# amathislab/BUCTD

Hardware: AMD Instinct MI355X
Metric: images/sec (train) BUCTD-CoAM-W48 384x288 (higher is better)
Workload: dtype f32 (3x3 convs: operands split exactly into 3 bf16 pieces, 6 bf16 MFMAs per product, fp32 accumulate - fp32-class); 1 GPU; BUCTD-CoAM-W48 (pose_hrnet_coam, ATT_MODULES [F,T,F,F], colored condition) 384x288 CrowdPose-14kpt full train step: fwd + JointsMSE + bwd + grad all-reduce + Adam + arg-max accuracy decode; global_batch=32, batch_per_gpu=32, input=N x 6 x 384 x 288 fp32, params=115581770, parallelism=dp1, hip_streams=4, conv_math=bf16x6, step_graph=False

## Files before the change

buctd_amd/_C.py:

```python
import ctypes as C
import os

import torch

_HERE = os.path.dirname(os.path.abspath(__file__))
LIB_PATH = os.path.join(_HERE, "lib", "libbuctd_hip.so")


class ConvDesc(C.Structure):
    _fields_ = [(n, C.c_int) for n in ("N", "H", "W", "Ci", "Co", "R", "S", "stride", "pad", "Ho", "Wo")]


class BasicBlockDesc(C.Structure):
    _fields_ = ([(n, C.c_int) for n in ("N", "H", "W", "C")] +
                [(n, C.c_void_p) for n in ("x", "w1_fwd", "w2_fwd", "w1_bwd", "w2_bwd", "gamma1", "beta1", "gamma2", "beta2",
                                           "running_mean1", "running_var1", "running_mean2", "running_var2")] +
                [(n, C.c_float) for n in ("eps1", "momentum1", "eps2", "momentum2")] +
                [(n, C.c_void_p) for n in ("z1", "z2", "y", "acc", "stat")])


class BasicBlockGrads(C.Structure):
    _fields_ = ([(n, C.c_void_p) for n in ("dy", "dz2", "dres", "dy1", "dz1", "dx", "dw1", "dw2", "dgamma1", "dbeta1",
                                           "dgamma2", "dbeta2")] +
                [(n, C.c_int) for n in ("acc_w1", "acc_w2", "acc_bn1", "acc_bn2")] +
                [("bn_acc", C.c_void_p), ("wg_ws", C.c_void_p), ("wg_ws_bytes", C.c_size_t)])


class BnAccIn(C.Structure):
    _fields_ = [("acc", C.c_void_p), ("rows", C.c_long), ("eps", C.c_float), ("momentum", C.c_float),
                ("mean_out", C.c_void_p), ("invstd_out", C.c_void_p), ("running_mean", C.c_void_p),
                ("running_var", C.c_void_p)]


class C3Conv(C.Structure):
    _fields_ = ([(n, C.c_int) for n in ("N", "H", "W", "Ci", "Co")] +
                [(n, C.c_void_p) for n in ("x", "wprep", "residual")] + [("relu", C.c_int)] +
                [(n, C.c_void_p) for n in ("y", "stats_acc")] + [("in_bn", C.POINTER(BnAccIn))] +
                [(n, C.c_void_p) for n in ("in_gamma", "in_beta")] + [("in_relu", C.c_int)] +
                [(n, C.c_void_p) for n in ("bn_z", "bn_y", "bn_mean", "bn_invstd", "bn_gamma", "bn_beta", "bn_acc")])


class C3ConvEval(C.Structure):
    _fields_ = ([(n, C.c_int) for n in ("N", "H", "W", "Ci", "Co")] +
                [(n, C.c_void_p) for n in ("x", "wprep", "scale", "shift", "residual")] + [("relu", C.c_int), ("y", C.c_void_p)])


class BnApplyItem(C.Structure):
    _fields_ = [("z", C.c_void_p), ("st", BnAccIn), ("gamma", C.c_void_p), ("beta", C.c_void_p), ("residual", C.c_void_p),
                ("relu", C.c_int), ("y", C.c_void_p), ("rows", C.c_long), ("C", C.c_int)]


class BnBwdItem(C.Structure):
    _fields_ = ([(n, C.c_void_p) for n in ("dy", "y", "z", "mean", "invstd", "gamma", "beta")] +
                [("relu", C.c_int), ("rows", C.c_long), ("C", C.c_int)] +
                [(n, C.c_void_p) for n in ("dz", "dres", "dgamma", "dbeta")] +
                [("accumulate", C.c_int), ("acc", C.c_void_p), ("acc_ready", C.c_int)])


class Wg3Conv(C.Structure):
    _fields_ = ([(n, C.c_int) for n in ("N", "H", "W", "Ci", "Co")] +
                [(n, C.c_void_p) for n in ("x", "dy", "dw")] + [("accumulate", C.c_int)] +
                [(n, C.c_void_p) for n in ("x_mean", "x_invstd", "x_gamma", "x_beta")] + [("x_relu", C.c_int)] +
                [("workspace", C.c_void_p), ("workspace_bytes", C.c_size_t)])


class MhaArgs(C.Structure):
    _fields_ = ([(n, C.c_int) for n in ("B", "T", "h", "dh")] +
                [(n, C.c_void_p) for n in ("q", "k", "v")] + [(n, C.c_int) for n in ("ldq", "ldk", "ldv")] +
                [("out", C.c_void_p), ("ldo", C.c_int), ("lse", C.c_void_p), ("scale", C.c_float), ("p_drop", C.c_float),
                 ("dout", C.c_void_p), ("lddo", C.c_int)] +
                [(n, C.c_void_p) for n in ("dq", "dk", "dv")] + [(n, C.c_int) for n in ("lddq", "lddk", "lddv")])


class RefineArgs(C.Structure):
    _fields_ = ([(n, C.c_void_p) for n in ("coords", "maxvals", "offset", "center", "scale", "box_score", "items",
                                           "cond_trunc", "cond_joints", "status", "hist_preds", "hist_score",
                                           "hist_box_score", "hist_keypoint_score", "hist_center", "hist_scale")] +
                [(n, C.c_int) for n in ("B", "K", "pass_", "passes", "heatmap_w", "heatmap_h", "crop_w", "crop_h")] +
                [(n, C.c_double) for n in ("margin", "aspect_ratio", "in_vis_thre", "scale_thre")])


class SampleGeomArgs(C.Structure):
    _fields_ = ([(n, C.c_void_p) for n in ("joints", "joints_vis", "cond", "cond_vis", "center", "scale", "bbox",
                                           "half_body", "draws", "bbox_draws", "flags", "pair", "items", "out_joints",
                                           "out_joints_vis", "out_cond", "out_cond_vis", "cond_trunc", "target_xy",
                                           "target_vis", "out_center", "out_scale", "out_rotation", "status")] +
                [(n, C.c_int) for n in ("B", "K", "crop_w", "crop_h", "keep_rect", "bbox_aug")] +
                [(n, C.c_double) for n in ("margin", "aspect_ratio", "scale_thre", "stride_x", "stride_y")])


class MatmulDesc(C.Structure):
    _fields_ = [
        ("batch", C.c_int), ("M", C.c_int), ("N", C.c_int), ("K", C.c_int),
        ("a_layout", C.c_int), ("b_layout", C.c_int),
        ("lda", C.c_int), ("ldb", C.c_int), ("ldc", C.c_int),
        ("stride_a", C.c_long), ("stride_b", C.c_long), ("stride_c", C.c_long),
        ("Kc", C.c_int), ("group_stride_a", C.c_long), ("group_stride_bk", C.c_long),
        ("Nc", C.c_int), ("group_stride_bn", C.c_long), ("group_stride_c", C.c_long),
        ("alpha", C.c_float), ("bias_axis", C.c_int),
    ]


_P = C.c_void_p
_I = C.c_int
_L = C.c_long
_F = C.c_float
_U64 = C.c_uint64
_SZ = C.c_size_t
_PD = C.POINTER(ConvDesc)
_PM = C.POINTER(MatmulDesc)
_PI = C.POINTER(C.c_int)

SIGNATURES = {
    "buctd_version": (_I, []),
    "buctd_last_error": (C.c_char_p, []),
    "buctd_conv2d_fwd": (_I, [_PD, _P, _P, _P, _P, _P, _P, _I, _P, _P, _P]),
    "buctd_conv2d_fwd_thin": (_I, [_PD]),
    "buctd_conv2d_dgrad": (_I, [_PD, _P, _P, _P, _P, _P, _P]),
    "buctd_conv2d_stats_groups": (_I, [_PD, _I, _PI, _PI]),
    "buctd_conv2d_wgrad_workspace": (_SZ, [_PD]),
    "buctd_conv2d_wgrad": (_I, [_PD, _P, _P, _P, _I, _P, _SZ, _P]),
    "buctd_conv2d_plan": (_I, [_PD, _I, _I, _PI]),
    "buctd_matmul_workspace": (_SZ, [_PM]),
    "buctd_matmul": (_I, [_PM, _P, _P, _P, _P, _P, _SZ, _P]),
    "buctd_matmul_plan": (_I, [_PM, _P, _P, _PI]),
    "buctd_bn_finalize": (_I, [_P, _P, _I, _I, _L, _I, _F, _F, _P, _P, _P, _P, _P]),
    "buctd_conv3x3_bf16x3_supported": (_I, [_I, _I, _I, _I, _I]),
    "buctd_conv3x3_bf16x3_stats_groups": (_I, [_I, _I, _I, _I, _I, _PI, _PI]),
    "buctd_conv3x3_bf16x3_prep_bytes": (_SZ, [_I, _I, _I]),
    "buctd_conv3x3_bf16x3_prep": (_I, [_I, _I, _P, _I, _P, _P]),
    "buctd_conv3x3_bf16x3_prep_batched": (_I, [_P, _I, _L, _P]),
    "buctd_conv3x3_bf16x3": (_I, [_I, _I, _I, _I, _I, _P, _P, _P, _P, _P, _P, _I, _P, _P, _P, _P]),
    "buctd_conv3x3_wgrad_bf16x3_supported": (_I, [_I, _I, _I, _I, _I]),
    "buctd_conv3x3_wgrad_bf16x3_workspace": (_SZ, [_I, _I, _I, _I, _I]),
    "buctd_conv3x3_wgrad_bf16x3": (_I, [_I, _I, _I, _I, _I, _P, _P, _P, _I, _P, _SZ, _P]),
    "buctd_conv3x3_bf16x6_supported": (_I, [_I, _I, _I, _I, _I]),
    "buctd_conv3x3_bf16x6_stats_groups": (_I, [_I, _I, _I, _I, _I, _PI, _PI]),
    "buctd_conv3x3_bf16x6_prep_bytes": (_SZ, [_I, _I, _I]),
    "buctd_conv3x3_bf16x6_prep": (_I, [_I, _I, _P, _I, _P, _P]),
    "buctd_conv3x3_bf16x6": (_I, [_I, _I, _I, _I, _I, _P, _P, _P, _P, _P, _P, _I, _P, _P, _P, _P]),
    "buctd_conv3x3_bf16x6_bnin": (_I, [_I, _I, _I, _I, _I, _P, _P, _P, _P, _P, _P, _I, _P, _P, _P, _P, _P, _P, _P, _I, _P]),
    "buctd_conv3x3_bf16x6_bnstat": (_I, [_I, _I, _I, _I, _I, _P, _P, _P, _P, _P, _P, _P, _P, _P, _P, _P, _P]),
    "buctd_bn_bwd_from_partials": (_I, [_P, _P, _P, _P, _P, _P, _P, _I, _L, _I, _P, _I, _P, _P, _P, _P, _I, _P, _SZ, _P]),
    "buctd_conv3x3_wgrad_bf16x6_bnin": (_I, [_I, _I, _I, _I, _I, _P, _P, _P, _I, _P, _P, _P, _P, _I, _P, _SZ, _P]),
    "buctd_conv3x3_wgrad_bf16x6_supported": (_I, [_I, _I, _I, _I, _I]),
    "buctd_conv3x3_wgrad_bf16x6_workspace": (_SZ, [_I, _I, _I, _I, _I]),
    "buctd_conv3x3_wgrad_bf16x6": (_I, [_I, _I, _I, _I, _I, _P, _P, _P, _I, _P, _SZ, _P]),
    "buctd_bn_stats": (_I, [_P, _L, _I, _P, _PI, _PI, _P]),
    "buctd_bn_stats_groups": (_I, [_L, _I, _PI, _PI]),
    "buctd_bn_apply": (_I, [_P, _P, _P, _P, _P, _P, _I, _P, _L, _I, _P]),
    "buctd_bn_bwd_workspace": (_SZ, [_L, _I]),
    "buctd_bn_bwd": (_I, [_P, _P, _P, _P, _P, _P, _P, _I, _L, _I, _P, _P, _P, _P, _I, _P, _SZ, _P]),
    "buctd_bn_fold": (_I, [_P, _P, _P, _P, _F, _I, _P, _P, _P]),
    "buctd_bn_acc_bytes": (_SZ, [_I]),
    "buctd_bn_apply_acc": (_I, [_P, C.POINTER(BnAccIn), _P, _P, _P, _I, _P, _L, _I, _P]),
    "buctd_bn_bwd_acc": (_I, [_P, _P, _P, _P, _P, _P, _P, _I, _L, _I, _P, _P, _P, _P, _I, _P, _I, _P]),
    "buctd_conv3x3_bf16x6_acc": (_I, [_I] * 5 + [_P, _P, _P, _I, _P, _P, C.POINTER(BnAccIn), _P, _P, _I, _P]),
    "buctd_conv3x3_bf16x6_bnstat_acc": (_I, [_I] * 5 + [_P] * 12),
    "buctd_gconv_x6_fwd_acc": (_I, [_I] * 6 + [_P] * 6),
    "buctd_conv3x3_bf16x6_group": (_I, [_I, C.POINTER(C3Conv), _P]),
    "buctd_conv3x3_bf16x6_group_eval": (_I, [_I, C.POINTER(C3ConvEval), _P]),
    "buctd_conv3x3_bf16x6_group_workgroups": (_I, [_I, C.POINTER(C3Conv)]),
    "buctd_conv3x3_bf16x6_plan": (_I, [_I, _I, _I, _I, _I, _I, C.POINTER(C.c_int)]),
    "buctd_conv3x3_wgrad_bf16x6_plan": (_I, [_I, _I, _I, _I, _I, C.POINTER(C.c_int)]),
    "buctd_gconv_wgrad_x6_supported": (_I, [_I] * 6),
    "buctd_gconv_wgrad_x6_workspace": (_SZ, [_I] * 6),
    "buctd_gconv_wgrad_x6": (_I, [_I] * 6 + [_P, _P, _P, _I, _P, _SZ, _P]),
    "buctd_bn_apply_acc_group": (_I, [_I, C.POINTER(BnApplyItem), _P]),
    "buctd_bn_bwd_acc_group": (_I, [_I, C.POINTER(BnBwdItem), _P]),
    "buctd_conv3x3_wgrad_bf16x6_group_workspace": (_SZ, [_I] * 6),
    "buctd_conv3x3_wgrad_bf16x6_group": (_I, [_I, C.POINTER(Wg3Conv), _P]),
    "buctd_conv3x3_wgrad_bf16x6_group_workgroups": (_I, [_I, C.POINTER(Wg3Conv)]),
    "buctd_stream_fork": (_I, [_P, _P]),
    "buctd_basic_branches_fwd_train": (_I, [_I, _I, C.POINTER(BasicBlockDesc), _P]),
    "buctd_basic_branches_bwd": (_I, [_I, _I, C.POINTER(BasicBlockDesc), C.POINTER(BasicBlockGrads), _P, _P]),
    "buctd_basic_chain_fwd_train": (_I, [_I, C.POINTER(BasicBlockDesc), _P]),
    "buctd_basic_chain_bwd": (_I, [_I, C.POINTER(BasicBlockDesc), C.POINTER(BasicBlockGrads), _P, _P]),
    "buctd_x6_image_dims": (_I, [_I, _I, _I, _P, _P]),
    "buctd_x6_image_bytes": (C.c_size_t, [_I, _I, _I]),
    "buctd_x6_image": (_I, [_P, _I, _I, _I, _L, _L, _I, _L, _L, _I, _P, _P]),
    "buctd_x6_gemm": (_I, [_I, _I, _I, _P, _P, _P, _I, _F, _P, _L, _I, _L, _P]),
    "buctd_add": (_I, [_P, _P, _P, _L, _I, _P]),
    "buctd_add_n": (_I, [C.POINTER(_P), _I, _P, _L, _P]),
    "buctd_mul": (_I, [_P, _P, _P, _L, _P]),
    "buctd_scale": (_I, [_P, _P, _F, _P, _L, _P]),
    "buctd_copy_channels": (_I, [_P, _L, _I, _I, _P, _I, _I, _I, _P]),
    "buctd_add_bcast": (_I, [_P, _P, _P, _L, _L, _P]),
    "buctd_relu_bwd": (_I, [_P, _P, _P, _L, _P]),
    "buctd_colsum_workspace": (_SZ, [_L, _I]),
    "buctd_colsum": (_I, [_P, _L, _I, _P, _I, _P, _SZ, _P]),
    "buctd_nchw_to_nhwc": (_I, [_P, _I, _I, _I, _I, _I, _I, _P, _P]),
    "buctd_nhwc_to_nchw": (_I, [_P, _I, _I, _I, _I, _P, _P]),
    "buctd_fuse_sum": (_I, [C.POINTER(_P), _PI, _I, _I, _I, _I, _I, _I, _P, _P]),
    "buctd_fuse_sum_bwd": (_I, [_P, _P, _I, _I, _I, _I, _I, _P, _P]),
    "buctd_resize_bilinear": (_I, [_P, _I, _I, _I, _I, _I, _I, _I, _I, _P, _P]),
    "buctd_maxpool3x3s2_fwd": (_I, [_P, _I, _I, _I, _I, _P, _P, _P]),
    "buctd_maxpool3x3s2_bwd": (_I, [_P, _P, _I, _I, _I, _I, _P, _P]),
    "buctd_softmax_dropout_fwd": (_I, [_P, _L, _I, _F, _F, _U64, _P, _P, _P]),
    "buctd_softmax_dropout_bwd": (_I, [_P, _P, _L, _I, _F, _F, _U64, _P, _P]),
    "buctd_softmax_dropout_fwd_dseed": (_I, [_P, _L, _I, _F, _F, _P, _P, _P, _P]),
    "buctd_softmax_dropout_bwd_dseed": (_I, [_P, _P, _L, _I, _F, _F, _P, _P, _P]),
    "buctd_dropout": (_I, [_P, _P, _L, _F, _U64, _P]),
    "buctd_dropout_dseed": (_I, [_P, _P, _L, _F, _P, _P]),
    "buctd_dropout_seed_fill": (_I, [_P, _I, _U64, _U64, _P]),
    "buctd_attn_smallqk_supported": (_I, [_I, _I, _I]),
    "buctd_attn_smallqk_fwd": (_I, [_I, _I, _I, _I, _P, _P, _P, _F, _F, _U64, _I, _P, _P, _P, _P]),
    "buctd_attn_smallqk_bwd": (_I, [_I, _I, _I, _I, _P, _P, _P, _P, _P, _P, _P, _F, _F, _U64, _I, _P, _P, _P, _P, _P]),
    "buctd_attn_smallqk_fwd_dseed": (_I, [_I, _I, _I, _I, _P, _P, _P, _F, _F, _P, _I, _P, _P, _P, _P]),
    "buctd_attn_smallqk_bwd_dseed": (_I, [_I, _I, _I, _I, _P, _P, _P, _P, _P, _P, _P, _F, _F, _P, _I, _P, _P, _P, _P, _P]),
    "buctd_layernorm_fwd": (_I, [_P, _P, _P, _L, _I, _F, _P, _P, _P, _P]),
    "buctd_add_layernorm_fwd": (_I, [_P, _P, _P, _P, _L, _I, _F, _P, _P, _P, _P, _P]),
    "buctd_layernorm_bwd_workspace": (_SZ, [_L, _I]),
    "buctd_layernorm_bwd": (_I, [_P, _P, _P, _P, _P, _L, _I, _P, _P, _P, _I, _P, _SZ, _P]),
    "buctd_joints_mse": (_I, [_P, _P, _P, _I, _I, _I, _P, _P, _F, _P, _SZ, _P]),
    "buctd_joints_ohkm_mse_workspace": (_SZ, [_I, _I]),
    "buctd_joints_ohkm_mse": (_I, [_P, _P, _P, _I, _I, _I, _I, _P, _P, _F, _P, _SZ, _P]),
    "buctd_argmax_decode": (_I, [_P, _I, _I, _I, _P, _P, _P, _P]),
    "buctd_warp_affine_norm": (_I, [_P, _I, _I, _I, _P, _P, _P, _L, _P, _P]),
    "buctd_cond_render_into": (_I, [_P, _I, _P, _I, _I, _I, _I, _I, _I, _P, _L, _P, _SZ, _P]),
    "buctd_cond_geometry": (_I, [_P, _P, _P, _P, _I, _I, _P, _P, _P, _P]),
    "buctd_cond_mirror": (_I, [_P, _I, _P, _P, _I, _I, _I, _P, _P]),
    "buctd_mirror_rows": (_I, [_P, _L, _P, _L, _P, _I, _I, _I, _I, _I, _P]),
    "buctd_refine_step": (_I, [C.POINTER(RefineArgs), _P]),
    "buctd_sample_geometry": (_I, [C.POINTER(SampleGeomArgs), _P]),
    "buctd_synthesize_pose": (_I, [_P, _P, _P, _P, _P, _P, _I, _I, _I, C.c_ulonglong, _P, _P]),
    "buctd_mha_fwd_supported": (_I, [_I, _I]),
    "buctd_mha_fwd": (_I, [_I, _I, _I, _P, _P, _P, _I, _I, _F, _P, _P, _P]),
    "buctd_mha_fwd_bf16x6": (_I, [_I, _I, _I, _P, _P, _P, _I, _I, _F, _P, _P, _P]),
    "buctd_gconv_x6_supported": (_I, [_I] * 7),
    "buctd_gconv_x6_prep_bytes": (_SZ, [_I, _I, _I, _I]),
    "buctd_gconv_x6_prep": (_I, [_I, _I, _I, _P, _I, _P, _P]),
    "buctd_gconv_x6_prep_item_bytes": (_SZ, []),
    "buctd_gconv_x6_prep_item": (_I, [_I, _I, _I, _P, _I, _P, _P]),
    "buctd_gconv_x6_prep_batched": (_I, [_P, _I, _P]),
    "buctd_gconv_x6_stats_groups": (_I, [_I] * 6 + [_PI, _PI]),
    "buctd_gconv_x6_fwd": (_I, [_I] * 6 + [_P] * 6 + [_I, _P, _P, _P, _P]),
    "buctd_gconv_x6_dgrad": (_I, [_I] * 6 + [_P] * 4 + [_P]),
    "buctd_mha_fwd_bf16x6_workspace": (_SZ, [_I, _I, _I]),
    "buctd_mha_fwd_bf16x6_ws": (_I, [_I, _I, _I, _P, _P, _P, _I, _I, _F, _P, _P, _P, _SZ, _P]),
    "buctd_mha_train_supported": (_I, [_I, _I]),
    "buctd_mha_fwd_train": (_I, [_I, _I, _I, _P, _P, _P, _I, _I, _F, _F, _U64, _P, _P, _P]),
    "buctd_mha_bwd_workspace": (_SZ, [_I, _I]),
    "buctd_mha_bwd": (_I, [_I, _I, _I, _P, _P, _P, _I, _I, _P, _P, _P, _F, _F, _U64, _P, _P, _I, _P, _I, _P, _SZ, _P]),
    "buctd_mha_fwd_train_dseed": (_I, [_I, _I, _I, _P, _P, _P, _I, _I, _F, _F, _P, _P, _P, _P]),
    "buctd_mha_bwd_dseed": (_I, [_I, _I, _I, _P, _P, _P, _I, _I, _P, _P, _P, _F, _F, _P, _P, _P, _I, _P, _I, _P, _SZ, _P]),
    "buctd_mha_heads_fwd_supported": (_I, [_I, _I, _I]),
    "buctd_mha_heads_fwd": (_I, [C.POINTER(MhaArgs), _P]),
    "buctd_mha_heads_fwd_bf16x6": (_I, [C.POINTER(MhaArgs), _P]),
    "buctd_mha_heads_train_supported": (_I, [_I, _I, _I]),
    "buctd_mha_heads_fwd_train": (_I, [C.POINTER(MhaArgs), _U64, _P]),
    "buctd_mha_heads_bwd_workspace": (_SZ, [_I, _I, _I]),
    "buctd_mha_heads_bwd": (_I, [C.POINTER(MhaArgs), _U64, _P, _SZ, _P]),
    "buctd_mha_heads_fwd_train_dseed": (_I, [C.POINTER(MhaArgs), _P, _P]),
    "buctd_mha_heads_bwd_dseed": (_I, [C.POINTER(MhaArgs), _P, _P, _SZ, _P]),
    "buctd_nms_workspace": (_SZ, [_I]),
    "buctd_nms": (_I, [_P, _P, _P, _I, _I, _F, _P, _SZ, _P]),
    "buctd_cpu_nms": (_I, [_P, _I, _P, _F, _P, _P]),
    "buctd_argmax_decode_refined": (_I, [_P, _I, _I, _I, _P, _P, _P, _P, _P]),
    "buctd_argmax_decode_dark": (_I, [_P, _I, _I, _I, _P, _P, _P, _P, _P]),
    "buctd_gaussian_target": (_I, [_P, _P, _I, _I, _I, _I, _F, _F, _F, _P, _P, _P]),
    "buctd_cond_render_workspace": (_SZ, [_I, _I, _I, _I]),
    "buctd_cond_render": (_I, [_P, _I, _P, _I, _I, _I, _I, _I, _I, _P, _P, _SZ, _P]),
    "buctd_flipback_avg": (_I, [_P, _P, _P, _I, _I, _I, _I, _I, _P, _P]),
    "buctd_sgd_step": (_I, [_P, _P, _P, _L, _F, _F, _F, _I, _I, _F, _P]),
    "buctd_adam_step": (_I, [_P, _P, _P, _P, _L, _F, _F, _F, _F, _I, _F, _P]),
    "buctd_bf16_pack_conv": (_I, [_P, _L, _L, _L, _L, _I, _I, _I, _P, _P, _P, _P, _P, _F, _P, _P, _P]),
    "buctd_bf16_conv": (_I, [_P, _I, _I, _I, _I, _P, _P, _I, _I, _I, _I, _P, _I, _I, _P, _P, _SZ, _P]),
    "buctd_bf16_fuse_sum": (_I, [C.POINTER(_P), _PI, _I, _I, _I, _I, _I, _I, _P, _P]),
    "buctd_bf16_from_f32": (_I, [_P, _L, _P, _P]),
}

_lib = None


class BuctdHipError(RuntimeError):
    pass


def lib():
    global _lib
    if _lib is None:
        if not os.path.isfile(LIB_PATH):
            raise BuctdHipError(
                f"{LIB_PATH} is missing - build it with `make` (or __graft_entry__.build()); "
                "buctd_amd has no CPU / eager fallback")
        handle = C.CDLL(LIB_PATH, mode=C.RTLD_GLOBAL)
        for name, (res, args) in SIGNATURES.items():
            fn = getattr(handle, name)
            fn.restype = res
            fn.argtypes = args
        _lib = handle
    return _lib


def check(rc, what=""):
    if rc != 0:
        msg = lib().buctd_last_error()
        raise BuctdHipError(f"{what} failed ({rc}): {msg.decode() if msg else ''}")


_raw_stream = getattr(torch._C, "_cuda_getCurrentRawStream", None)
_raw_device = getattr(torch._C, "_cuda_getDevice", None)


def current_stream_handle():
    if _raw_stream is not None and _raw_device is not None:
        return _raw_stream(_raw_device())
    return torch.cuda.current_stream().cuda_stream


def stream_ptr():
# ... 10 lines not shown
```

buctd_amd/csrc/block.hip:

```cpp
#include "common.h"
#include "../../include/buctd_hip.h"
#include <string.h>

#define BLK_TRY(call)      \
  do {                     \
    const int rc_ = (call); \
    if (rc_) return rc_;   \
  } while (0)

static bool fwd_ptrs_ok(const buctd_basic_block& b) {
  return b.x && b.w1_fwd && b.w2_fwd && b.z1 && b.z2 && b.y && b.acc && b.stat;
}

static bool bwd_ptrs_ok(const buctd_basic_block& b, const buctd_basic_block_grads& g) {
  return b.x && b.w1_bwd && b.w2_bwd && b.z1 && b.z2 && b.y && b.stat && g.dy && g.dres && g.dy1 && g.dw1 && g.dw2 && g.bn_acc &&
         g.wg_ws && g.dz2 && g.dz1;
}


static float* mean1_of(const buctd_basic_block& b) { return b.stat; }
static float* invstd1_of(const buctd_basic_block& b) { return b.stat + b.C; }
static float* mean2_of(const buctd_basic_block& b) { return b.stat + 2 * b.C; }
static float* invstd2_of(const buctd_basic_block& b) { return b.stat + 3 * b.C; }
static void* acc1_of(void* acc) { return acc; }
static void* acc2_of(void* acc, int C) { return (char*)acc + buctd_bn_acc_bytes(C); }

static void acc_in_of(const buctd_basic_block& b, int second, buctd_bn_acc_in* st) {
  st->acc = second ? acc2_of(b.acc, b.C) : acc1_of(b.acc);
  st->rows = (long)b.N * b.H * b.W;
  st->eps = second ? b.eps2 : b.eps1;
  st->momentum = second ? b.momentum2 : b.momentum1;
  st->mean_out = second ? mean2_of(b) : mean1_of(b);
  st->invstd_out = second ? invstd2_of(b) : invstd1_of(b);
  st->running_mean = second ? b.running_mean2 : b.running_mean1;
  st->running_var = second ? b.running_var2 : b.running_var1;
}

static buctd_c3_conv c3_of(const buctd_basic_block& b) {
  buctd_c3_conv c;
  memset(&c, 0, sizeof(c));
  c.N = b.N; c.H = b.H; c.W = b.W; c.Ci = c.Co = b.C;
  return c;
}

static int stream_fork(hipStream_t from, hipStream_t to, const char* who) {
  if (from == to) return BUCTD_OK;
  static thread_local hipEvent_t evs[16] = {nullptr};
  int devid = 0;
  if (hipGetDevice(&devid) != hipSuccess || devid < 0 || devid >= 16) {
    buctd_set_error("%s: cannot identify the current device", who);
    return BUCTD_ELAUNCH;
  }
  hipEvent_t& ev = evs[devid];
  if (!ev && hipEventCreateWithFlags(&ev, hipEventDisableTiming) != hipSuccess) {
    buctd_set_error("%s: hipEventCreate failed", who);
    return BUCTD_ELAUNCH;
  }
  if (hipEventRecord(ev, from) != hipSuccess || hipStreamWaitEvent(to, ev, 0) != hipSuccess) {
    buctd_set_error("%s: stream fork failed", who);
    return BUCTD_ELAUNCH;
  }
  return BUCTD_OK;
}

static int issue_conv_fwd(bool group, int n, const buctd_c3_conv* c, void* s) {
  if (group) return buctd_conv3x3_bf16x6_group(n, c, s);
  return buctd_conv3x3_bf16x6_acc(c->N, c->H, c->W, c->Ci, c->Co, c->x, c->wprep, c->residual, c->relu, c->y, c->stats_acc,
                                  c->in_bn, c->in_gamma, c->in_beta, c->in_relu, s);
}
static int issue_dgrad(bool group, int n, const buctd_c3_conv* c, void* s) {
  if (group) return buctd_conv3x3_bf16x6_group(n, c, s);
  if (c->bn_acc)
    return buctd_conv3x3_bf16x6_bnstat_acc(c->N, c->H, c->W, c->Ci, c->Co, c->x, c->wprep, c->residual, c->y, c->bn_z, c->bn_y,
                                           c->bn_mean, c->bn_invstd, c->bn_gamma, c->bn_beta, c->bn_acc, s);
  return buctd_conv3x3_bf16x6(c->N, c->H, c->W, c->Ci, c->Co, c->x, c->wprep, nullptr, nullptr, nullptr, c->residual, 0, c->y,
                              nullptr, nullptr, s);
}
static int issue_wgrad(bool group, int n, const buctd_wg3_conv* c, void* s) {
  if (group) return buctd_conv3x3_wgrad_bf16x6_group(n, c, s);
  if (c->x_mean)
    return buctd_conv3x3_wgrad_bf16x6_bnin(c->N, c->H, c->W, c->Ci, c->Co, c->x, c->dy, c->dw, c->accumulate, c->x_mean,
                                           c->x_invstd, c->x_gamma, c->x_beta, c->x_relu, c->workspace, c->workspace_bytes, s);
  return buctd_conv3x3_wgrad_bf16x6(c->N, c->H, c->W, c->Ci, c->Co, c->x, c->dy, c->dw, c->accumulate, c->workspace,
                                    c->workspace_bytes, s);
}
static int issue_bn_apply(bool group, int n, const buctd_bn_apply_item* a, void* s) {
  if (group) return buctd_bn_apply_acc_group(n, a, s);
  return buctd_bn_apply_acc(a->z, &a->st, a->gamma, a->beta, a->residual, a->relu, a->y, a->rows, a->C, s);
}
static int issue_bn_bwd(bool group, int n, const buctd_bn_bwd_item* i, void* s) {
  if (group) return buctd_bn_bwd_acc_group(n, i, s);
  return buctd_bn_bwd_acc(i->dy, i->y, i->z, i->mean, i->invstd, i->gamma, i->beta, i->relu, i->rows, i->C, i->dz, i->dres,
                          i->dgamma, i->dbeta, i->accumulate, i->acc, i->acc_ready, s);
}

#define BR_MAX 4

static int row_fwd_train(bool group, int nb, int n, const buctd_basic_block* blocks, void* stream) {
  for (int k = 0; k < n; ++k) {
    buctd_c3_conv cv[BR_MAX];
    buctd_bn_acc_in st1[BR_MAX];
    buctd_bn_apply_item ap[BR_MAX];
    for (int b = 0; b < nb; ++b) {
      const buctd_basic_block& B = blocks[b * n + k];
      buctd_c3_conv& c = cv[b] = c3_of(B);
      c.x = B.x; c.wprep = B.w1_fwd; c.y = B.z1; c.stats_acc = acc1_of(B.acc);
    }
    BLK_TRY(issue_conv_fwd(group, nb, cv, stream));
    for (int b = 0; b < nb; ++b) {
      const buctd_basic_block& B = blocks[b * n + k];
      buctd_c3_conv& c = cv[b];
      acc_in_of(B, 0, &st1[b]);
      c.x = B.z1; c.wprep = B.w2_fwd; c.y = B.z2; c.stats_acc = acc2_of(B.acc, B.C);
      c.in_bn = &st1[b]; c.in_gamma = B.gamma1; c.in_beta = B.beta1; c.in_relu = 1;
    }
    BLK_TRY(issue_conv_fwd(group, nb, cv, stream));
    for (int b = 0; b < nb; ++b) {
      const buctd_basic_block& B = blocks[b * n + k];
      buctd_bn_apply_item& a = ap[b];
      a.z = B.z2;
      acc_in_of(B, 1, &a.st);
      a.gamma = B.gamma2; a.beta = B.beta2; a.residual = B.x; a.relu = 1; a.y = B.y;
      a.rows = a.st.rows; a.C = B.C;
    }
    BLK_TRY(issue_bn_apply(group, nb, ap, stream));
  }
  return BUCTD_OK;
}

static bool bn2_sums_chain(const buctd_basic_block* b, const buctd_basic_block_grads* g) {
  return g->dx && g->dx == g[-1].dy && g[-1].bn_acc && b[-1].y == b->x && b[-1].N == b->N && b[-1].H == b->H && b[-1].W == b->W &&
         b[-1].C == b->C;
}

static int row_bwd(bool group, const char* who, int nb, int n, const buctd_basic_block* blocks,
                   const buctd_basic_block_grads* grads, void* stream, void* side_stream) {
  hipStream_t main_s = (hipStream_t)stream, side_s = side_stream ? (hipStream_t)side_stream : main_s;
  bool ready[BR_MAX] = {false, false, false, false};
  for (int k = n - 1; k >= 0; --k) {
    buctd_bn_bwd_item bi[BR_MAX];
    buctd_wg3_conv wg[BR_MAX];
    buctd_c3_conv cv[BR_MAX];
    bool chain[BR_MAX];
    for (int b = 0; b < nb; ++b) {
      const buctd_basic_block& B = blocks[b * n + k];
      const buctd_basic_block_grads& G = grads[b * n + k];
      chain[b] = k > 0 && bn2_sums_chain(&B, &G);
      bi[b] = buctd_bn_bwd_item{G.dy, B.y, B.z2, mean2_of(B), invstd2_of(B), B.gamma2, nullptr, 1, (long)B.N * B.H * B.W, B.C,
                                G.dz2, G.dres, G.dgamma2, G.dbeta2, G.acc_bn2, acc2_of(G.bn_acc, B.C), ready[b] ? 1 : 0};
    }
    BLK_TRY(issue_bn_bwd(group, nb, bi, stream));
    BLK_TRY(stream_fork(main_s, side_s, who));
    for (int b = 0; b < nb; ++b) {
      const buctd_basic_block& B = blocks[b * n + k];
      const buctd_basic_block_grads& G = grads[b * n + k];
      wg[b] = buctd_wg3_conv{B.N, B.H, B.W, B.C, B.C, B.z1, G.dz2, G.dw2, G.acc_w2, mean1_of(B), invstd1_of(B), B.gamma1, B.beta1,
                             1, G.wg_ws, G.wg_ws_bytes};
    }
    BLK_TRY(issue_wgrad(group, nb, wg, side_s));
    for (int b = 0; b < nb; ++b) {
      const buctd_basic_block& B = blocks[b * n + k];
      const buctd_basic_block_grads& G = grads[b * n + k];
      buctd_c3_conv& c = cv[b] = c3_of(B);
      c.x = G.dz2; c.wprep = B.w2_bwd; c.y = G.dy1;
      c.bn_z = B.z1; c.bn_mean = mean1_of(B); c.bn_invstd = invstd1_of(B); c.bn_gamma = B.gamma1; c.bn_beta = B.beta1;
      c.bn_acc = acc1_of(G.bn_acc);
    }
    BLK_TRY(issue_dgrad(group, nb, cv, stream));
    for (int b = 0; b < nb; ++b) {
      const buctd_basic_block& B = blocks[b * n + k];
      const buctd_basic_block_grads& G = grads[b * n + k];
      bi[b] = buctd_bn_bwd_item{G.dy1, nullptr, B.z1, mean1_of(B), invstd1_of(B), B.gamma1, B.beta1, 1, (long)B.N * B.H * B.W, B.C,
                                G.dz1, nullptr, G.dgamma1, G.dbeta1, G.acc_bn1, acc1_of(G.bn_acc), 1};
    }
    BLK_TRY(issue_bn_bwd(group, nb, bi, stream));
    BLK_TRY(stream_fork(main_s, side_s, who));
    for (int b = 0; b < nb; ++b) {
      const buctd_basic_block& B = blocks[b * n + k];
      const buctd_basic_block_grads& G = grads[b * n + k];
      wg[b] = buctd_wg3_conv{B.N, B.H, B.W, B.C, B.C, B.x, G.dz1, G.dw1, G.acc_w1, nullptr, nullptr, nullptr, nullptr, 0,
                             G.wg_ws, G.wg_ws_bytes};
    }
    BLK_TRY(issue_wgrad(group, nb, wg, side_s));
    int m = 0;
    for (int b = 0; b < nb; ++b) {
      const buctd_basic_block& B = blocks[b * n + k];
      const buctd_basic_block_grads& G = grads[b * n + k];
      ready[b] = chain[b];
      if (!G.dx) continue;
      buctd_c3_conv& c = cv[m++] = c3_of(B);
      c.x = G.dz1; c.wprep = B.w1_bwd; c.residual = G.dres; c.y = G.dx;
      if (chain[b]) {
        const buctd_basic_block& Bp = blocks[b * n + k - 1];
        c.bn_z = Bp.z2; c.bn_y = Bp.y; c.bn_mean = mean2_of(Bp); c.bn_invstd = invstd2_of(Bp); c.bn_gamma = Bp.gamma2;
        c.bn_acc = acc2_of(grads[b * n + k - 1].bn_acc, B.C);
      }
    }
    if (m) BLK_TRY(issue_dgrad(group, m, cv, stream));
  }
  return BUCTD_OK;
}

extern "C" int buctd_basic_chain_fwd_train(int n, const buctd_basic_block* blocks, void* stream) {
  BUCTD_CHECK_ARG(n > 0 && blocks, "buctd_basic_chain_fwd_train: bad argument");
  for (int k = 0; k < n; ++k) BUCTD_CHECK_ARG(fwd_ptrs_ok(blocks[k]), "buctd_basic_chain_fwd_train: null pointer in block %d", k);
  return row_fwd_train(false, 1, n, blocks, stream);
}
extern "C" int buctd_basic_chain_bwd(int n, const buctd_basic_block* blocks, const buctd_basic_block_grads* grads, void* stream,
                                     void* side_stream) {
  BUCTD_CHECK_ARG(n > 0 && blocks && grads, "buctd_basic_chain_bwd: bad argument");
  for (int k = 0; k < n; ++k)
    BUCTD_CHECK_ARG(bwd_ptrs_ok(blocks[k], grads[k]), "buctd_basic_chain_bwd: null pointer in block %d", k);
  return row_bwd(false, "buctd_basic_chain_bwd", 1, n, blocks, grads, stream, side_stream);
}

extern "C" int buctd_basic_branches_fwd_train(int nb, int n, const buctd_basic_block* blocks, void* stream) {
  BUCTD_CHECK_ARG(nb > 0 && nb <= BR_MAX && n > 0 && blocks, "buctd_basic_branches_fwd_train: 1..%d branches", BR_MAX);
  for (int i = 0; i < nb * n; ++i)
    BUCTD_CHECK_ARG(fwd_ptrs_ok(blocks[i]), "buctd_basic_branches_fwd_train: null pointer in block %d", i);
  return row_fwd_train(true, nb, n, blocks, stream);
}
extern "C" int buctd_basic_branches_bwd(int nb, int n, const buctd_basic_block* blocks, const buctd_basic_block_grads* grads,
                                        void* stream, void* side_stream) {
  BUCTD_CHECK_ARG(nb > 0 && nb <= BR_MAX && n > 0 && blocks && grads, "buctd_basic_branches_bwd: 1..%d branches", BR_MAX);
  for (int i = 0; i < nb * n; ++i)
    BUCTD_CHECK_ARG(bwd_ptrs_ok(blocks[i], grads[i]), "buctd_basic_branches_bwd: null pointer in block %d", i);
  return row_bwd(true, "buctd_basic_branches_bwd", nb, n, blocks, grads, stream, side_stream);
}

extern "C" int buctd_stream_fork(void* from, void* to) {
  return stream_fork((hipStream_t)from, (hipStream_t)to, "buctd_stream_fork");
}
```

buctd_amd/csrc/c3_common.h:

```cpp
#pragma once
#include "common.h"
#include <stdlib.h>
#include "../../include/buctd_hip.h"
#include "bn_acc.h"

typedef __bf16 bf16x8 __attribute__((ext_vector_type(8)));
typedef unsigned short u16x4 __attribute__((ext_vector_type(4)));

#define CK 32

template <int NP> struct Geo;
template <> struct Geo<2> {
  static constexpr int ROWB = 160;
  static constexpr int PST = 64;
  static constexpr int CPR = 8;
  static constexpr int BROW = 128;
  static constexpr int BLDS = 160;
};
template <> struct Geo<3> {
  static constexpr int ROWB = 96;
  static constexpr int PST = 32;
  static constexpr int CPR = 4;
  static constexpr int BROW = 192;
  static constexpr int BLDS = 224;
};

struct C3Args {
  const float* x;
  const unsigned char* wp;
  float* out;
  const float* bias;
  const float* scale;
  const float* shift;
  const float* res;
  float* stats;
  int* counts;
  int N, H, W, Ci, Co;
  int SW, IB, P;
  int relu, na;
  const float* in_mean;
  const float* in_invstd;
  const float* in_gamma;
  const float* in_beta;
  int in_relu;
  int col_major;
  unsigned ib_mul, ib_sh, sw_mul, sw_sh;
  int omap, oH, oW, ost, oy0, ox0;
  const float* bs_z;
  const float* bs_y;
  const float* bs_mean;
  const float* bs_invstd;
  const float* bs_gamma;
  const float* bs_beta;
  float* bs_part;
  long long* stats_acc;
  long long* bs_acc;
  BnAccFwd in_acc;
};

#define C3G_MAX 4
struct C3Group {
  C3Args conv[C3G_MAX];
  int nconv;
  int tiles[C3G_MAX];
  int gx[C3G_MAX];
  int gy[C3G_MAX];
  int variant[C3G_MAX];
};

#define C3_EPI_EXCH_OFF 24576
#define C3_EPI_LDS (C3_EPI_EXCH_OFF + 256 * 16)

__device__ __forceinline__ int fast_div(int n, unsigned mul, unsigned sh) {
  return (int)(__umulhi((unsigned)n, mul) >> sh);
}

typedef float c3_f32x2 __attribute__((ext_vector_type(2)));
typedef __bf16 c3_bf16x2 __attribute__((ext_vector_type(2)));
typedef unsigned c3_u32x2 __attribute__((ext_vector_type(2)));
template <int NP, int PST>
__device__ __forceinline__ void split_store_pk(unsigned char* row, int c, f32x4 v) {
  c3_f32x2 lo = {v.x, v.y}, hi = {v.z, v.w};
#pragma unroll
  for (int q = 0; q < NP; ++q) {
    const unsigned a = __builtin_bit_cast(unsigned, __builtin_convertvector(lo, c3_bf16x2));
    const unsigned b = __builtin_bit_cast(unsigned, __builtin_convertvector(hi, c3_bf16x2));
    *reinterpret_cast<c3_u32x2*>(row + q * PST + 2 * c) = (c3_u32x2){a, b};
    if (q + 1 < NP) {
      lo -= (c3_f32x2){__uint_as_float(a << 16), __uint_as_float(a & 0xffff0000u)};
      hi -= (c3_f32x2){__uint_as_float(b << 16), __uint_as_float(b & 0xffff0000u)};
    }
  }
}

template <int NP, int PST>
__device__ __forceinline__ void split_store(unsigned char* row, int c, f32x4 v) {
#pragma unroll
  for (int q = 0; q < NP; ++q) {
    u16x4 pc;
#pragma unroll
    for (int j = 0; j < 4; ++j) {
      const __bf16 h = (__bf16)v[j];
      pc[j] = __builtin_bit_cast(unsigned short, h);
      v[j] -= (float)h;
    }
    *reinterpret_cast<u16x4*>(row + q * PST + 2 * c) = pc;
  }
}

#define MAX_SW 75

static inline int c3_row_width(int W) { return W + 1; }

template <int V>
struct IC { static constexpr int value = V; };

template <int MF, int NF, int WM, int WN>
__device__ __forceinline__ void c3_epilogue(const C3Args& p, f32x4 (&acc)[MF][NF], unsigned char* smem, int bx, int by,
                                            int p0, int n0) {
  const int t = threadIdx.x, lane = t & 63, wave = t >> 6;
  const int i16 = lane & 15, g = lane >> 4;
  const int wave_m = wave % WM, wave_n = wave / WM;
  constexpr int MR = MF * 16;
  constexpr int RH = (MR + 63) / 64;
  constexpr int LD = NF * 16 + 4;
  constexpr int EP = 1;
  static_assert(MR <= 128, "c3_epilogue: at most 128 rows per wave");
  float* stg = reinterpret_cast<float*>(smem) + wave * (EP * 16 * LD);
  int* rowoff = reinterpret_cast<int*>(smem) + 4 * EP * 16 * LD + wave * 128;
  unsigned long long vmask[RH];
  int cnt = 0;
#pragma unroll
  for (int h = 0; h < RH; ++h) {
    int myoff = -1;
    const int r = lane + 64 * h;
    if (r < MR) {
      const int pp = p0 + wave_m * MR + r;
      if (pp < p.P) {
        const int n = fast_div(pp, p.ib_mul, p.ib_sh);
        const int rem = pp - n * p.IB;
        const int yy = fast_div(rem, p.sw_mul, p.sw_sh), xx = rem - yy * p.SW;
        if (n < p.N && yy >= 1 && xx >= 1 && xx <= p.W)
          myoff = p.omap ? ((n * p.oH + (yy - 1) * p.ost + p.oy0) * p.oW + (xx - 1) * p.ost + p.ox0) * p.Co
                         : ((n * p.H + yy - 1) * p.W + xx - 1) * p.Co;
      }
    }
    vmask[h] = __ballot(myoff >= 0);
    cnt += __popcll(vmask[h]);
    rowoff[r] = myoff;
  }
  auto valid = [&](int row) -> bool { return (vmask[row >> 6] >> (row & 63)) & 1ull; };
  const int grp = bx * WM + wave_m;
  if (p.stats && p.counts && by == 0 && wave_n == 0 && lane == 0) p.counts[grp] = cnt;
  const int ncol0 = n0 + wave_n * NF * 16;
  float bv[NF];
#pragma unroll
  for (int nf = 0; nf < NF; ++nf) bv[nf] = p.bias ? p.bias[ncol0 + nf * 16 + i16] : 0.f;
  double2* exch = reinterpret_cast<double2*>(smem + C3_EPI_EXCH_OFF);
  if (p.stats || p.stats_acc) {
    const float inv_cnt = cnt > 0 ? 1.f / (float)cnt : 0.f;
#pragma unroll
    for (int nf = 0; nf < NF; ++nf) {
      float s1 = 0.f;
#pragma unroll
      for (int mf = 0; mf < MF; ++mf)
#pragma unroll
        for (int rg = 0; rg < 4; ++rg) s1 += valid(mf * 16 + g * 4 + rg) ? acc[mf][nf][rg] + bv[nf] : 0.f;
      s1 += __shfl_xor(s1, 16, 64);
      s1 += __shfl_xor(s1, 32, 64);
      const float mean = s1 * inv_cnt;
      float s2 = 0.f;
#pragma unroll
      for (int mf = 0; mf < MF; ++mf)
#pragma unroll
        for (int rg = 0; rg < 4; ++rg) {
          const float d = acc[mf][nf][rg] + bv[nf] - mean;
          s2 += valid(mf * 16 + g * 4 + rg) ? d * d : 0.f;
        }
      s2 += __shfl_xor(s2, 16, 64);
      s2 += __shfl_xor(s2, 32, 64);
      if (g == 0) {
        const int n = ncol0 + nf * 16 + i16;
        if (p.stats) *reinterpret_cast<float2*>(p.stats + ((long)grp * p.Co + n) * 2) = make_float2(mean, s2);
        if (p.stats_acc) {
          const double nn = (double)cnt, m = (double)mean;
          exch[wave_m * (WN * NF * 16) + wave_n * NF * 16 + nf * 16 + i16] = make_double2(nn * m, (double)s2 + nn * m * m);
        }
      }
    }
    if (p.stats_acc) {
      __syncthreads();
      if (t < WN * NF * 16) {
        double a1 = 0.0, a2 = 0.0;
#pragma unroll
        for (int w = 0; w < WM; ++w) {
          const double2 v = exch[w * (WN * NF * 16) + t];
          a1 += v.x;
          a2 += v.y;
        }
        bnacc_add(p.stats_acc, p.Co, bnacc_shard(), n0 + t, a1, a2);
      }
    }
  }
  constexpr int Q4 = NF * 4;
  constexpr int NACC = (64 % Q4 == 0) ? 1 : 3;
  static_assert(NF <= 4 && (64 % Q4 == 0 || Q4 == 12), "c3_epilogue: unexpected column count for the bs reduction");
  f32x4 bs1[NACC], bs2[NACC];
#pragma unroll
  for (int j = 0; j < NACC; ++j) bs1[j] = bs2[j] = (f32x4){0.f, 0.f, 0.f, 0.f};
  const bool bs_on = p.bs_part != nullptr || p.bs_acc != nullptr;
  const bool bs_rebuild = bs_on && p.bs_y == nullptr;
#define C3_EPI_SYNC() __builtin_amdgcn_wave_barrier()
  constexpr int NI = EP * NF;
  constexpr int NPASS = MF / EP;
  f32x4 pre_r[2][NI], pre_z[2][NI], pre_y[2][NI];
  const bool has_res = p.res != nullptr;
  const bool has_y = bs_on && !bs_rebuild;
  C3_EPI_SYNC();
  auto issue = [&](int ps, int buf) {
#pragma unroll
    for (int k = 0; k < NI; ++k) {
      const int item = lane + 64 * k;
      const int row = item / (NF * 4), c4 = item - row * (NF * 4);
      const int off = rowoff[ps * EP * 16 + row];
      const int o = off >= 0 ? off + ncol0 + c4 * 4 : 0;
      if (has_res) pre_r[buf][k] = *reinterpret_cast<const f32x4*>(p.res + o);
      if (bs_on) pre_z[buf][k] = *reinterpret_cast<const f32x4*>(p.bs_z + o);
      if (has_y) pre_y[buf][k] = *reinterpret_cast<const f32x4*>(p.bs_y + o);
    }
  };
  if (has_res || bs_on) issue(0, 0);
#pragma unroll
  for (int ps = 0; ps < NPASS; ++ps) {
    if (ps) C3_EPI_SYNC();
    if ((has_res || bs_on) && ps + 1 < NPASS) issue(ps + 1, (ps + 1) & 1);
#pragma unroll
    for (int e = 0; e < EP; ++e)
#pragma unroll
      for (int nf = 0; nf < NF; ++nf)
#pragma unroll
        for (int rg = 0; rg < 4; ++rg)
          stg[(e * 16 + g * 4 + rg) * LD + nf * 16 + i16] = acc[ps * EP + e][nf][rg] + bv[nf];
    C3_EPI_SYNC();
#pragma unroll
    for (int k = 0; k < NI; ++k) {
      const int item = lane + 64 * k;
      const int row = item / (NF * 4), c4 = item - row * (NF * 4);
      f32x4 v = *reinterpret_cast<const f32x4*>(stg + row * LD + c4 * 4);
      const int off = rowoff[ps * EP * 16 + row];
      const int n = ncol0 + c4 * 4;
      if (off >= 0) {
        if (p.scale) {
          const f32x4 sc = *reinterpret_cast<const f32x4*>(p.scale + n);
          const f32x4 sh = *reinterpret_cast<const f32x4*>(p.shift + n);
#pragma unroll
          for (int j = 0; j < 4; ++j) v[j] = v[j] * sc[j] + sh[j];
        }
        if (has_res) {
          const f32x4 r = pre_r[ps & 1][k];
#pragma unroll
          for (int j = 0; j < 4; ++j) v[j] += r[j];
        }
        if (p.relu) {
#pragma unroll
          for (int j = 0; j < 4; ++j) v[j] = fmaxf(v[j], 0.f);
        }
        *reinterpret_cast<f32x4*>(p.out + off + n) = v;
        if (bs_on) {
          const f32x4 zz = pre_z[ps & 1][k];
          const f32x4 mu = *reinterpret_cast<const f32x4*>(p.bs_mean + n);
          const f32x4 is = *reinterpret_cast<const f32x4*>(p.bs_invstd + n);
          f32x4 yy;
          if (bs_rebuild) {
            const f32x4 sc = is * *reinterpret_cast<const f32x4*>(p.bs_gamma + n);
            yy = (zz - mu) * sc + *reinterpret_cast<const f32x4*>(p.bs_beta + n);
          } else {
            yy = pre_y[ps & 1][k];
          }
          f32x4 gm = v;
#pragma unroll
          for (int j = 0; j < 4; ++j)
            if (!(yy[j] > 0.f)) gm[j] = 0.f;
          bs1[k % NACC] += gm;
          bs2[k % NACC] += gm * (zz - mu) * is;
        }
      }
    }
  }
  if (bs_on) {
    __syncthreads();
    f32x4* red = reinterpret_cast<f32x4*>(smem) + (size_t)wave * (NACC * 64 * 2);
#pragma unroll
    for (int j = 0; j < NACC; ++j) {
      red[(j * 64 + lane) * 2 + 0] = bs1[j];
      red[(j * 64 + lane) * 2 + 1] = bs2[j];
    }
    __syncthreads();
    if (lane < Q4) {
      f32x4 a1 = (f32x4){0.f, 0.f, 0.f, 0.f}, a2 = a1;
#pragma unroll
      for (int j = 0; j < NACC; ++j) {
        const int first = ((lane - (64 * j) % Q4) % Q4 + Q4) % Q4;
        for (int l = first; l < 64; l += Q4) {
          a1 += red[(j * 64 + l) * 2 + 0];
          a2 += red[(j * 64 + l) * 2 + 1];
        }
      }
      if (p.bs_part) {
        float* dst = p.bs_part + ((long)grp * 2) * p.Co + ncol0 + lane * 4;
        *reinterpret_cast<f32x4*>(dst) = a1;
        *reinterpret_cast<f32x4*>(dst + p.Co) = a2;
      }
      if (p.bs_acc) {
#pragma unroll
        for (int j = 0; j < 4; ++j)
          exch[wave_m * (WN * NF * 16) + wave_n * NF * 16 + lane * 4 + j] = make_double2((double)a1[j], (double)a2[j]);
      }
    }
    if (p.bs_acc) {
      __syncthreads();
      if (t < WN * NF * 16) {
        double a1 = 0.0, a2 = 0.0;
#pragma unroll
        for (int w = 0; w < WM; ++w) {
          const double2 v = exch[w * (WN * NF * 16) + t];
          a1 += v.x;
          a2 += v.y;
        }
        bnacc_add(p.bs_acc, p.Co, bnacc_shard(), n0 + t, a1, a2);
      }
    }
  }
}


static inline void magic_u32(unsigned d, unsigned* mul, unsigned* sh) {
  if (d == 1) { *mul = 0xFFFFFFFFu; *sh = 0; return; }
  unsigned l = 0;
  while ((1ull << l) < d) ++l;
  const unsigned long long m = ((1ull << (31 + l)) + d - 1) / d;
  *mul = (unsigned)m;
  *sh = l - 1;
}
```

buctd_amd/csrc/c3_lean.h:

```cpp
#pragma once
#include "c3_common.h"

enum { C3M_IN_BN = 1, C3M_STATS = 2, C3M_RES = 4, C3M_BS_REBUILD = 8, C3M_BS_Y = 16 };

#define C3_OOB 0x80000000u
__device__ __forceinline__ __amdgpu_buffer_rsrc_t c3_rsrc(const void* ptr, unsigned bytes) {
  return __builtin_amdgcn_make_buffer_rsrc(const_cast<void*>(ptr), 0, bytes, 0x00020000);
}
__device__ __forceinline__ f32x4 c3_bload(__amdgpu_buffer_rsrc_t r, unsigned off) {
  typedef unsigned u32x4_ __attribute__((ext_vector_type(4)));
  return __builtin_bit_cast(f32x4, __builtin_amdgcn_raw_buffer_load_b128(r, off, 0, 0));
}
__device__ __forceinline__ void c3_bstore(__amdgpu_buffer_rsrc_t r, unsigned off, f32x4 v) {
  typedef unsigned u32x4_ __attribute__((ext_vector_type(4)));
  __builtin_amdgcn_raw_buffer_store_b128(__builtin_bit_cast(u32x4_, v), r, off, 0, 0);
}

static inline size_t c3l_tab_bytes(int Ci, int BN) { return (size_t)3 * Ci * 4 + (size_t)4 * BN * 4; }

template <int MF, int NF, int WM, int WN, int MODE>
__device__ __forceinline__ void c3l_epilogue(const C3Args& p, f32x4 (&acc)[MF][NF], unsigned char* smem, float* tab, int p0,
                                             int n0) {
  constexpr bool STATS = (MODE & C3M_STATS) != 0, RES = (MODE & C3M_RES) != 0;
  constexpr bool BSR = (MODE & C3M_BS_REBUILD) != 0, BSY = (MODE & C3M_BS_Y) != 0, BS = BSR || BSY;
  static_assert(!(STATS && BS), "c3l_epilogue: forward statistics and backward sums never meet in one launch");
  const int t = threadIdx.x, lane = t & 63;
  const int wave = __builtin_amdgcn_readfirstlane(t >> 6);
  const int i16 = lane & 15, g = lane >> 4;
  const int wave_m = wave % WM, wave_n = wave / WM;
  constexpr int MR = MF * 16;
  constexpr int RH = (MR + 63) / 64;
  constexpr int LD = NF * 16 + 4;
  constexpr int BN = WN * NF * 16;
  constexpr int Q4 = NF * 4;
  constexpr int NACC = (64 % Q4 == 0) ? 1 : 3;
  constexpr int NI = NF;
  static_assert(MR <= 128 && NF <= 4 && (64 % Q4 == 0 || Q4 == 12), "c3l_epilogue: unexpected tile shape");
  float* stg = reinterpret_cast<float*>(smem) + wave * (16 * LD);
  int* rowoff = reinterpret_cast<int*>(smem) + 4 * 16 * LD + wave * 128;
  double2* exch = reinterpret_cast<double2*>(smem + C3_EPI_EXCH_OFF);

  const int oH = p.omap ? p.oH : p.H, oW = p.omap ? p.oW : p.W, ost = p.omap ? p.ost : 1;
  const int oy0 = p.omap ? p.oy0 : 0, ox0 = p.omap ? p.ox0 : 0;
  const unsigned obytes = (unsigned)p.N * oH * oW * p.Co * 4u;
  const __amdgpu_buffer_rsrc_t r_out = c3_rsrc(p.out, obytes);
  int cnt = 0;
  int r0 = -1;
#pragma unroll
  for (int h = 0; h < RH; ++h) {
    unsigned myoff = C3_OOB;
    const int r = lane + 64 * h;
    const int pp = p0 + wave_m * MR + r;
    const int n = fast_div(pp, p.ib_mul, p.ib_sh);
    const int rem = pp - n * p.IB;
    const int yy = fast_div(rem, p.sw_mul, p.sw_sh), xx = rem - yy * p.SW;
    if ((r < MR) & (pp < p.P) & (n < p.N) & (yy >= 1) & (xx >= 1) & (xx <= p.W))
      myoff = (unsigned)(((n * oH + (yy - 1) * ost + oy0) * oW + (xx - 1) * ost + ox0) * p.Co) * 4u;
    if (STATS) {
      const unsigned long long vm = __ballot(myoff != C3_OOB);
      cnt += __popcll(vm);
      if (r0 < 0 && vm) r0 = 64 * h + __builtin_ctzll(vm);
    }
    if (r < MR) reinterpret_cast<unsigned*>(rowoff)[r] = myoff;
  }
  const int ncol0 = n0 + wave_n * NF * 16;
  float* piv = tab + wave * (NF * 16);
  const float* btab = tab + wave_n * NF * 16;
  if constexpr (STATS) {
    r0 = r0 < 0 ? 0 : r0;
    const int mf0 = r0 >> 4, g0 = (r0 >> 2) & 3, rg0 = r0 & 3;
    float pv[NF];
#pragma unroll
    for (int nf = 0; nf < NF; ++nf) pv[nf] = 0.f;
#pragma unroll
    for (int mf = 0; mf < MF; ++mf)
      if (mf == mf0) {
#pragma unroll
        for (int nf = 0; nf < NF; ++nf)
          pv[nf] = rg0 == 0 ? acc[mf][nf][0] : rg0 == 1 ? acc[mf][nf][1] : rg0 == 2 ? acc[mf][nf][2] : acc[mf][nf][3];
      }
    if (g == g0) {
#pragma unroll
      for (int nf = 0; nf < NF; ++nf) piv[nf * 16 + i16] = pv[nf];
    }
  }
  __builtin_amdgcn_wave_barrier();

  const float* sp[NI];
  const unsigned* rp[NI];
  int c4_k[NI];
#pragma unroll
  for (int k = 0; k < NI; ++k) {
    const int item = lane + 64 * k;
    const int row = item / Q4;
    c4_k[k] = item - row * Q4;
    sp[k] = stg + row * LD + c4_k[k] * 4;
    rp[k] = reinterpret_cast<const unsigned*>(rowoff) + row;
  }
  const unsigned colb = (unsigned)ncol0 * 4u;
  f32x4 s1[NACC], s2[NACC], pq[NACC];
#pragma unroll
  for (int j = 0; j < NACC; ++j) {
    s1[j] = s2[j] = (f32x4){0.f, 0.f, 0.f, 0.f};
    if constexpr (STATS) pq[j] = *reinterpret_cast<const f32x4*>(piv + c4_k[j] * 4);
  }
  [[maybe_unused]] __amdgpu_buffer_rsrc_t r_res, r_z, r_y;
  if constexpr (RES) r_res = c3_rsrc(p.res, obytes);
  if constexpr (BS) r_z = c3_rsrc(p.bs_z, obytes);
  if constexpr (BSY) r_y = c3_rsrc(p.bs_y, obytes);
  f32x4 pre_r[2][RES ? NI : 1], pre_z[2][BS ? NI : 1], pre_y[2][BSY ? NI : 1];
  auto issue = [&](int ps, int buf) {
#pragma unroll
    for (int k = 0; k < NI; ++k) {
      const unsigned o = rp[k][ps * 16] + colb + c4_k[k] * 16;
      if constexpr (RES) pre_r[buf][k] = c3_bload(r_res, o);
      if constexpr (BS) pre_z[buf][k] = c3_bload(r_z, o);
      if constexpr (BSY) pre_y[buf][k] = c3_bload(r_y, o);
    }
  };
  if constexpr (RES || BS) issue(0, 0);
#pragma unroll
  for (int ps = 0; ps < MF; ++ps) {
    if (ps) __builtin_amdgcn_wave_barrier();
    if constexpr (RES || BS) {
      if (ps + 1 < MF) issue(ps + 1, (ps + 1) & 1);
    }
#pragma unroll
    for (int nf = 0; nf < NF; ++nf)
#pragma unroll
      for (int rg = 0; rg < 4; ++rg) stg[(g * 4 + rg) * LD + nf * 16 + i16] = acc[ps][nf][rg];
    __builtin_amdgcn_wave_barrier();
    f32x4 v[NI];
    unsigned off[NI];
#pragma unroll
    for (int k = 0; k < NI; ++k) {
      v[k] = *reinterpret_cast<const f32x4*>(sp[k]);
      off[k] = rp[k][ps * 16];
    }
#pragma unroll
    for (int k = 0; k < NI; ++k) {
      const bool ok = off[k] != C3_OOB;
      if constexpr (RES) v[k] += pre_r[ps & 1][k];
      c3_bstore(r_out, off[k] + colb + c4_k[k] * 16, v[k]);
      if constexpr (STATS) {
        f32x4 d = v[k] - pq[k % NACC];
#pragma unroll
        for (int j = 0; j < 4; ++j) d[j] = ok ? d[j] : 0.f;
        s1[k % NACC] += d;
        f32x4 q = s2[k % NACC];
#pragma unroll
        for (int j = 0; j < 4; ++j) q[j] = __builtin_fmaf(d[j], d[j], q[j]);
        s2[k % NACC] = q;
      }
      if constexpr (BS) {
        const f32x4 zz = pre_z[ps & 1][k];
        const f32x4 mu = *reinterpret_cast<const f32x4*>(btab + c4_k[k] * 4);
        const f32x4 is = *reinterpret_cast<const f32x4*>(btab + BN + c4_k[k] * 4);
        f32x4 yy;
        if constexpr (BSR) {
          const f32x4 sc = *reinterpret_cast<const f32x4*>(btab + 2 * BN + c4_k[k] * 4);
          yy = (zz - mu) * sc + *reinterpret_cast<const f32x4*>(btab + 3 * BN + c4_k[k] * 4);
        } else {
          yy = pre_y[ps & 1][k];
        }
        f32x4 gm;
#pragma unroll
        for (int j = 0; j < 4; ++j) gm[j] = (ok && yy[j] > 0.f) ? v[k][j] : 0.f;
        s1[k % NACC] += gm;
        f32x4 tm = gm * (zz - mu) * is;
        s2[k % NACC] += tm;
      }
    }
    if constexpr (STATS || BS) {
#pragma unroll
      for (int j = 0; j < NACC; ++j) asm volatile("" : "+v"(s1[j]), "+v"(s2[j]));
    }
  }
  if constexpr (STATS || BS) {
    __syncthreads();
    f32x4* red = reinterpret_cast<f32x4*>(smem) + (size_t)wave * (NACC * 64 * 2);
#pragma unroll
    for (int j = 0; j < NACC; ++j) {
      red[(j * 64 + lane) * 2 + 0] = s1[j];
      red[(j * 64 + lane) * 2 + 1] = s2[j];
    }
    __builtin_amdgcn_wave_barrier();
    if (lane < Q4) {
      if constexpr (BS) {
        f32x4 a1 = (f32x4){0.f, 0.f, 0.f, 0.f}, a2 = a1;
#pragma unroll
        for (int j = 0; j < NACC; ++j) {
          const int first = ((lane - (64 * j) % Q4) % Q4 + Q4) % Q4;
          for (int l = first; l < 64; l += Q4) {
            a1 += red[(j * 64 + l) * 2 + 0];
            a2 += red[(j * 64 + l) * 2 + 1];
          }
        }
#pragma unroll
        for (int j = 0; j < 4; ++j)
          exch[wave_m * BN + wave_n * NF * 16 + lane * 4 + j] = make_double2((double)a1[j], (double)a2[j]);
      } else {
        double a1[4] = {0.0, 0.0, 0.0, 0.0}, a2[4] = {0.0, 0.0, 0.0, 0.0};
#pragma unroll
        for (int j = 0; j < NACC; ++j) {
          const int first = ((lane - (64 * j) % Q4) % Q4 + Q4) % Q4;
          for (int l = first; l < 64; l += Q4) {
            const f32x4 u1 = red[(j * 64 + l) * 2 + 0], u2 = red[(j * 64 + l) * 2 + 1];
#pragma unroll
            for (int e = 0; e < 4; ++e) {
              a1[e] += (double)u1[e];
              a2[e] += (double)u2[e];
            }
          }
        }
        const double nn = (double)cnt;
#pragma unroll
        for (int e = 0; e < 4; ++e) {
          const double pi = (double)piv[lane * 4 + e];
          exch[wave_m * BN + wave_n * NF * 16 + lane * 4 + e] =
              make_double2(a1[e] + nn * pi, a2[e] + 2.0 * pi * a1[e] + nn * pi * pi);
        }
      }
    }
    __syncthreads();
    if (t < BN) {
      double a1 = 0.0, a2 = 0.0;
#pragma unroll
      for (int w = 0; w < WM; ++w) {
        const double2 v = exch[w * BN + t];
        a1 += v.x;
        a2 += v.y;
      }
      bnacc_add(STATS ? p.stats_acc : p.bs_acc, p.Co, bnacc_shard(), n0 + t, a1, a2);
    }
  }
}

template <int BM, bool IN_BN>
struct C3Stager {
  static constexpr int ROWB = Geo<3>::ROWB, PST = Geo<3>::PST, CPR = Geo<3>::CPR;
  static constexpr int RPP = 256 / CPR;
  static constexpr int PA = (BM + 2 * MAX_SW + 2 + RPP - 1) / RPP;
  static constexpr int P0 = (BM + 2 * 3 + 2) / RPP < PA ? (BM + 2 * 3 + 2) / RPP : PA;
  unsigned goff[PA], lrow[PA];
  f32x4 areg[PA];
  int arows, c4, prow;
  __amdgpu_buffer_rsrc_t r_x;

  __device__ __forceinline__ void init(const C3Args& p) {
    const int t = threadIdx.x;
    arows = p.na * 32;
    c4 = (t % CPR) * 4;
    prow = t / CPR;
    r_x = c3_rsrc(p.x, (unsigned)p.N * p.H * p.W * p.Ci * 4u);
#pragma unroll
    for (int q = 0; q < PA; ++q) {
      const int row = prow + RPP * q;
      lrow[q] = (unsigned)(row < arows ? row : arows - 1) * ROWB + 2 * c4;
    }
  }
  __device__ __forceinline__ void make(const C3Args& p, int p0) {
    const int halo = p.SW + 1;
#pragma unroll
    for (int q = 0; q < PA; ++q) {
      const int row = prow + RPP * q;
      const int pp = p0 - halo + row;
      const int n = fast_div(pp, p.ib_mul, p.ib_sh);
      const int rem = pp - n * p.IB;
      const int yy = fast_div(rem, p.sw_mul, p.sw_sh);
      const int xx = rem - yy * p.SW;
      const bool real = (row < arows) & (pp >= 0) & (pp < p.P) & (n < p.N) & (yy >= 1) & (xx >= 1) & (xx <= p.W);
      goff[q] = real ? (unsigned)(((n * p.H + yy - 1) * p.W + xx - 1) * p.Ci + c4) * 4u : C3_OOB;
    }
  }
  __device__ __forceinline__ void load(int c0) {
#pragma unroll
    for (int q = 0; q < P0; ++q) areg[q] = c3_bload(r_x, goff[q] + (unsigned)c0 * 4u);
#pragma unroll
    for (int q0 = P0; q0 < PA; q0 += 2)
      if (RPP * q0 < arows) {
        areg[q0] = c3_bload(r_x, goff[q0] + (unsigned)c0 * 4u);
        if (q0 + 1 < PA) areg[q0 + 1] = c3_bload(r_x, goff[q0 + 1] + (unsigned)c0 * 4u);
      }
  }
  __device__ __forceinline__ void store_pass(const C3Args& p, unsigned char* At, int q, const f32x4& mu, const f32x4& sc,
                                             const f32x4& be) {
    f32x4 v = areg[q];
    if constexpr (IN_BN) {
      const bool real = goff[q] != C3_OOB;
#pragma unroll
      for (int j = 0; j < 4; ++j) {
        const float u = (v[j] - mu[j]) * sc[j] + be[j];
        const float w = p.in_relu ? fmaxf(u, 0.f) : u;
        v[j] = real ? w : 0.f;
      }
    }
    split_store_pk<3, PST>(At + lrow[q], 0, v);
  }
  __device__ __forceinline__ void store(const C3Args& p, unsigned char* At, int c0, const float* bntab) {
    f32x4 mu = (f32x4){0.f, 0.f, 0.f, 0.f}, sc = mu, be = mu;
    if constexpr (IN_BN) {
      mu = *reinterpret_cast<const f32x4*>(bntab + c0 + c4);
      sc = *reinterpret_cast<const f32x4*>(bntab + p.Ci + c0 + c4);
      be = *reinterpret_cast<const f32x4*>(bntab + 2 * p.Ci + c0 + c4);
    }
#pragma unroll
    for (int q = 0; q < P0; ++q) store_pass(p, At, q, mu, sc, be);
#pragma unroll
    for (int q0 = P0; q0 < PA; q0 += 2)
      if (RPP * q0 < arows) {
        store_pass(p, At, q0, mu, sc, be);
        if (q0 + 1 < PA) store_pass(p, At, q0 + 1, mu, sc, be);
      }
  }
};

template <int MF, int NF, int WM, int WN, bool DBUF, bool BPF_, int MODE>
__device__ __forceinline__ void c3l_tile(const C3Args& p, unsigned char* smem, int bx, int by) {
  static_assert(DBUF || !BPF_, "c3l_tile: the single-buffer form fetches its B fragments in place (the next chunk's rows ride behind them)");
  constexpr bool IN_BN = (MODE & C3M_IN_BN) != 0;
// ... 158 lines not shown
```

buctd_amd/csrc/conv3x3.hip:

```cpp
#include "c3_common.h"
#include <string.h>

enum { C3M_IN_BN = 1, C3M_STATS = 2, C3M_RES = 4, C3M_BS_REBUILD = 8, C3M_BS_Y = 16 };
int c3_lean_launch(const C3Group& h, int fam, int mode, unsigned grid, size_t lds, hipStream_t st);

template <int NP, int MF, int NF, int WM, int WN>
__global__ __launch_bounds__(256, 2) void conv3x3_split_kernel(C3Args p) {
  using G = Geo<NP>;
  constexpr int ROWB = G::ROWB, PST = G::PST, CPR = G::CPR, BROW = G::BROW, BLDS = G::BLDS;
  constexpr int BM = WM * MF * 16, BN = WN * NF * 16;
  constexpr int RPP = 256 / CPR;
  constexpr int PA = (BM + 2 * MAX_SW + 2 + RPP - 1) / RPP;
  constexpr int BPR = BROW / 16;
  constexpr int PB = (BN * BPR + 255) / 256;
  extern __shared__ __attribute__((aligned(16))) unsigned char smem[];
  const int na = p.na;
  const int arows = na * 32;
  unsigned char* At = smem;
  unsigned char* Bt = smem + (size_t)arows * ROWB;

  const int t = threadIdx.x, lane = t & 63, wave = t >> 6;
  const int i16 = lane & 15, g = lane >> 4;
  const int wave_m = wave % WM, wave_n = wave / WM;

  int bx, by;
  {
    const unsigned gx = gridDim.x, gy = gridDim.y, total = gx * gy;
    const unsigned lin = blockIdx.y * gx + blockIdx.x;
    const unsigned xcd = lin & 7, idx = lin >> 3, per = total >> 3, rem = total & 7;
    const unsigned L = xcd < rem ? xcd * (per + 1) + idx : rem * (per + 1) + (xcd - rem) * per + idx;
    bx = (int)(L / gy);
    by = (int)(L - (unsigned)bx * gy);
  }
  const int p0 = bx * BM, n0 = by * BN;
  const int halo = p.SW + 1;
  const int c4 = (t % CPR) * 4;
  const int prow = t / CPR;

  int goff[PA];
#pragma unroll
  for (int q = 0; q < PA; ++q) {
    const int row = prow + RPP * q;
    const int pp = p0 - halo + row;
    int o = row < arows ? -1 : -2;
    if (row < arows && pp >= 0 && pp < p.P) {
      const int n = fast_div(pp, p.ib_mul, p.ib_sh);
      const int rem = pp - n * p.IB;
      const int yy = fast_div(rem, p.sw_mul, p.sw_sh);
      const int xx = rem - yy * p.SW;
      if (n < p.N && yy >= 1 && xx >= 1 && xx <= p.W) o = ((n * p.H + yy - 1) * p.W + xx - 1) * p.Ci;
    }
    goff[q] = o;
  }

  f32x4 areg[PA], breg[PB];
  auto load_a = [&](int c0, int cw) {
#pragma unroll
    for (int q = 0; q < PA; ++q)
      if (RPP * q < arows) {
        const bool ok = goff[q] >= 0 && c4 < cw * 16;
        areg[q] = *reinterpret_cast<const f32x4*>(p.x + (ok ? goff[q] + c0 + c4 : 0));
      }
  };
  auto store_a = [&](int cw) {
#pragma unroll
    for (int q = 0; q < PA; ++q)
      if (RPP * q < arows && goff[q] != -2) {
        const int row = prow + RPP * q;
        const bool ok = goff[q] >= 0 && c4 < cw * 16;
        split_store<NP, PST>(At + (size_t)row * ROWB, c4, ok ? areg[q] : (f32x4){0.f, 0.f, 0.f, 0.f});
      }
  };
  int bsrc[PB], bdst[PB];
#pragma unroll
  for (int q = 0; q < PB; ++q) {
    const int id = t + 256 * q;
    const int nl = id / BPR, pc = id - nl * BPR;
    const bool ok = nl < BN;
    bsrc[q] = ok ? (n0 + nl) * BROW + pc * 16 : 0;
    bdst[q] = ok ? nl * BLDS + pc * 16 : (nl & 15) * BLDS + BROW + (t & 1) * 16;
  }
  const long step_bytes = (long)p.Co * BROW;
  auto load_b = [&](int gs) {
    const unsigned char* src = p.wp + gs * step_bytes;
#pragma unroll
    for (int q = 0; q < PB; ++q) breg[q] = *reinterpret_cast<const f32x4*>(src + bsrc[q]);
  };
  auto store_b = [&](int buf) {
    unsigned char* dst = Bt + (size_t)buf * BN * BLDS;
#pragma unroll
    for (int q = 0; q < PB; ++q) *reinterpret_cast<f32x4*>(dst + bdst[q]) = breg[q];
  };

  f32x4 acc[MF][NF];
#pragma unroll
  for (int mf = 0; mf < MF; ++mf)
#pragma unroll
    for (int nf = 0; nf < NF; ++nf) acc[mf][nf] = (f32x4){0.f, 0.f, 0.f, 0.f};

  const int nfull = NP == 2 ? p.Ci / CK : 0;
  const int ntail = NP == 2 ? ((p.Ci % CK) ? 1 : 0) : p.Ci / 16;
  const int nchunks = nfull + ntail, last_step = nfull * 9 + ntail * 5 - 1;
  const unsigned char* abase = At + (size_t)(wave_m * MF * 16 + i16) * ROWB + (g & 1) * 16;
  const unsigned char* bbase = Bt + (size_t)(wave_n * NF * 16 + i16) * BLDS + g * 16;
  const bool lowk = g < 2;
  int gs = 0, buf = 0;

  auto run_chunk = [&](auto cw_tag) {
    constexpr int CW = decltype(cw_tag)::value;
    constexpr int NS = CW == 2 ? 9 : 5;
#pragma unroll
    for (int s = 0; s < NS; ++s) {
      load_b(gs < last_step ? gs + 1 : last_step);
      const int tap0 = CW == 2 ? s : 2 * s;
      const int tap1 = CW == 2 ? s : (2 * s + 1 < 9 ? 2 * s + 1 : 2 * s);
      const int o0 = ((tap0 / 3) * p.SW + tap0 % 3) * ROWB;
      const int o1 = ((tap1 / 3) * p.SW + tap1 % 3) * ROWB + (CW == 2 ? 32 : 0);
      const unsigned char* ap = abase + (lowk ? o0 : o1);
      const unsigned char* bp = bbase + (size_t)buf * BN * BLDS;
      bf16x8 a[NP][MF], b[NP][NF];
#pragma unroll
      for (int nf = 0; nf < NF; ++nf)
#pragma unroll
        for (int q = 0; q < NP; ++q) b[q][nf] = *reinterpret_cast<const bf16x8*>(bp + nf * 16 * BLDS + q * 64);
#pragma unroll
      for (int mf = 0; mf < MF; ++mf)
#pragma unroll
        for (int q = 0; q < NP; ++q) a[q][mf] = *reinterpret_cast<const bf16x8*>(ap + mf * 16 * ROWB + q * PST);
#pragma unroll
      for (int mf = 0; mf < MF; ++mf) {
#define C3_MMA(qa, qb)                                                                                          \
  _Pragma("unroll") for (int nf = 0; nf < NF; ++nf) acc[mf][nf] =                                                \
      __builtin_amdgcn_mfma_f32_16x16x32_bf16(a[qa][mf], b[qb][nf], acc[mf][nf], 0, 0, 0);
        if constexpr (NP == 3) {
          C3_MMA(2, 0) C3_MMA(0, 2) C3_MMA(1, 1) C3_MMA(1, 0) C3_MMA(0, 1) C3_MMA(0, 0)
        } else {
          C3_MMA(1, 0) C3_MMA(0, 1) C3_MMA(0, 0)
        }
#undef C3_MMA
      }
      store_b(buf ^ 1);
      __syncthreads();
      buf ^= 1;
      ++gs;
    }
  };

  const int cw0 = nfull > 0 ? 2 : 1;
  load_a(0, cw0);
  load_b(0);
  store_a(cw0);
  store_b(0);
  if (nchunks > 1) load_a(cw0 * 16, nfull > 1 ? 2 : 1);
  __syncthreads();
  int c_next = cw0 * 16;
  for (int ch = 0; ch < nchunks; ++ch) {
// ... 330 lines not shown
  }
  split_store<2, 64>(reinterpret_cast<unsigned char*>(it.wprep) + rown * 128, c4, v);
}

__device__ __forceinline__ void prep3_piece(const float* __restrict__ w, unsigned char* __restrict__ out, int Kc, int Nc,
                                            int flip, long idx) {
  const int k4 = (int)(idx & 7);
  const long rown = idx >> 3;
  const int n = (int)(rown % Nc), step = (int)(rown / Nc);
  const int chunk = step / 5, s = step - chunk * 5;
  const int tap = 2 * s + (k4 >> 2);
  const int cc = chunk * 16 + (k4 & 3) * 4;
  f32x4 v = (f32x4){0.f, 0.f, 0.f, 0.f};
  if (tap < 9) {
    if (!flip) v = *reinterpret_cast<const f32x4*>(w + ((long)n * 9 + tap) * Kc + cc);
    else {
#pragma unroll
      for (int j = 0; j < 4; ++j) v[j] = w[((long)(cc + j) * 9 + (8 - tap)) * Nc + n];
    }
  }
  const int lane = (k4 >> 1) * 16 + (n & 15);
  unsigned char* dst = out + (((size_t)step * (Nc / 16) + (n >> 4)) * 3) * 1024 + lane * 16;
  split_store<3, 1024>(dst, (k4 & 1) * 4, v);
}
__global__ __launch_bounds__(256) void conv3x3_prep3_kernel(const float* __restrict__ w, unsigned char* __restrict__ out,
                                                            int Kc, int Nc, int flip, long items) {
  const long idx = (long)blockIdx.x * 256 + threadIdx.x;
  if (idx >= items) return;
  prep3_piece(w, out, Kc, Nc, flip, idx);
}

struct C3Plan { int MF, NF, WM, WN, BM, BN, na; size_t lds; bool single; };


static int c3_steps(int Kc, int np) { return np == 3 ? (Kc / 16) * 5 : (Kc / CK) * 9 + ((Kc % CK) ? 5 : 0); }

static bool c3_plan(int np, int N, int H, int W, int Ci, int Co, C3Plan* pl) {
  if (N <= 0 || H <= 0 || W <= 0 || Ci <= 0 || Co <= 0 || Ci % 16 != 0 || Co % 16 != 0 || c3_row_width(W) > MAX_SW) return false;
  const int rowb = np == 3 ? Geo<3>::ROWB : Geo<2>::ROWB, blds = np == 3 ? Geo<3>::BLDS : Geo<2>::BLDS;
  const long P = (long)N * (H + 1) * c3_row_width(W) + c3_row_width(W);
  int nf, wn;
  if (Co % 96 == 0) { nf = 3; wn = 2; }
  else if (Co % 48 == 0) { nf = 3; wn = 1; }
  else if (Co % 128 == 0) { nf = 4; wn = 2; }
  else if (Co % 64 == 0) { nf = 4; wn = 1; }
  else if (Co % 32 == 0) { nf = 2; wn = 1; }
  else { nf = 1; wn = 1; }
  if (np == 2 && Co % 96 == 0 && ((P + 127) / 128) * (Co / 96) < 320) { nf = 3; wn = 1; }
  bool small = false;
  if (np == 3 && Co % 32 == 0 && ((P + 127) / 128) * ((Co + 95) / 96) < 200) { nf = 2; wn = 1; small = true; }
  int wm = 4 / wn, bn = wn * nf * 16;
  int mf = 1;
  const int cand[2] = {4, 2};
  for (int i = (nf == 4 ? 1 : 0); i < 2; ++i) {
    const long blocks = ((P + wm * cand[i] * 16 - 1) / (wm * cand[i] * 16)) * (Co / bn);
    const long need = np == 3 ? (small ? 160 : 224) : 320;
    if (blocks >= need) { mf = cand[i]; break; }
  }
  bool single = false;
  if (np == 3 && nf == 3 && wn == 1 && Co == bn) {
    const long b8 = (P + 511) / 512;
    if (b8 > 256 && b8 <= 512) {
      mf = 8; single = true;
      if ((P + 447) / 448 <= 512) mf = 7;
    }
  }
  pl->MF = mf; pl->NF = nf; pl->WM = wm; pl->WN = wn; pl->BM = wm * mf * 16; pl->BN = bn; pl->single = single;
  pl->na = (pl->BM + 2 * c3_row_width(W) + 3 + 31) / 32;
  size_t stage = (size_t)4 * (mf >= 2 ? 2 : 1) * 16 * (nf * 16 + 4) * 4 + 4 * 128 * 4;
  if (np == 3 && stage < (size_t)C3_EPI_LDS) stage = C3_EPI_LDS;
  if (np == 3) {
    const int nb = single ? 1 : 2;
    while ((size_t)nb * pl->na * 32 * rowb < stage) ++pl->na;
    pl->lds = (size_t)nb * pl->na * 32 * rowb + (size_t)3 * Ci * sizeof(float);
  } else {
    while ((size_t)pl->na * 32 * rowb < stage) ++pl->na;
    pl->lds = (size_t)pl->na * 32 * rowb + (size_t)2 * pl->BN * blds;
  }
  return pl->lds <= 160 * 1024;
}

static bool c3_np_ok(int np) { return np == 2 || np == 3; }

template <int NP, int MF, int NF, int WM, int WN>
static int c3_launch(const C3Args& a, const C3Plan& pl, hipStream_t st) {
  static unsigned char attr_done[3][BUCTD_MAX_DEVICES] = {{0}};
  void (*fn)(C3Args);
  int variant = 0;
  if constexpr (NP == 3) {
    if (MF >= 7) fn = conv3x3_x6_kernel<MF, NF, WM, WN, false, false, 2>;
    else { fn = conv3x3_x6_kernel<MF, NF, WM, WN, true, true, 2>; variant = 2; }
  }
  else fn = conv3x3_split_kernel<NP, (MF > 4 ? 4 : MF), NF, WM, WN>;
  if (const int rc = buctd_raise_lds_limit(reinterpret_cast<const void*>(fn), 160 * 1024, attr_done[variant], "conv3x3 (split bf16)"))
    return rc;
  dim3 grid(ceil_div(a.P, pl.BM), a.Co / pl.BN);
  hipLaunchKernelGGL(fn, grid, dim3(256), pl.lds, st, a);
  BUCTD_CHECK_LAUNCH("buctd_conv3x3 (split bf16)");
  return BUCTD_OK;
}

template <int NP>
static int c3_dispatch(const C3Args& a, const C3Plan& pl, hipStream_t st, bool dry = false) {
#define C3_CASE(mf, nf, wm, wn) \
  if (pl.MF == mf && pl.NF == nf && pl.WN == wn) return dry ? BUCTD_OK : c3_launch<NP, mf, nf, wm, wn>(a, pl, st);
#define C3_MF(nf, wm, wn) C3_CASE(4, nf, wm, wn) C3_CASE(2, nf, wm, wn) C3_CASE(1, nf, wm, wn)
  if constexpr (NP == 3) { C3_CASE(8, 3, 4, 1) C3_CASE(7, 3, 4, 1) C3_CASE(8, 3, 2, 2) }
  C3_MF(1, 4, 1) C3_MF(2, 4, 1) C3_MF(3, 4, 1) C3_MF(3, 2, 2)
  C3_CASE(2, 4, 4, 1) C3_CASE(1, 4, 4, 1) C3_CASE(2, 4, 2, 2) C3_CASE(1, 4, 2, 2)
#undef C3_MF
#undef C3_CASE
  buctd_set_error("conv3x3 (split bf16): no kernel for MF=%d NF=%d WN=%d", pl.MF, pl.NF, pl.WN);
  return BUCTD_EINVAL;
}

static int c3_supported(int np, int N, int H, int W, int Ci, int Co) {
  C3Plan pl;
  return c3_np_ok(np) && c3_plan(np, N, H, W, Ci, Co, &pl) ? 1 : 0;
}

static int c3_stats_groups(int np, int N, int H, int W, int Ci, int Co, int* ngroups, int* rows_per_group) {
  C3Plan pl;
  BUCTD_CHECK_ARG(ngroups && rows_per_group && c3_np_ok(np) && c3_plan(np, N, H, W, Ci, Co, &pl),
                  "buctd_conv3x3_*_stats_groups: unsupported shape");
  const long P = (long)N * (H + 1) * c3_row_width(W) + c3_row_width(W);
  *ngroups = ceil_div(P, pl.BM) * pl.WM;
  *rows_per_group = pl.MF * 16;
  return BUCTD_OK;
}

static size_t c3_prep_bytes(int np, int Ci, int Co, int flip) {
  if (!c3_np_ok(np) || Ci <= 0 || Co <= 0 || Ci % 16 != 0 || Co % 16 != 0) return 0;
  const int Kc = flip ? Co : Ci, Nc = flip ? Ci : Co;
  return (size_t)c3_steps(Kc, np) * Nc * (np == 3 ? Geo<3>::BROW : Geo<2>::BROW);
}

static int c3_prep(int np, int Ci, int Co, const float* w, int flip, void* wprep, void* stream) {
  BUCTD_CHECK_ARG(w && wprep && c3_np_ok(np), "buctd_conv3x3_*_prep: null pointer");
  BUCTD_CHECK_ARG(Ci > 0 && Co > 0 && Ci % 16 == 0 && Co % 16 == 0, "buctd_conv3x3_*_prep: Ci=%d Co=%d must be multiples of 16",
                  Ci, Co);
  const int Kc = flip ? Co : Ci, Nc = flip ? Ci : Co;
  const long pieces = (long)c3_steps(Kc, np) * Nc * 8;
  if (np == 3)
    hipLaunchKernelGGL(conv3x3_prep3_kernel, dim3(ceil_div(pieces, 256)), dim3(256), 0, (hipStream_t)stream, w,
                       (unsigned char*)wprep, Kc, Nc, flip ? 1 : 0, pieces);
  else
    hipLaunchKernelGGL(conv3x3_prep_kernel, dim3(ceil_div(pieces, 256)), dim3(256), 0, (hipStream_t)stream, w,
                       (unsigned char*)wprep, Kc, Nc, flip ? 1 : 0, pieces);
  BUCTD_CHECK_LAUNCH("buctd_conv3x3_*_prep");
  return BUCTD_OK;
}

struct C3InBn { const float* mean; const float* invstd; const float* gamma; const float* beta; int relu; };
struct C3BwdStat { const float* z; const float* y; const float* mean; const float* invstd; const float* gamma; const float* beta; float* part; long long* acc; };
struct C3Acc { long long* stats_acc; const buctd_bn_acc_in* in; };

static int c3_fill_shape(int np, int N, int H, int W, int Ci, int Co, C3Args& a, C3Plan& pl) {
  BUCTD_CHECK_ARG(c3_np_ok(np) && c3_plan(np, N, H, W, Ci, Co, &pl),
                  "buctd_conv3x3 (split bf16): unsupported shape N%d H%d W%d Ci%d Co%d", N, H, W, Ci, Co);
  a.N = N; a.H = H; a.W = W; a.Ci = Ci; a.Co = Co;
  a.SW = c3_row_width(W); a.IB = (H + 1) * a.SW;
  const long P = (long)N * a.IB + a.SW;
  BUCTD_CHECK_ARG(P < 2147483647L && (long)N * H * W * (Ci > Co ? Ci : Co) < 2147483647L,
                  "buctd_conv3x3 (split bf16): tensor too large");
  a.P = (int)P;
  a.na = pl.na;
  a.omap = 0; a.oH = H; a.oW = W; a.ost = 1; a.oy0 = a.ox0 = 0;
  a.col_major = (np == 3 && Co / pl.BN >= 2 && (size_t)c3_steps(Ci, 3) * Co * Geo<3>::BROW > ((size_t)3 << 20)) ? 1 : 0;
  magic_u32((unsigned)a.IB, &a.ib_mul, &a.ib_sh);
  magic_u32((unsigned)a.SW, &a.sw_mul, &a.sw_sh);
  return BUCTD_OK;
}

static int c3_fill(int np, int N, int H, int W, int Ci, int Co, const float* x, const void* wprep, const float* bias,
                   const float* scale, const float* shift, const float* residual, int relu, float* y,
                   float* stats_partials, int* stats_counts, const C3InBn* in_bn, const C3BwdStat* bst, const C3Acc* accs,
                   C3Args& a, C3Plan& pl) {
  BUCTD_CHECK_ARG(x && wprep && y, "buctd_conv3x3 (split bf16): null tensor pointer");
  if (const int rc = c3_fill_shape(np, N, H, W, Ci, Co, a, pl)) return rc;
  BUCTD_CHECK_ARG((scale == nullptr) == (shift == nullptr), "buctd_conv3x3 (split bf16): scale and shift go together");
  BUCTD_CHECK_ARG((stats_partials == nullptr) == (stats_counts == nullptr),
                  "buctd_conv3x3 (split bf16): stats partials and counts go together");
  a.x = x; a.wp = (const unsigned char*)wprep; a.out = y; a.bias = bias; a.scale = scale; a.shift = shift;
  a.res = residual; a.stats = stats_partials; a.counts = stats_counts;
  a.relu = relu;
  a.in_mean = a.in_invstd = a.in_gamma = a.in_beta = nullptr;
  a.in_relu = 0;
  if (in_bn && in_bn->mean) {
    BUCTD_CHECK_ARG(np == 3 && in_bn->invstd && in_bn->gamma && in_bn->beta,
                    "buctd_conv3x3: fused input BatchNorm needs the bf16x6 kernel and all four statistics arrays");
    a.in_mean = in_bn->mean; a.in_invstd = in_bn->invstd; a.in_gamma = in_bn->gamma; a.in_beta = in_bn->beta;
    a.in_relu = in_bn->relu;
  }
  a.stats_acc = nullptr; a.bs_acc = nullptr;
  memset(&a.in_acc, 0, sizeof(a.in_acc));
  if (accs) {
    BUCTD_CHECK_ARG(np == 3, "buctd_conv3x3: statistics accumulators need the bf16x6 kernel");
    a.stats_acc = accs->stats_acc;
    if (accs->in && accs->in->acc) {
      const buctd_bn_acc_in& i = *accs->in;
      BUCTD_CHECK_ARG(in_bn && !in_bn->mean && in_bn->gamma && in_bn->beta && i.rows > 0 && i.mean_out && i.invstd_out &&
                          (i.running_mean == nullptr) == (i.running_var == nullptr),
                      "buctd_conv3x3: input BatchNorm from an accumulator needs gamma, beta, rows, mean_out and invstd_out");
      a.in_gamma = in_bn->gamma; a.in_beta = in_bn->beta; a.in_relu = in_bn->relu;
      a.in_acc.acc = (const long long*)i.acc; a.in_acc.rows = (double)i.rows; a.in_acc.eps = i.eps; a.in_acc.momentum = i.momentum;
      a.in_acc.mean_out = i.mean_out; a.in_acc.invstd_out = i.invstd_out; a.in_acc.rmean = i.running_mean; a.in_acc.rvar = i.running_var;
    }
  }
  a.bs_z = a.bs_y = a.bs_mean = a.bs_invstd = a.bs_gamma = a.bs_beta = nullptr;
  a.bs_part = nullptr;
  if (bst && (bst->part || bst->acc)) {
    BUCTD_CHECK_ARG(np == 3 && bst->z && bst->mean && bst->invstd && (bst->y || (bst->gamma && bst->beta)),
                    "buctd_conv3x3: the BatchNorm-backward by-product needs the bf16x6 kernel, z, mean, invstd and y or gamma + beta");
    a.bs_z = bst->z; a.bs_y = bst->y; a.bs_mean = bst->mean; a.bs_invstd = bst->invstd; a.bs_gamma = bst->gamma;
    a.bs_beta = bst->beta; a.bs_part = bst->part; a.bs_acc = bst->acc;
  }
  return BUCTD_OK;
}

static int c3_lean_mask(int m) {
  switch (m) {
    case C3M_STATS: case C3M_STATS | C3M_IN_BN: case C3M_BS_REBUILD: case C3M_RES | C3M_BS_Y: case C3M_RES: return m;
    default: return -1;
  }
}

static int c3_lean_mode(const C3Args& a) {
  if ((long)a.N * a.H * a.W * (a.Ci > a.Co ? a.Ci : a.Co) * 4 >= 2147483648L) return -1;
  if (a.bias || a.scale || a.shift || a.relu || a.stats || a.counts || a.bs_part || a.omap || a.in_mean || a.in_invstd) return -1;
  if (a.in_acc.acc && (!a.in_gamma || !a.in_beta)) return -1;
  int m = 0;
  if (a.in_acc.acc) m |= C3M_IN_BN;
  if (a.stats_acc) m |= C3M_STATS;
  if (a.res) m |= C3M_RES;
  if (a.bs_acc) m |= a.bs_y ? C3M_BS_Y : C3M_BS_REBUILD;
  return c3_lean_mask(m);
}

static int c3_group_variant(const C3Plan& pl, int* fam, bool general = false) {
  struct V { int mf, nf, wm, wn; };
  static const V f0[] = {{7, 3, 4, 1}, {4, 3, 2, 2}, {2, 2, 4, 1}, {4, 3, 4, 1}, {4, 2, 4, 1}};
  static const V f1[] = {{4, 2, 4, 1}, {1, 4, 4, 1}, {2, 2, 4, 1}, {1, 2, 4, 1}, {2, 4, 4, 1}, {2, 4, 2, 2}, {1, 3, 4, 1}, {2, 3, 4, 1}};
  for (int f = 0; f < 2; ++f) {
    if (*fam >= 0 && *fam != f) continue;
    const V* l = f ? f1 : f0;
    const int n = f ? (general ? 8 : 6) : 5;
    for (int i = 0; i < n; ++i)
      if (l[i].mf == pl.MF && l[i].nf == pl.NF && l[i].wm == pl.WM && l[i].wn == pl.WN) {
        *fam = f;
        return i;
      }
  }
  return -1;
}

struct C3Dry { int kernel, fam, variant, wgs; };

static int c3_group_launch(int n, const C3Args* a, const C3Plan* pl, hipStream_t stream, bool* done, C3Dry* dry = nullptr) {
  *done = false;
  int order[C3G_MAX];
  double cost[C3G_MAX];
  int lean = c3_lean_mode(a[0]);
  for (int k = 0; k < n; ++k) {
    cost[k] = (double)pl[k].BM * pl[k].BN * a[k].Ci;
    order[k] = k;
    if (c3_lean_mode(a[k]) != lean) lean = -1;
  }
  if (n == 1 && lean < 0) return BUCTD_OK;
  int fam = -1;
  bool ok = false;
  int var[C3G_MAX];
  for (int f = 0; f < 2 && !ok; ++f) {
    ok = true;
    for (int k = 0; k < n && ok; ++k) {
      fam = f;
      var[k] = c3_group_variant(pl[k], &fam, lean < 0);
      ok = var[k] >= 0;
    }
  }
  if (!ok) return BUCTD_OK;
  for (int i = 1; i < n; ++i)
    for (int j = i; j > 0 && cost[order[j]] > cost[order[j - 1]]; --j) { const int t = order[j]; order[j] = order[j - 1]; order[j - 1] = t; }
  C3Group h;
  h.nconv = n;
  size_t lds = 0;
  unsigned per_xcd = 0;
  for (int i = 0; i < n; ++i) {
    const int k = order[i];
    h.conv[i] = a[k];
    h.gx[i] = ceil_div(h.conv[i].P, pl[k].BM);
    h.gy[i] = h.conv[i].Co / pl[k].BN;
    h.tiles[i] = h.gx[i] * h.gy[i];
    h.variant[i] = var[k];
    const size_t l = pl[k].lds + (lean >= 0 ? (size_t)4 * pl[k].BN * sizeof(float) : 0);
    if (l > lds) lds = l;
    per_xcd += ((unsigned)h.tiles[i] + 7) >> 3;
  }
  for (int i = n; i < C3G_MAX; ++i) h.tiles[i] = h.gx[i] = h.gy[i] = h.variant[i] = 0;
  if (lds > 160 * 1024) return BUCTD_OK;
  *done = true;
  if (dry) { *dry = C3Dry{1, fam, h.variant[0], (int)(per_xcd * 8)}; return BUCTD_OK; }
  if (lean >= 0) return c3_lean_launch(h, fam, lean, per_xcd * 8, lds, stream);
  static unsigned char attr_done[2][BUCTD_MAX_DEVICES] = {{0}};
  void (*fn)(C3Group) = fam ? conv3x3_x6_group_kernel<1> : conv3x3_x6_group_kernel<0>;
  if (const int rc = buctd_raise_lds_limit(reinterpret_cast<const void*>(fn), 160 * 1024, attr_done[fam], "buctd_conv3x3_bf16x6_group"))
    return rc;
  hipLaunchKernelGGL(fn, dim3(per_xcd * 8), dim3(256), lds, stream, h);
  BUCTD_CHECK_LAUNCH("buctd_conv3x3_bf16x6_group");
  return BUCTD_OK;
}

static int c3_launch_one(const C3Args& a, const C3Plan& pl, hipStream_t stream, C3Dry* dry = nullptr) {
  bool done = false;
  const int rc = c3_group_launch(1, &a, &pl, stream, &done, dry);
  if (rc || done) return rc;
  if (dry) *dry = C3Dry{0, -1, -1, ceil_div(a.P, pl.BM) * (a.Co / pl.BN)};
  return c3_dispatch<3>(a, pl, stream, dry != nullptr);
}

static int c3_run(int np, int N, int H, int W, int Ci, int Co, const float* x, const void* wprep, const float* bias,
                  const float* scale, const float* shift, const float* residual, int relu, float* y,
                  float* stats_partials, int* stats_counts, void* stream, const C3InBn* in_bn = nullptr,
                  const C3BwdStat* bst = nullptr, const C3Acc* accs = nullptr) {
  C3Args a;
  C3Plan pl;
  const int rc = c3_fill(np, N, H, W, Ci, Co, x, wprep, bias, scale, shift, residual, relu, y, stats_partials, stats_counts,
                         in_bn, bst, accs, a, pl);
  if (rc) return rc;
  return np == 3 ? c3_launch_one(a, pl, (hipStream_t)stream) : c3_dispatch<2>(a, pl, (hipStream_t)stream);
}

extern "C" int buctd_conv3x3_bf16x3_supported(int N, int H, int W, int Ci, int Co) { return c3_supported(2, N, H, W, Ci, Co); }
extern "C" int buctd_conv3x3_bf16x3_stats_groups(int N, int H, int W, int Ci, int Co, int* ngroups, int* rows_per_group) {
  return c3_stats_groups(2, N, H, W, Ci, Co, ngroups, rows_per_group);
}
extern "C" size_t buctd_conv3x3_bf16x3_prep_bytes(int Ci, int Co, int flip) { return c3_prep_bytes(2, Ci, Co, flip); }
extern "C" int buctd_conv3x3_bf16x3_prep(int Ci, int Co, const float* w, int flip, void* wprep, void* stream) {
  return c3_prep(2, Ci, Co, w, flip, wprep, stream);
}
extern "C" int buctd_conv3x3_bf16x3_prep_batched(const buctd_c3_prep_item* items_device, int n, long total_pieces,
                                                 void* stream) {
  BUCTD_CHECK_ARG(items_device && n > 0 && total_pieces > 0, "buctd_conv3x3_bf16x3_prep_batched: bad argument");
  hipLaunchKernelGGL(conv3x3_prep_batched_kernel, dim3(ceil_div(total_pieces, 256)), dim3(256), 0, (hipStream_t)stream,
                     items_device, n, total_pieces);
  BUCTD_CHECK_LAUNCH("buctd_conv3x3_bf16x3_prep_batched");
  return BUCTD_OK;
}
extern "C" int buctd_conv3x3_bf16x3(int N, int H, int W, int Ci, int Co, const float* x, const void* wprep,
                                    const float* bias, const float* scale, const float* shift, const float* residual,
                                    int relu, float* y, float* stats_partials, int* stats_counts, void* stream) {
  return c3_run(2, N, H, W, Ci, Co, x, wprep, bias, scale, shift, residual, relu, y, stats_partials, stats_counts, stream);
}

extern "C" int buctd_conv3x3_bf16x6_supported(int N, int H, int W, int Ci, int Co) { return c3_supported(3, N, H, W, Ci, Co); }
extern "C" int buctd_conv3x3_bf16x6_stats_groups(int N, int H, int W, int Ci, int Co, int* ngroups, int* rows_per_group) {
  return c3_stats_groups(3, N, H, W, Ci, Co, ngroups, rows_per_group);
}
extern "C" size_t buctd_conv3x3_bf16x6_prep_bytes(int Ci, int Co, int flip) { return c3_prep_bytes(3, Ci, Co, flip); }
extern "C" int buctd_conv3x3_bf16x6_prep(int Ci, int Co, const float* w, int flip, void* wprep, void* stream) {
  return c3_prep(3, Ci, Co, w, flip, wprep, stream);
}
extern "C" int buctd_conv3x3_bf16x6(int N, int H, int W, int Ci, int Co, const float* x, const void* wprep,
                                    const float* bias, const float* scale, const float* shift, const float* residual,
                                    int relu, float* y, float* stats_partials, int* stats_counts, void* stream) {
  return c3_run(3, N, H, W, Ci, Co, x, wprep, bias, scale, shift, residual, relu, y, stats_partials, stats_counts, stream);
}
extern "C" int buctd_conv3x3_bf16x6_bnin(int N, int H, int W, int Ci, int Co, const float* x, const void* wprep,
                                         const float* bias, const float* scale, const float* shift,
                                         const float* residual, int relu, float* y, float* stats_partials,
                                         int* stats_counts, const float* in_mean, const float* in_invstd,
                                         const float* in_gamma, const float* in_beta, int in_relu, void* stream) {
  C3InBn b{in_mean, in_invstd, in_gamma, in_beta, in_relu};
  return c3_run(3, N, H, W, Ci, Co, x, wprep, bias, scale, shift, residual, relu, y, stats_partials, stats_counts, stream, &b);
}

extern "C" int buctd_conv3x3_bf16x6_bnstat(int N, int H, int W, int Ci, int Co, const float* x, const void* wprep,
                                           const float* residual, float* y, const float* bn_z, const float* bn_y,
                                           const float* bn_mean, const float* bn_invstd, const float* bn_gamma,
                                           const float* bn_beta, float* bn_part, void* stream) {
  C3BwdStat b{bn_z, bn_y, bn_mean, bn_invstd, bn_gamma, bn_beta, bn_part, nullptr};
  BUCTD_CHECK_ARG(bn_part, "buctd_conv3x3_bf16x6_bnstat: null partials pointer");
  return c3_run(3, N, H, W, Ci, Co, x, wprep, nullptr, nullptr, nullptr, residual, 0, y, nullptr, nullptr, stream, nullptr,
                &b);
}

extern "C" int buctd_conv3x3_bf16x6_acc(int N, int H, int W, int Ci, int Co, const float* x, const void* wprep,
                                        const float* residual, int relu, float* y, void* stats_acc,
                                        const buctd_bn_acc_in* in_bn, const float* in_gamma, const float* in_beta, int in_relu,
                                        void* stream) {
  C3InBn b{nullptr, nullptr, in_gamma, in_beta, in_relu};
  C3Acc a{(long long*)stats_acc, in_bn};
  BUCTD_CHECK_ARG(!in_bn || in_bn->acc, "buctd_conv3x3_bf16x6_acc: in_bn without an accumulator");
  return c3_run(3, N, H, W, Ci, Co, x, wprep, nullptr, nullptr, nullptr, residual, relu, y, nullptr, nullptr, stream,
                in_bn ? &b : nullptr, nullptr, &a);
}
extern "C" int buctd_conv3x3_bf16x6_bnstat_acc(int N, int H, int W, int Ci, int Co, const float* x, const void* wprep,
                                               const float* residual, float* y, const float* bn_z, const float* bn_y,
                                               const float* bn_mean, const float* bn_invstd, const float* bn_gamma,
                                               const float* bn_beta, void* bn_acc, void* stream) {
  C3BwdStat b{bn_z, bn_y, bn_mean, bn_invstd, bn_gamma, bn_beta, nullptr, (long long*)bn_acc};
  BUCTD_CHECK_ARG(bn_acc, "buctd_conv3x3_bf16x6_bnstat_acc: null accumulator");
  return c3_run(3, N, H, W, Ci, Co, x, wprep, nullptr, nullptr, nullptr, residual, 0, y, nullptr, nullptr, stream, nullptr,
                &b);
}

static int c3_group_fill(int n, const buctd_c3_conv* convs, C3Args* a, C3Plan* pl) {
  for (int k = 0; k < n; ++k) {
    const buctd_c3_conv& c = convs[k];
    C3InBn ib{nullptr, nullptr, c.in_gamma, c.in_beta, c.in_relu};
    C3BwdStat bs{c.bn_z, c.bn_y, c.bn_mean, c.bn_invstd, c.bn_gamma, c.bn_beta, nullptr, (long long*)c.bn_acc};
    C3Acc ac{(long long*)c.stats_acc, c.in_bn};
    BUCTD_CHECK_ARG(!c.in_bn || c.in_bn->acc, "buctd_conv3x3_bf16x6_group: in_bn without an accumulator");
    const int rc = c3_fill(3, c.N, c.H, c.W, c.Ci, c.Co, c.x, c.wprep, nullptr, nullptr, nullptr, c.residual, c.relu, c.y,
                           nullptr, nullptr, c.in_bn ? &ib : nullptr, c.bn_acc ? &bs : nullptr, &ac, a[k], pl[k]);
    if (rc) return rc;
  }
  return BUCTD_OK;
}

extern "C" int buctd_conv3x3_bf16x6_group(int n, const buctd_c3_conv* convs, void* stream) {
  BUCTD_CHECK_ARG(n > 0 && n <= C3G_MAX && convs, "buctd_conv3x3_bf16x6_group: 1..%d convolutions", C3G_MAX);
  C3Args a[C3G_MAX];
  C3Plan pl[C3G_MAX];
  if (const int rc0 = c3_group_fill(n, convs, a, pl)) return rc0;
  bool done = false;
  const int rc = c3_group_launch(n, a, pl, (hipStream_t)stream, &done);
  if (rc || done) return rc;
  for (int k = 0; k < n; ++k)
    if (const int rc1 = c3_launch_one(a[k], pl[k], (hipStream_t)stream)) return rc1;
  return BUCTD_OK;
}

extern "C" int buctd_conv3x3_bf16x6_group_eval(int n, const buctd_c3_conv_eval* convs, void* stream) {
  BUCTD_CHECK_ARG(n > 0 && n <= C3G_MAX && convs, "buctd_conv3x3_bf16x6_group_eval: 1..%d convolutions", C3G_MAX);
  C3Args a[C3G_MAX];
  C3Plan pl[C3G_MAX];
  for (int k = 0; k < n; ++k) {
    const buctd_c3_conv_eval& c = convs[k];
    const int rc = c3_fill(3, c.N, c.H, c.W, c.Ci, c.Co, c.x, c.wprep, nullptr, c.scale, c.shift, c.residual, c.relu, c.y,
                           nullptr, nullptr, nullptr, nullptr, nullptr, a[k], pl[k]);
    if (rc) return rc;
  }
  bool done = false;
  const int rc = n > 1 ? c3_group_launch(n, a, pl, (hipStream_t)stream, &done) : BUCTD_OK;
  if (rc || done) return rc;
  for (int k = 0; k < n; ++k)
    if (const int rc1 = c3_dispatch<3>(a[k], pl[k], (hipStream_t)stream)) return rc1;
  return BUCTD_OK;
}

extern "C" int buctd_conv3x3_bf16x6_group_workgroups(int n, const buctd_c3_conv* convs) {
  BUCTD_CHECK_ARG(n > 0 && n <= C3G_MAX && convs, "buctd_conv3x3_bf16x6_group_workgroups: 1..%d convolutions", C3G_MAX);
  C3Args a[C3G_MAX];
  C3Plan pl[C3G_MAX];
  if (const int rc0 = c3_group_fill(n, convs, a, pl)) return rc0;
  bool done = false;
  C3Dry dry{};
  const int rc = c3_group_launch(n, a, pl, nullptr, &done, &dry);
  if (rc) return rc;
  return done ? dry.wgs : 0;
}

extern "C" int buctd_conv3x3_bf16x6_plan(int N, int H, int W, int Ci, int Co, int option_set, int* out) {
  BUCTD_CHECK_ARG(out && (option_set == -1 || c3_lean_mask(option_set) >= 0),
                  "buctd_conv3x3_bf16x6_plan: option set %d is not one of the train-mode sets (or -1)", option_set);
  static const float some = 0.f;
  const float* on = &some;
  C3Args a{};
  C3Plan pl;
  if (const int rc = c3_fill_shape(3, N, H, W, Ci, Co, a, pl)) return rc;
  if (option_set >= 0) {
    if (option_set & C3M_IN_BN) { a.in_acc.acc = (const long long*)on; a.in_gamma = a.in_beta = on; }
    if (option_set & C3M_STATS) a.stats_acc = (long long*)on;
    if (option_set & C3M_RES) a.res = on;
    if (option_set & (C3M_BS_REBUILD | C3M_BS_Y)) a.bs_acc = (long long*)on;
    if (option_set & C3M_BS_Y) a.bs_y = on;
  }
  C3Dry dry{};
  if (const int rc = c3_launch_one(a, pl, nullptr, &dry)) return rc;
  const int v[11] = {pl.MF, pl.NF, pl.WM, pl.WN, pl.single ? 1 : 0, a.col_major, dry.kernel, dry.fam, dry.variant, pl.BM, pl.BN};
  for (int i = 0; i < 11; ++i) out[i] = v[i];
  return BUCTD_OK;
}
```

buctd_amd/csrc/conv3x3_lean.hip:

```cpp
#include "c3_lean.h"

template <int FAM, int MODE>
__global__ __launch_bounds__(256, 2) void conv3x3_x6_lean_kernel(C3Group g_) {
  extern __shared__ __attribute__((aligned(16))) unsigned char smem[];
  const C3Group& g = *(const C3Group*)__builtin_amdgcn_kernarg_segment_ptr();
  const unsigned lin = blockIdx.x, xcd = lin & 7;
  unsigned idx = lin >> 3;
  int c = -1;
  unsigned L = 0;
  for (int k = 0; k < g.nconv; ++k) {
    const unsigned total = (unsigned)g.tiles[k], per = total >> 3, rem = total & 7;
    const unsigned mine = per + (xcd < rem ? 1u : 0u);
    if (idx < mine) {
      L = xcd < rem ? xcd * (per + 1) + idx : rem * (per + 1) + (xcd - rem) * per + idx;
      c = k;
      break;
    }
    idx -= mine;
  }
  if (c < 0) return;
  const C3Args& p = g.conv[c];
  int bx, by;
  if (p.col_major) {
    by = (int)(L / (unsigned)g.gx[c]);
    bx = (int)(L - (unsigned)by * g.gx[c]);
  } else {
    bx = (int)(L / (unsigned)g.gy[c]);
    by = (int)(L - (unsigned)bx * g.gy[c]);
  }
  const int v = g.variant[c];
  if constexpr (FAM == 0) {
    switch (v) {
      case 0: c3l_tile<7, 3, 4, 1, false, false, MODE>(p, smem, bx, by); break;
      case 1: c3l_tile<4, 3, 2, 2, true, true, MODE>(p, smem, bx, by); break;
      case 2: c3l_tile<2, 2, 4, 1, true, true, MODE>(p, smem, bx, by); break;
      case 3: c3l_tile<4, 3, 4, 1, true, true, MODE>(p, smem, bx, by); break;
      default: c3l_tile<4, 2, 4, 1, true, true, MODE>(p, smem, bx, by); break;
    }
  } else {
    switch (v) {
      case 0: c3l_tile<4, 2, 4, 1, true, true, MODE>(p, smem, bx, by); break;
      case 1: c3l_tile<1, 4, 4, 1, true, true, MODE>(p, smem, bx, by); break;
      case 2: c3l_tile<2, 2, 4, 1, true, true, MODE>(p, smem, bx, by); break;
      case 3: c3l_tile<1, 2, 4, 1, true, true, MODE>(p, smem, bx, by); break;
      case 4: c3l_tile<2, 4, 4, 1, true, true, MODE>(p, smem, bx, by); break;
      default: c3l_tile<2, 4, 2, 2, true, true, MODE>(p, smem, bx, by); break;
    }
  }
}

int c3_lean_launch(const C3Group& h, int fam, int mode, unsigned grid, size_t lds, hipStream_t st) {
  static unsigned char attr_done[2][5][BUCTD_MAX_DEVICES] = {{{0}}};
  void (*fn)(C3Group) = nullptr;
  int mi = -1;
#define C3L_PICK(i, m)                                                                               \
  if (mode == (m)) {                                                                                 \
    mi = i;                                                                                          \
    fn = fam ? conv3x3_x6_lean_kernel<1, (m)> : conv3x3_x6_lean_kernel<0, (m)>;                      \
  }
  C3L_PICK(0, C3M_STATS)
  C3L_PICK(1, C3M_STATS | C3M_IN_BN)
  C3L_PICK(2, C3M_BS_REBUILD)
  C3L_PICK(3, C3M_RES | C3M_BS_Y)
  C3L_PICK(4, C3M_RES)
#undef C3L_PICK
  if (!fn) {
    buctd_set_error("conv3x3 (bf16x6, train mode): no kernel for option set %d", mode);
    return BUCTD_EINVAL;
  }
  if (const int rc = buctd_raise_lds_limit(reinterpret_cast<const void*>(fn), 160 * 1024, attr_done[fam ? 1 : 0][mi],
                                           "conv3x3 (bf16x6, train mode)"))
    return rc;
  hipLaunchKernelGGL(fn, dim3(grid), dim3(256), lds, st, h);
  BUCTD_CHECK_LAUNCH("conv3x3 (bf16x6, train mode)");
  return BUCTD_OK;
}
```

buctd_amd/csrc/conv_gather_x6.hip:

```cpp
#include "c3_lean.h"
#include <string.h>

#define GC_MAXT 9
#define GC_TAB_OFF (56 * 1024)

struct GcClass {
  int ntaps, nhs, nsteps;
  int oy0, ox0;
  long wp_off;
  unsigned pdy, pdx;
};

struct GcArgs {
  C3Args e;
  const float* src;
  const unsigned char* wp;
  int SH, SWd, SC, ss, cpt;
  int ncls;
  GcClass cls[4];
};

template <int MF, int NF, int WM, int WN, int MODE>
__global__ __launch_bounds__(256, 2) void gconv_x6_kernel(GcArgs p) {
  constexpr int BM = WM * MF * 16, BN = WN * NF * 16, ROWB = 96, PST = 32, BROW = 192;
// ... 383 lines not shown
  for (; blk < p.nblocks; blk += nwaves) {
    f32x4 acc[2][NFT];
#pragma unroll
    for (int mf = 0; mf < 2; ++mf)
#pragma unroll
      for (int nf = 0; nf < NFT; ++nf) acc[mf][nf] = (f32x4){0.f, 0.f, 0.f, 0.f};
    for (int sIdx = 0; sIdx < KS; ++sIdx) {
      bf16x8 a[3][2];
#pragma unroll
      for (int mf = 0; mf < 2; ++mf) {
        c3_f32x2 v[4] = {{an[mf][0].x, an[mf][0].y}, {an[mf][0].z, an[mf][0].w}, {an[mf][1].x, an[mf][1].y}, {an[mf][1].z, an[mf][1].w}};
#pragma unroll
        for (int q = 0; q < 3; ++q) {
          unsigned w[4];
#pragma unroll
          for (int j = 0; j < 4; ++j) {
            w[j] = __builtin_bit_cast(unsigned, __builtin_convertvector(v[j], c3_bf16x2));
            if (q < 2) v[j] -= (c3_f32x2){__uint_as_float(w[j] << 16), __uint_as_float(w[j] & 0xffff0000u)};
          }
          typedef unsigned r1_u32x4 __attribute__((ext_vector_type(4)));
          a[q][mf] = __builtin_bit_cast(bf16x8, (r1_u32x4){w[0], w[1], w[2], w[3]});
        }
      }
      if (sIdx + 1 < KS) load_a(blk, sIdx + 1);
      else if (blk + nwaves < p.nblocks) load_a(blk + nwaves, 0);
      const unsigned char* bs = bl + (size_t)sIdx * Co * R1_WROW;
#pragma unroll
      for (int nf = 0; nf < NFT; ++nf) {
        bf16x8 b[3];
#pragma unroll
        for (int q = 0; q < 3; ++q) b[q] = *reinterpret_cast<const bf16x8*>(bs + (size_t)nf * 16 * R1_WROW + q * 64);
#define R1_MMA(qa, qb)                                                                                      \
  _Pragma("unroll") for (int mf = 0; mf < 2; ++mf) acc[mf][nf] =                                            \
      __builtin_amdgcn_mfma_f32_16x16x32_bf16(a[qa][mf], b[qb], acc[mf][nf], 0, 0, 0);
        R1_MMA(2, 0) R1_MMA(0, 2) R1_MMA(1, 1) R1_MMA(1, 0) R1_MMA(0, 1) R1_MMA(0, 0)
#undef R1_MMA
      }
    }
    if (first && p.stats_acc) {
      first = false;
#pragma unroll
      for (int nf = 0; nf < NFT; ++nf) piv[nf] = __shfl(acc[0][nf][0] + (p.bias ? p.bias[nf * 16 + i16] : 0.f), i16, 64);
    }
#pragma unroll
    for (int mf = 0; mf < 2; ++mf)
#pragma unroll
      for (int rg = 0; rg < 4; ++rg) nrows += ((long)blk * 32 + mf * 16 + g * 4 + rg < p.rows) ? 1 : 0;
#pragma unroll
    for (int mf = 0; mf < 2; ++mf) {
#pragma unroll
      for (int cg = 0; cg < NFT / 4; ++cg) {
#pragma unroll
        for (int nl = 0; nl < 4; ++nl) {
          const int nf = cg * 4 + nl;
          const float bv = p.bias ? p.bias[nf * 16 + i16] : 0.f;
#pragma unroll
          for (int rg = 0; rg < 4; ++rg) {
            const float v = acc[mf][nf][rg] + bv;
            stg[(g * 4 + rg) * R1_LD + nl * 16 + i16] = v;
            if ((long)blk * 32 + mf * 16 + g * 4 + rg < p.rows) {
              const float d = v - piv[nf];
              s1[nf] += d;
              s2[nf] = __builtin_fmaf(d, d, s2[nf]);
            }
          }
        }
        __builtin_amdgcn_wave_barrier();
#pragma unroll
        for (int k = 0; k < 4; ++k) {
          const int item = lane + 64 * k, row = item >> 4, c4 = item & 15;
          const long grow = (long)blk * 32 + mf * 16 + row;
          f32x4 v = *reinterpret_cast<const f32x4*>(stg + row * R1_LD + c4 * 4);
          if (grow < p.rows) {
            const long o = grow * Co + cg * 64 + c4 * 4;
            if (p.res) v += *reinterpret_cast<const f32x4*>(p.res + o);
            *reinterpret_cast<f32x4*>(p.out + o) = v;
          }
        }
        __builtin_amdgcn_wave_barrier();
      }
    }
  }
  if (p.stats_acc) {
    __syncthreads();
    double2* exch = reinterpret_cast<double2*>(smem);
#pragma unroll
    for (int nf = 0; nf < NFT; ++nf) {
      const double pi = (double)piv[nf], nn = (double)nrows;
      double a1 = (double)s1[nf] + nn * pi, a2 = (double)s2[nf] + 2.0 * pi * (double)s1[nf] + nn * pi * pi;
      a1 += __shfl_xor(a1, 16, 64); a1 += __shfl_xor(a1, 32, 64);
      a2 += __shfl_xor(a2, 16, 64); a2 += __shfl_xor(a2, 32, 64);
      if (g == 0) exch[wave * Co + nf * 16 + i16] = make_double2(a1, a2);
    }
    __syncthreads();
    for (int c = t; c < Co; c += 512) {
      double a1 = 0.0, a2 = 0.0;
#pragma unroll
      for (int w = 0; w < 8; ++w) {
        const double2 v = exch[w * Co + c];
        a1 += v.x;
        a2 += v.y;
      }
      bnacc_add(p.stats_acc, Co, bnacc_shard(), c, a1, a2);
    }
  }
}

static bool r1_ok(int kind, long rows, int cin, int cout) {
  if (kind != 1 || cin % 32 || (cout != 64 && cout != 128 && cout != 256)) return false;
  const size_t lds = (size_t)(cin / 32) * cout * R1_WROW + (size_t)8 * R1_STG;
  return lds <= 150 * 1024 && (size_t)8 * cout * 16 <= (size_t)(cin / 32) * cout * R1_WROW && rows >= 65536;
}

static int r1_run(long rows, int cin, int cout, const float* x, const void* wprep, const float* bias, const float* residual, float* out,
                  long long* stats_acc, hipStream_t st, const char* who) {
  R1Args a;
  a.x = x; a.wp = (const unsigned char*)wprep; a.bias = bias; a.res = residual; a.out = out; a.stats_acc = stats_acc;
  a.rows = rows; a.Ci = cin; a.Co = cout; a.nblocks = (int)((rows + 31) / 32);
  const size_t lds = (size_t)(cin / 32) * cout * R1_WROW + (size_t)8 * R1_STG;
  static unsigned char done[3][BUCTD_MAX_DEVICES] = {{0}};
  void (*fn)(R1Args) = cout == 64 ? conv1x1_rows_x6_kernel<4> : cout == 128 ? conv1x1_rows_x6_kernel<8> : conv1x1_rows_x6_kernel<16>;
  if (const int rc = buctd_raise_lds_limit(reinterpret_cast<const void*>(fn), 160 * 1024, done[cout == 64 ? 0 : cout == 128 ? 1 : 2], who))
    return rc;
  int grid = 256;
  if (grid * 8 > a.nblocks) grid = (a.nblocks + 7) / 8;
  hipLaunchKernelGGL(fn, dim3(grid), dim3(512), lds, st, a);
  BUCTD_CHECK_LAUNCH(who);
  return BUCTD_OK;
}

static int gc_run(int kind, int dir, int N, int H, int W, int Ci, int Co, const float* src, const void* wprep, const float* bias,
                  const float* scale, const float* shift, const float* residual, int relu, float* out, float* stats_partials,
                  int* stats_counts, void* stream, const char* who, long long* stats_acc = nullptr) {
  int Hg, Wg, SH, SWd, SC, nout;
  BUCTD_CHECK_ARG(src && wprep && out, "%s: null tensor pointer", who);
  BUCTD_CHECK_ARG(gc_geo(kind, dir, N, H, W, Ci, Co, &Hg, &Wg, &SH, &SWd, &SC, &nout),
                  "%s: unsupported shape kind %d N%d H%d W%d Ci%d Co%d", who, kind, N, H, W, Ci, Co);
  BUCTD_CHECK_ARG((scale == nullptr) == (shift == nullptr), "%s: scale and shift go together", who);
  BUCTD_CHECK_ARG((stats_partials == nullptr) == (stats_counts == nullptr), "%s: stats partials and counts go together", who);
  BUCTD_CHECK_ARG(!(dir && stats_partials), "%s: no statistics on the data gradient", who);
  if (!scale && !relu && !stats_partials && r1_ok(kind, (long)N * H * W, SC, nout))
    return r1_run((long)N * H * W, SC, nout, src, wprep, bias, residual, out, stats_acc, (hipStream_t)stream, who);
  GcPlan pl;
  gc_plan(nout, (long)N * (Hg + 1) * (Wg + 2) + Wg + 2, &pl);
  GcArgs a;
  C3Args& e = a.e;
  e.x = nullptr; e.wp = nullptr; e.out = out; e.bias = bias; e.scale = scale; e.shift = shift; e.res = residual;
  e.stats = stats_partials; e.counts = stats_counts;
  e.N = N; e.H = Hg; e.W = Wg; e.Ci = SC; e.Co = nout;
  e.SW = Wg + 2; e.IB = (Hg + 1) * (Wg + 2);
  e.P = (int)((long)N * e.IB + e.SW);
  e.relu = relu; e.na = 0;
  e.in_mean = e.in_invstd = e.in_gamma = e.in_beta = nullptr; e.in_relu = 0; e.col_major = 0;
  e.bs_z = e.bs_y = e.bs_mean = e.bs_invstd = e.bs_gamma = e.bs_beta = nullptr; e.bs_part = nullptr;
  e.stats_acc = stats_acc; e.bs_acc = nullptr;
  memset(&e.in_acc, 0, sizeof(e.in_acc));
  BUCTD_CHECK_ARG(!(dir && stats_acc), "%s: no statistics on the data gradient", who);
  magic_u32((unsigned)e.IB, &e.ib_mul, &e.ib_sh);
  magic_u32((unsigned)e.SW, &e.sw_mul, &e.sw_sh);
  const bool par = kind == 2 && dir;
  e.omap = par ? 1 : 0; e.oH = H; e.oW = W; e.ost = par ? 2 : 1; e.oy0 = e.ox0 = 0;
  a.src = src; a.wp = (const unsigned char*)wprep;
  a.SH = SH; a.SWd = SWd; a.SC = SC; a.ss = (kind == 2 && !dir) ? 2 : 1; a.cpt = SC / 16;
  a.ncls = gc_ncls(kind, dir);
  long off = 0;
  int tr[GC_MAXT], ts[GC_MAXT];
  for (int c = 0; c < 4; ++c) {
    GcClass& k = a.cls[c];
    k.ntaps = k.nhs = k.nsteps = 0; k.oy0 = k.ox0 = 0; k.wp_off = 0; k.pdy = k.pdx = 0u;
    if (c >= a.ncls) continue;
    int tdy[GC_MAXT], tdx[GC_MAXT];
    k.ntaps = gc_taps(kind, dir, c, tr, ts, tdy, tdx);
    k.pdy = k.pdx = 0u;
    for (int t = 0; t < k.ntaps; ++t) {
      k.pdy |= (unsigned)(tdy[t] + 1) << (2 * t);
      k.pdx |= (unsigned)(tdx[t] + 1) << (2 * t);
    }
    k.nhs = k.ntaps * a.cpt;
    k.nsteps = (k.nhs + 1) / 2;
    k.oy0 = par ? (c >> 1) : 0; k.ox0 = par ? (c & 1) : 0;
    k.wp_off = off;
    off += (long)gc_class_bytes(k.ntaps, SC, nout);
  }
  const int tiles = (e.P + pl.BM - 1) / pl.BM, ncol = nout / pl.BN;
  hipStream_t st = (hipStream_t)stream;
  int mode = -1;
  if (!bias && !scale && !relu && !stats_partials && !(stats_acc && residual) &&
      (long)N * H * W * (Ci > Co ? Ci : Co) * 4 < 2147483648L)
    mode = stats_acc ? C3M_STATS : residual ? C3M_RES : 0;
  if (pl.NF == 3 && pl.WM == 2) gc_launch<4, 3, 2, 2>(a, tiles, ncol, st, mode);
  else if (pl.NF == 4 && pl.WM == 2) gc_launch<4, 4, 2, 2>(a, tiles, ncol, st, mode);
  else if (pl.NF == 4) gc_launch<2, 4, 4, 1>(a, tiles, ncol, st, mode);
  else gc_launch<2, 3, 4, 1>(a, tiles, ncol, st, mode);
  BUCTD_CHECK_LAUNCH(who);
  return BUCTD_OK;
}

extern "C" int buctd_gconv_x6_fwd(int kind, int N, int H, int W, int Ci, int Co, const float* x, const void* wprep,
                                  const float* bias, const float* scale, const float* shift, const float* residual, int relu,
                                  float* y, float* stats_partials, int* stats_counts, void* stream) {
  return gc_run(kind, 0, N, H, W, Ci, Co, x, wprep, bias, scale, shift, residual, relu, y, stats_partials, stats_counts, stream,
                "buctd_gconv_x6_fwd");
}

extern "C" int buctd_gconv_x6_fwd_acc(int kind, int N, int H, int W, int Ci, int Co, const float* x, const void* wprep,
                                      const float* bias, float* y, void* stats_acc, void* stream) {
  BUCTD_CHECK_ARG(stats_acc, "buctd_gconv_x6_fwd_acc: null accumulator");
  return gc_run(kind, 0, N, H, W, Ci, Co, x, wprep, bias, nullptr, nullptr, nullptr, 0, y, nullptr, nullptr, stream,
                "buctd_gconv_x6_fwd_acc", (long long*)stats_acc);
}

extern "C" int buctd_gconv_x6_dgrad(int kind, int N, int H, int W, int Ci, int Co, const float* dy, const void* wprep,
                                    const float* residual, float* dx, void* stream) {
  return gc_run(kind, 1, N, H, W, Ci, Co, dy, wprep, nullptr, nullptr, nullptr, residual, 0, dx, nullptr, nullptr, stream,
                "buctd_gconv_x6_dgrad");
}
```

buctd_amd/ops.py:

```python
import ctypes as C
import math

import torch

from . import _C
from ._C import ConvDesc, MatmulDesc, check, lib, ptr, stream_ptr

_capture = {"on": False, "events": set(), "allow_seeds": False, "seed_table": None, "seed_draws": 0}
_SEED_TABLE_SLOTS = 1024


def capturing():
    return _capture["on"]


def _new_event(stream=None):
    ev = torch.cuda.Event()
    ev.record(stream) if stream is not None else ev.record()
    if _capture["on"]:
        _capture["events"].add(id(ev))
        _capture.setdefault("keep", []).append(ev)
    return ev


# ... 1477 lines not shown
        return y

    @staticmethod
    def backward(ctx, dy):
        c1, c2, c3, cd = ctx.sub
        _unpack_subs(ctx, ctx.sub)
        r3 = ConvBnAct.backward(c3, dy)
        d_out2, dres = r3[0], r3[4]
        d_out1 = ConvBnAct.backward(c2, d_out2)[0]
        dx = None
        if ctx.needs_input_grad[0]:
            if cd is not None:
                dres = ConvBnAct.backward(cd, dres)[0]
            c1.dx_residual = dres
        elif cd is not None:
            ConvBnAct.backward(cd, dres)
        dx = ConvBnAct.backward(c1, d_out1)[0]
        for c in ctx.sub:
            if c is not None:
                c.saved_tensors = ()
        return dx, None, None


class ForkConvBnFn(torch.autograd.Function):

    @staticmethod
    def forward(ctx, x, w0, groups):
        need = ctx.needs_input_grad[0]
        subs, outs = [], []
        for conv, bn, relu in groups:
            c = _SubCtx(need)
            s, p = conv._geom()
            outs.append(ConvBnAct.forward(c, x, conv.weight, conv.bias, bn, None, relu, s, p, True, None))
            subs.append(c)
        ctx.sub = subs
        _pack_subs(ctx, subs)
        return tuple(outs)

    @staticmethod
    def backward(ctx, *dys):
        subs = ctx.sub
        _unpack_subs(ctx, subs)
        dx = None
        for c, dy in zip(subs, dys):
            if dy is None:
                continue
            c.dx_residual = dx
            r = ConvBnAct.backward(c, dy)[0]
            dx = r if r is not None else dx
        for c in subs:
            c.saved_tensors = ()
        return dx, None, None


class BasicBlockFn(torch.autograd.Function):

    @staticmethod
    def forward(ctx, x, w1, bn1, w2, bn2):
        fuse = bn_in_fusable(tuple(x.shape), w2)
        veto = native_block_veto["fn"]
        if (fuse and bn_in_fusable(tuple(x.shape), w1) and bn1.track_running_stats == bn2.track_running_stats
                and not (veto is not None and veto(tuple(x.shape)))):
            ctx.native = True
            return _chain_forward(ctx, x, [(w1, bn1, w2, bn2)])
        ctx.native = False
        z1, part, info = conv_fwd(x, w1, None, 1, 1, stats="acc")
        Cn = z1.shape[-1]
        rows = z1.numel() // Cn
        y1 = None
        if info[0] == "acc":
            bnin1 = BnAccInput(part, rows, bn1, True, relu=True)
            if fuse:
                z2, part2, info2 = conv_fwd(z1, w2, None, 1, 1, stats="acc", in_bn=bnin1)
            else:
                y1 = bn_apply_acc(z1, bnin1, None, True)
                z2, part2, info2 = conv_fwd(y1, w2, None, 1, 1, stats="acc")
            bnin2 = BnAccInput(part2, rows, bn2, True)
            y = bn_apply_acc(z2, bnin2, x, True)
            mean1, invstd1, mean2, invstd2 = bnin1.mean, bnin1.invstd, bnin2.mean, bnin2.invstd
        else:
            def fin(bn, part, info):
                track = bn.track_running_stats
                return bn_finalize(part, info, rows, Cn, bn.eps, 0.1 if bn.momentum is None else bn.momentum,
                                   bn.running_mean if track else None, bn.running_var if track else None)
            mean1, invstd1 = fin(bn1, part, info)
            if fuse:
                z2, part2, info2 = conv_fwd(z1, w2, None, 1, 1, stats=True, in_bn=(mean1, invstd1, bn1.weight, bn1.bias, True))
            else:
                y1 = bn_apply(z1, mean1, invstd1, bn1.weight, bn1.bias, None, True)
                z2, part2, info2 = conv_fwd(y1, w2, None, 1, 1, stats=True)
            mean2, invstd2 = fin(bn2, part2, info2)
            y = bn_apply(z2, mean2, invstd2, bn2.weight, bn2.bias, x, True)
        for bn in (bn1, bn2):
            if bn.track_running_stats:
                _count_batch(bn)
        ctx.meta = (w1, bn1, w2, bn2, fuse)
        ctx.save_for_backward(x, z1, mean1, invstd1, None if fuse else y1, z2, mean2, invstd2, y)
        return y

    @staticmethod
    def backward(ctx, dy):
        if ctx.native:
            return _chain_backward(ctx, dy, ctx.needs_input_grad[0]), None, None, None, None
        w1, bn1, w2, bn2, fuse = ctx.meta
        x, z1, mean1, invstd1, y1, z2, mean2, invstd2, y2 = ctx.saved_tensors
        dy = _contig(dy)
        dg, acc_g = grad_target(bn2.weight)
        db, acc_b = grad_target(bn2.bias)
        assert acc_g == acc_b
        dz2, dres = bn_bwd(dy, y2, z2, mean2, invstd2, bn2.weight, True, True, dg, db, acc_g)
        dy1 = conv_dgrad(dz2, w2, tuple(z1.shape), 1, 1)
        dw, acc_w = grad_target(w2)
        if fuse:
            conv_wgrad_async(z1, dz2, w2, 1, 1, dw, acc_w, x_bn=(mean1, invstd1, bn1.weight, bn1.bias, True))
        else:
            conv_wgrad_async(y1, dz2, w2, 1, 1, dw, acc_w)
        grad_done(bn2.weight, bn2.bias, w2)
        dg, acc_g = grad_target(bn1.weight)
        db, acc_b = grad_target(bn1.bias)
        assert acc_g == acc_b
        dz1, _ = bn_bwd(dy1, None, z1, mean1, invstd1, bn1.weight, True, False, dg, db, acc_g, beta=bn1.bias)
        dx = conv_dgrad(dz1, w1, tuple(x.shape), 1, 1, residual=dres) if ctx.needs_input_grad[0] else None
        dw, acc_w = grad_target(w1)
        conv_wgrad_async(x, dz1, w1, 1, 1, dw, acc_w)
        grad_done(bn1.weight, bn1.bias, w1)
        return dx, None, None, None, None


def _block_desc(d, shape, step, xin, params, act, stat, acc=None):
    w1, bn1, w2, bn2 = params
    d.N, d.H, d.W, d.C = shape
    d.x = xin
    d.gamma1, d.beta1 = bn1.weight.data_ptr(), bn1.bias.data_ptr()
    d.gamma2, d.beta2 = bn2.weight.data_ptr(), bn2.bias.data_ptr()
    d.z1, d.z2, d.y = act, act + step, act + 2 * step
    d.stat = stat
    if acc is None:
        d.w1_bwd = _conv3x3_prepared(w1, 1).data_ptr()
        d.w2_bwd = _conv3x3_prepared(w2, 1).data_ptr()
    else:
        d.w1_fwd = _conv3x3_prepared(w1, 0).data_ptr()
        d.w2_fwd = _conv3x3_prepared(w2, 0).data_ptr()
        if bn1.track_running_stats:
            d.running_mean1, d.running_var1 = bn1.running_mean.data_ptr(), bn1.running_var.data_ptr()
            d.running_mean2, d.running_var2 = bn2.running_mean.data_ptr(), bn2.running_var.data_ptr()
            _count_batch(bn1)
            _count_batch(bn2)
        d.eps1, d.momentum1 = bn1.eps, 0.1 if bn1.momentum is None else bn1.momentum
        d.eps2, d.momentum2 = bn2.eps, 0.1 if bn2.momentum is None else bn2.momentum
        d.acc = acc
    return act + 2 * step


def _block_grads(g, tmp, step, dy, want_dx, params, bn_acc, ws, ws_bytes):
    w1, bn1, w2, bn2 = params
    g.dy = dy
    g.dz2, g.dres, g.dy1, g.dz1 = tmp, tmp + step, tmp + 2 * step, tmp + 3 * step
    g.dx = tmp + 4 * step if want_dx else 0
    dg2, acc_g2 = grad_target(bn2.weight)
    db2, acc_b2 = grad_target(bn2.bias)
    dw2, acc_w2 = grad_target(w2)
    dg1, acc_g1 = grad_target(bn1.weight)
    db1, acc_b1 = grad_target(bn1.bias)
    dw1, acc_w1 = grad_target(w1)
    assert acc_g2 == acc_b2 and acc_g1 == acc_b1
    weight_rsc(dw1)
    weight_rsc(dw2)
    g.dw1, g.dw2 = dw1.data_ptr(), dw2.data_ptr()
    g.dgamma1, g.dbeta1, g.dgamma2, g.dbeta2 = dg1.data_ptr(), db1.data_ptr(), dg2.data_ptr(), db2.data_ptr()
    g.acc_w1, g.acc_w2, g.acc_bn1, g.acc_bn2 = int(acc_w1), int(acc_w2), int(acc_g1), int(acc_g2)
    g.bn_acc = bn_acc
    g.wg_ws, g.wg_ws_bytes = ws, ws_bytes


def _native_bwd_done(side, tensors, blocks):
    if side is not None:
        for t in tensors:
            t.record_stream(side)
        _queue_join()
    elif _branch["on"]:
        _queue_join()
    for (w1, bn1, w2, bn2) in blocks:
        grad_done(bn2.weight, bn2.bias, w2)
        grad_done(bn1.weight, bn1.bias, w1)


class _Chain:
    ACT = 3
    STAT = 4
    TMP, DX = 5, 4
    ACCS = 2

    def __init__(self, x, blocks, descs, at=0):
        self.x, self.blocks, self.n, self.descs, self.at, self.shape = x, blocks, len(blocks), descs, at, tuple(x.shape)
        self.step, self.accb = 4 * x.numel(), self.ACCS * acc_bytes(self.shape[3])

    def _fill(self, act, stat, pbase=None):
        shape, step, accb, descs, at = self.shape, self.step, self.accb, self.descs, self.at
        xin, abase, sbase, astep, sstep = self.x.data_ptr(), act.data_ptr(), stat.data_ptr(), self.ACT * step, self.STAT * shape[3] * 4
        for k, blk in enumerate(self.blocks):
            xin = _block_desc(descs[at + k], shape, step, xin, blk, abase + astep * k, sbase + sstep * k, pbase and pbase + k * accb)

    def forward(self):
        n, shape, dev = self.n, self.shape, self.x.device
        act = torch.empty((n, self.ACT) + shape, dtype=torch.float32, device=dev)
        stat = torch.empty((n, self.STAT, shape[3]), dtype=torch.float32, device=dev)
        self._fill(act, stat, AccRef(shape[3], dev, self.ACCS * n).ptr)
        return act, stat

    def grad_buffers(self, slabs=TMP):
        self.tmp = torch.empty((self.n, slabs) + self.shape, dtype=torch.float32, device=self.x.device)
        self.bn_acc = AccRef(self.shape[3], self.x.device, self.ACCS * self.n).ptr
        return self.tmp

    def backward(self, grads, act, stat, dy, want_dx, ws, ws_bytes):
        n, step, tb, at, bn_acc, accb = self.n, self.step, self.tmp.data_ptr(), self.at, self.bn_acc, self.accb
        tstep = self.TMP * step
        self._fill(act, stat)
        for k, blk in enumerate(self.blocks):
            up = dy.data_ptr() if k == n - 1 else tb + tstep * (k + 1) + self.DX * step
            _block_grads(grads[at + k], tb + tstep * k, step, up, k > 0 or want_dx, blk, bn_acc + k * accb, ws, ws_bytes)


def _chain_forward(ctx, x, blocks):
    n = len(blocks)
    descs = (_C.BasicBlockDesc * n)()
    act, stat = _Chain(x, blocks, descs).forward()
    check(lib().buctd_basic_chain_fwd_train(n, descs, stream_ptr()), "basic_chain_fwd_train")
    ctx.blocks = blocks
    ctx.save_for_backward(x, act, stat)
    return act[n - 1, 2]


def _chain_backward(ctx, dy, want_dx):
    blocks = ctx.blocks
    n = len(blocks)
    x, act, stat = ctx.saved_tensors
    dy = _contig(dy)
    descs = (_C.BasicBlockDesc * n)()
    grads = (_C.BasicBlockGrads * n)()
    ch = _Chain(x, blocks, descs)
    tmp = ch.grad_buffers(_Chain.TMP if (n > 1 or want_dx) else _Chain.TMP - 1)
    main = torch.cuda.current_stream(x.device)
    use_side = _side["on"]
    side = _side_stream(x.device) if use_side else main
    wg_ws = workspace_on(side, _wgrad3x3_workspace("bf16x6", *ch.shape, ch.shape[3]), x.device)
    ch.backward(grads, act, stat, dy, want_dx, wg_ws.data_ptr(), wg_ws.numel())
    check(lib().buctd_basic_chain_bwd(n, descs, grads, main.cuda_stream, side.cuda_stream if use_side else None),
          "basic_chain_bwd")
    _native_bwd_done(side if use_side else None, (x, act, stat, tmp, dy), reversed(blocks))
    return tmp[0, _Chain.DX] if want_dx else None


class BasicChainFn(torch.autograd.Function):

    @staticmethod
    def forward(ctx, x, w_first, blocks):
        return _chain_forward(ctx, x, blocks)

    @staticmethod
    def backward(ctx, dy):
        return _chain_backward(ctx, dy, ctx.needs_input_grad[0]), None, None


_GROUP_BRANCHES = {"on": True}


def set_group_branches(on):
    old = _GROUP_BRANCHES["on"]
    _GROUP_BRANCHES["on"] = bool(on)
    return old


_GROUP_PARTS = {"n": 2}


def set_group_parts(n):
    old = _GROUP_PARTS["n"]
    _GROUP_PARTS["n"] = int(n)
    return old


def group_branch_partition(nb):
    if _GROUP_PARTS["n"] <= 1 or nb < 3:
        return [list(range(nb))]
    if nb == 3:
        return [[0], [1, 2]] if _GROUP_PARTS["n"] == 2 else [[0, 2], [1]]
    return [[0, 1], [2, 3]] if _GROUP_PARTS["n"] == 2 else [[0, 3], [1, 2]]


def group_branches_ok(xs, chains):
    if not (_GROUP_BRANCHES["on"] and 1 <= len(xs) <= 4 and len({len(c) for c in chains}) == 1):
        return False
    cfs = set()
    for x, chain in zip(xs, chains):
        if not (x.is_cuda and x.dim() == 4 and native_chain_ok(tuple(x.shape)) and bn_in_fusable(tuple(x.shape), chain[0][0])):
            return False
        Cn = x.shape[-1]
        cfs.add(3 if Cn % 48 == 0 else 2 if Cn % 32 == 0 else 0)
    return len(cfs) == 1 and 0 not in cfs


def eval_branches_ok(xs, chains):
    if not (_GROUP_BRANCHES["on"] and _conv_math["mode"] == "bf16x6" and 2 <= len(xs) <= 4 and len({len(c) for c in chains}) == 1):
        return False
    for x, chain in zip(xs, chains):
        if not (x.is_cuda and x.dim() == 4 and x.dtype == torch.float32 and x.is_contiguous()):
            return False
        for (w1, _, w2, _) in chain:
            if not (_bf16x3_ok(conv_desc(x.shape, _wshape(w1), 1, 1)) and _bf16x3_ok(conv_desc(x.shape, _wshape(w2), 1, 1))):
                return False
            if _wshape(w1)[0] != x.shape[-1] or _wshape(w2)[0] != x.shape[-1]:
                return False

    def one_kernel():
        items = (_C.C3Conv * len(xs))()
        for it, x in zip(items, xs):
            it.N, it.H, it.W, it.Ci, it.Co = x.shape[0], x.shape[1], x.shape[2], x.shape[3], x.shape[3]
            it.x = it.wprep = it.y = xs[0].data_ptr()
        return lib().buctd_conv3x3_bf16x6_group_workgroups(len(xs), items) > 0
    return _memo(("evalgrp",) + tuple(tuple(x.shape) for x in xs), one_kernel)


def basic_branches_eval(xs, chains):
    nb, n = len(xs), len(chains[0])
    cur = list(xs)
    for k in range(n):
        folded = [(bn_fold_cached(ch[k][1], ch[k][1].weight, ch[k][1].bias, ch[k][1].eps),
                   bn_fold_cached(ch[k][3], ch[k][3].weight, ch[k][3].bias, ch[k][3].eps)) for ch in chains]
        mids = [torch.empty_like(x) for x in cur]
        outs = [torch.empty_like(x) for x in cur]
        for half, dst in ((0, mids), (1, outs)):
            items = (_C.C3ConvEval * nb)()
            for b in range(nb):
                x = cur[b] if half == 0 else mids[b]
                w = chains[b][k][2 * half]
                weight_rsc(w)
                N, H, W, Cn = x.shape
                sc, sh = folded[b][half]
                it = items[b]
                it.N, it.H, it.W, it.Ci, it.Co = N, H, W, Cn, _wshape(w)[0]
                it.x, it.wprep = x.data_ptr(), _conv3x3_prepared(w, 0).data_ptr()
                it.scale, it.shift = sc.data_ptr(), sh.data_ptr()
                it.residual = cur[b].data_ptr() if half == 1 else None
                it.relu = 1
                it.y = dst[b].data_ptr()
            check(lib().buctd_conv3x3_bf16x6_group_eval(nb, items, stream_ptr()), "conv3x3_group_eval")
        cur = outs
    return cur


class BasicBranchesFn(torch.autograd.Function):

    @staticmethod
    def forward(ctx, w_first, chains, *xs):
        nb, n = len(xs), len(chains[0])
        descs = (_C.BasicBlockDesc * (nb * n))()
        acts, stats = zip(*(_Chain(x, chains[b], descs, b * n).forward() for b, x in enumerate(xs)))
        check(lib().buctd_basic_branches_fwd_train(nb, n, descs, stream_ptr()), "basic_branches_fwd_train")
        ctx.chains = chains
        ctx.save_for_backward(*xs, *acts, *stats)
        return tuple(act[n - 1, 2] for act in acts)

    @staticmethod
    def backward(ctx, *dys):
        chains = ctx.chains
        nb, n = len(chains), len(chains[0])
        saved = ctx.saved_tensors
        xs, acts, stats = saved[:nb], saved[nb:2 * nb], saved[2 * nb:]
        dev = xs[0].device
        descs = (_C.BasicBlockDesc * (nb * n))()
        grads = (_C.BasicBlockGrads * (nb * n))()
        main = torch.cuda.current_stream(dev)
        use_side = _side["on"]
        side = _side_stream(dev) if use_side else main
        needs = []
        for x in xs:
            N, H, W, Cn = x.shape
            needs.append(_memo(("wg3g", nb, N, H, W, Cn), lambda: (int(lib().buctd_conv3x3_wgrad_bf16x6_group_workspace(
                nb, N, H, W, Cn, Cn)) + 255) & ~255))
        wg_ws = workspace_on(side, sum(needs), dev)
        ws_ptr = wg_ws.data_ptr()
        tmps, keep = [], []
        for b, x in enumerate(xs):
            dy = torch.zeros_like(x) if dys[b] is None else _contig(dys[b])
            keep.append(dy)
            ch = _Chain(x, chains[b], descs, b * n)
            tmps.append(ch.grad_buffers())
            ch.backward(grads, acts[b], stats[b], dy, ctx.needs_input_grad[2 + b], ws_ptr, needs[b])
            ws_ptr += needs[b]
        check(lib().buctd_basic_branches_bwd(nb, n, descs, grads, main.cuda_stream, side.cuda_stream if use_side else None),
              "basic_branches_bwd")
        _native_bwd_done(side if use_side else None, list(xs) + list(acts) + list(stats) + tmps + keep,
                         (chains[b][k] for k in range(n - 1, -1, -1) for b in range(nb)))
        return (None, None) + tuple(tmps[b][0, _Chain.DX] if ctx.needs_input_grad[2 + b] else None for b in range(nb))


class Conv(torch.autograd.Function):

    @staticmethod
    def forward(ctx, x, w, b, stride, pad, relu):
        y = conv_fwd(x, w, b, stride, pad, relu=relu)
        ctx.meta = (w, b, stride, pad, relu, tuple(x.shape))
        ctx.save_for_backward(x, y if relu else None)
        return y

    @staticmethod
    def backward(ctx, dy):
        w, b, stride, pad, relu, x_shape = ctx.meta
        x, y = ctx.saved_tensors
        dy = _contig(dy)
        if relu:
            dy = relu_bwd(dy, y)
        dx = conv_dgrad(dy, w, x_shape, stride, pad) if ctx.needs_input_grad[0] else None
        if w.requires_grad:
            dw, acc = grad_target(w)
            conv_wgrad_async(x, dy, w, stride, pad, dw, acc)
        if b is not None and b.requires_grad:
            db, acc = grad_target(b)
            colsum(dy, dy.shape[-1], db, acc)
        grad_done(w, b)
        return dx, None, None, None, None, None


class FuseSum(torch.autograd.Function):

    @staticmethod
    def forward(ctx, shifts, relu, *terms):
        out = fuse_sum(list(terms), list(shifts), relu)
        ctx.shifts, ctx.relu = shifts, relu
        ctx.save_for_backward(out if relu else None)
        return out

    @staticmethod
    def backward(ctx, dy):
        (y,) = ctx.saved_tensors
        dy = _contig(dy)
        cache = {}
        grads = []
        for j, s in enumerate(ctx.shifts):
            if not ctx.needs_input_grad[2 + j]:
                grads.append(None)
                continue
            if s not in cache:
                cache[s] = fuse_sum_bwd(dy, y, s) if s > 0 or ctx.relu else dy
            grads.append(cache[s])
        return (None, None, *grads)


class AddN(torch.autograd.Function):

    @staticmethod
    def forward(ctx, a, b, c):
        out = add(a, b)
        if c is not None:
            out = add(out, c, out=out)
        ctx.n = 3 if c is not None else 2
        return out

    @staticmethod
    def backward(ctx, dy):
        return dy, dy, (dy if ctx.n == 3 else None)


def add_n(terms):
    acc = terms[0]
    k = 1
    while k < len(terms):
        group = [acc] + list(terms[k:k + 3])
        k += 3
        out = torch.empty_like(acc)
        arr = (C.c_void_p * len(group))(*[t.data_ptr() for t in group])
        check(lib().buctd_add_n(arr, len(group), ptr(out), acc.numel(), stream_ptr()), "add_n")
        acc = out
    return acc


class FanOut(torch.autograd.Function):

    @staticmethod
    def forward(ctx, x, n):
        return tuple(x.view_as(x) for _ in range(n))

    @staticmethod
    def backward(ctx, *grads):
        gs = [_contig(g) for g in grads if g is not None]
        if not gs:
            return None, None
        return (gs[0] if len(gs) == 1 else add_n(gs)), None


class ToNCHW(torch.autograd.Function):
    @staticmethod
    def forward(ctx, x):
        return nhwc_to_nchw(x)

    @staticmethod
    def backward(ctx, dy):
        return nchw_to_nhwc(_contig(dy))


class PositionAttention(torch.autograd.Function):

    @staticmethod
    def forward(ctx, q, k, v, h, p_drop, training):
        packed = k is None
        B, Tq = q.shape[0], q.shape[1]
        ldq = q.shape[2]
        hdk = ldq // 2 if packed else ldq
        kt, k_off, ldk = (q, hdk, ldq) if packed else (k, 0, k.shape[2])
        Tk = kt.shape[1]
        dk, dv = hdk // h, v.shape[2] // h
        scale = 1.0 / math.sqrt(dk)
        p_eff = p_drop if training else 0.0
        seed = next_seed()
        S = torch.empty((B, h, Tq, Tk), dtype=torch.float32, device=q.device)
        for i in range(h):
            matmul(q, kt, S, batch=B, M=Tq, N=Tk, K=dk, a_layout=0, b_layout=0, lda=ldq, ldb=ldk, ldc=Tk,
                   stride_a=Tq * ldq, stride_b=Tk * ldk, stride_c=h * Tq * Tk, a_off=i * dk, b_off=k_off + i * dk,
                   c_off=i * Tq * Tk)
        P, Pd = softmax_dropout_fwd(S, Tk, scale, p_eff, seed)
        O = torch.empty((B, Tq, h * dv), dtype=torch.float32, device=q.device)
        for i in range(h):
            matmul(Pd, v, O, batch=B, M=Tq, N=dv, K=Tk, a_layout=0, b_layout=1, lda=Tk, ldb=h * dv, ldc=h * dv,
                   stride_a=h * Tq * Tk, stride_b=Tk * h * dv, stride_c=Tq * h * dv, a_off=i * Tq * Tk,
                   b_off=i * dv, c_off=i * dv)
        ctx.meta = (h, dk, dv, scale, p_eff, seed, packed)
        ctx.save_for_backward(q, k, v, P, Pd if p_eff > 0 else None)
        return O

    @staticmethod
    def backward(ctx, dO):
        h, dk, dv, scale, p_eff, seed, packed = ctx.meta
        q, k, v, P, Pd = ctx.saved_tensors
        if Pd is None:
            Pd = P
        dO = _contig(dO)
        B, Tq, ldq = q.shape
        hdk = h * dk
        kt, k_off, ldk = (q, hdk, ldq) if packed else (k, 0, k.shape[2])
        Tk = kt.shape[1]
        hdv = h * dv
        dq = torch.empty_like(q)
        dkk = dq if packed else torch.empty_like(k)
        dvv = torch.empty_like(v)
        dP = torch.empty_like(P)
        for i in range(h):
            matmul(Pd, dO, dvv, batch=B, M=Tk, N=dv, K=Tq, a_layout=1, b_layout=1, lda=Tk, ldb=hdv, ldc=hdv,
# ... 327 lines not shown
```

include/buctd_hip.h:

```cpp
#ifndef BUCTD_HIP_H
#define BUCTD_HIP_H
#include <stddef.h>
#include <stdint.h>

#ifdef __cplusplus
extern "C" {
#endif

int buctd_version(void);
const char* buctd_last_error(void);

typedef struct {
  int N, H, W, Ci;
  int Co, R, S;
  int stride, pad;
  int Ho, Wo;
} buctd_conv_desc;

int buctd_conv2d_fwd_thin(const buctd_conv_desc* d);
int buctd_conv2d_fwd(const buctd_conv_desc* d, const float* x, const float* w, const float* bias,
                     const float* scale, const float* shift, const float* residual, int relu, float* y,
                     float* stats_partials, void* stream);
int buctd_conv2d_dgrad(const buctd_conv_desc* d, const float* dy, const float* w, const float* bias, float* dx,
                       float* stats_partials, void* stream);
int buctd_conv2d_stats_groups(const buctd_conv_desc* d, int transposed, int* ngroups, int* rows_per_group);
size_t buctd_conv2d_wgrad_workspace(const buctd_conv_desc* d);
int buctd_conv2d_wgrad(const buctd_conv_desc* d, const float* x, const float* dy, float* dw, int accumulate,
                       void* workspace, size_t workspace_bytes, void* stream);
#define BUCTD_CONV_BIAS 1
#define BUCTD_CONV_SCALE 2
#define BUCTD_CONV_RESIDUAL 4
#define BUCTD_CONV_RELU 8
#define BUCTD_CONV_STATS 16
#define BUCTD_CONV_PLAN_INTS 11
int buctd_conv2d_plan(const buctd_conv_desc* d, int direction, int flags, int* out);

int buctd_conv3x3_bf16x6_supported(int N, int H, int W, int Ci, int Co);
int buctd_conv3x3_bf16x6_stats_groups(int N, int H, int W, int Ci, int Co, int* ngroups, int* rows_per_group);
size_t buctd_conv3x3_bf16x6_prep_bytes(int Ci, int Co, int flip);
int buctd_conv3x3_bf16x6_prep(int Ci, int Co, const float* w, int flip, void* wprep, void* stream);
int buctd_conv3x3_bf16x6(int N, int H, int W, int Ci, int Co, const float* x, const void* wprep, const float* bias,
                         const float* scale, const float* shift, const float* residual, int relu, float* y,
                         float* stats_partials, int* stats_counts, void* stream);
int buctd_conv3x3_bf16x6_bnin(int N, int H, int W, int Ci, int Co, const float* x, const void* wprep, const float* bias,
                              const float* scale, const float* shift, const float* residual, int relu, float* y,
                              float* stats_partials, int* stats_counts, const float* in_mean, const float* in_invstd,
                              const float* in_gamma, const float* in_beta, int in_relu, void* stream);
int buctd_conv3x3_bf16x6_bnstat(int N, int H, int W, int Ci, int Co, const float* x, const void* wprep, const float* residual,
                                float* y, const float* bn_z, const float* bn_y, const float* bn_mean, const float* bn_invstd,
                                const float* bn_gamma, const float* bn_beta, float* bn_part, void* stream);
struct buctd_bn_acc_in_;
int buctd_conv3x3_bf16x6_acc(int N, int H, int W, int Ci, int Co, const float* x, const void* wprep, const float* residual,
                             int relu, float* y, void* stats_acc, const struct buctd_bn_acc_in_* in_bn, const float* in_gamma,
                             const float* in_beta, int in_relu, void* stream);
int buctd_conv3x3_bf16x6_bnstat_acc(int N, int H, int W, int Ci, int Co, const float* x, const void* wprep,
                                    const float* residual, float* y, const float* bn_z, const float* bn_y,
                                    const float* bn_mean, const float* bn_invstd, const float* bn_gamma, const float* bn_beta,
                                    void* bn_acc, void* stream);
typedef struct {
  int N, H, W, Ci, Co;
  const float* x;
  const void* wprep;
  const float* residual;
  int relu;
  float* y;
  void* stats_acc;
  const struct buctd_bn_acc_in_* in_bn;
  const float *in_gamma, *in_beta;
  int in_relu;
  const float *bn_z, *bn_y, *bn_mean, *bn_invstd, *bn_gamma, *bn_beta;
  void* bn_acc;
} buctd_c3_conv;
int buctd_conv3x3_bf16x6_group(int n, const buctd_c3_conv* convs, void* stream);
typedef struct {
  int N, H, W, Ci, Co;
  const float* x;
  const void* wprep;
  const float *scale, *shift;
  const float* residual;
  int relu;
  float* y;
} buctd_c3_conv_eval;
int buctd_conv3x3_bf16x6_group_eval(int n, const buctd_c3_conv_eval* convs, void* stream);
int buctd_conv3x3_bf16x6_group_workgroups(int n, const buctd_c3_conv* convs);
int buctd_conv3x3_bf16x6_plan(int N, int H, int W, int Ci, int Co, int option_set, int* out);
int buctd_conv3x3_bf16x3_supported(int N, int H, int W, int Ci, int Co);
int buctd_conv3x3_bf16x3_stats_groups(int N, int H, int W, int Ci, int Co, int* ngroups, int* rows_per_group);
size_t buctd_conv3x3_bf16x3_prep_bytes(int Ci, int Co, int flip);
int buctd_conv3x3_bf16x3_prep(int Ci, int Co, const float* w, int flip, void* wprep, void* stream);
typedef struct {
  const float* w;
  void* wprep;
  int Ci, Co, flip, reserved;
  long piece_begin;
} buctd_c3_prep_item;
int buctd_conv3x3_bf16x3_prep_batched(const buctd_c3_prep_item* items_device, int n, long total_pieces, void* stream);
int buctd_conv3x3_bf16x3(int N, int H, int W, int Ci, int Co, const float* x, const void* wprep, const float* bias,
                         const float* scale, const float* shift, const float* residual, int relu, float* y,
                         float* stats_partials, int* stats_counts, void* stream);

int buctd_conv3x3_wgrad_bf16x6_supported(int N, int H, int W, int Ci, int Co);
int buctd_conv3x3_wgrad_bf16x6_plan(int N, int H, int W, int Ci, int Co, int* out);
size_t buctd_conv3x3_wgrad_bf16x6_workspace(int N, int H, int W, int Ci, int Co);
int buctd_conv3x3_wgrad_bf16x6(int N, int H, int W, int Ci, int Co, const float* x, const float* dy, float* dw,
                               int accumulate, void* workspace, size_t workspace_bytes, void* stream);
int buctd_conv3x3_wgrad_bf16x6_bnin(int N, int H, int W, int Ci, int Co, const float* x, const float* dy, float* dw,
                                    int accumulate, const float* x_mean, const float* x_invstd, const float* x_gamma,
                                    const float* x_beta, int x_relu, void* workspace, size_t workspace_bytes,
                                    void* stream);
typedef struct {
  int N, H, W, Ci, Co;
  const float *x, *dy;
  float* dw;
  int accumulate;
  const float *x_mean, *x_invstd, *x_gamma, *x_beta;
  int x_relu;
  void* workspace;
  size_t workspace_bytes;
} buctd_wg3_conv;
size_t buctd_conv3x3_wgrad_bf16x6_group_workspace(int n, int N, int H, int W, int Ci, int Co);
int buctd_conv3x3_wgrad_bf16x6_group(int n, const buctd_wg3_conv* convs, void* stream);
int buctd_conv3x3_wgrad_bf16x6_group_workgroups(int n, const buctd_wg3_conv* convs);
int buctd_conv3x3_wgrad_bf16x3_supported(int N, int H, int W, int Ci, int Co);
size_t buctd_conv3x3_wgrad_bf16x3_workspace(int N, int H, int W, int Ci, int Co);
int buctd_conv3x3_wgrad_bf16x3(int N, int H, int W, int Ci, int Co, const float* x, const float* dy, float* dw,
                               int accumulate, void* workspace, size_t workspace_bytes, void* stream);

typedef struct {
  int batch, M, N, K;
  int a_layout;
  int b_layout;
  int lda, ldb, ldc;
  long stride_a, stride_b, stride_c;
  int Kc; long group_stride_a, group_stride_bk;
  int Nc; long group_stride_bn, group_stride_c;
  float alpha;
  int bias_axis;
} buctd_matmul_desc;
size_t buctd_matmul_workspace(const buctd_matmul_desc* d);
int buctd_matmul(const buctd_matmul_desc* d, const float* A, const float* B, const float* bias, float* C,
                 void* workspace, size_t workspace_bytes, void* stream);
#define BUCTD_MATMUL_PLAN_INTS 8
int buctd_matmul_plan(const buctd_matmul_desc* d, const void* A, const void* B, int* out);

int buctd_bn_finalize(const float* partials, const int* group_counts, int ngroups, int rows_per_group, long rows,
                      int C, float eps, float momentum, float* mean, float* invstd, float* running_mean,
                      float* running_var, void* stream);
int buctd_bn_stats(const float* z, long rows, int C, float* partials, int* ngroups, int* rows_per_group,
                   void* stream);
int buctd_bn_stats_groups(long rows, int C, int* ngroups, int* rows_per_group);
int buctd_bn_apply(const float* z, const float* mean, const float* invstd, const float* gamma, const float* beta,
                   const float* residual, int relu, float* y, long rows, int C, void* stream);
size_t buctd_bn_bwd_workspace(long rows, int C);
int buctd_bn_bwd(const float* dy, const float* y, const float* z, const float* mean, const float* invstd,
                 const float* gamma, const float* beta, int relu, long rows, int C, float* dz, float* dres,
                 float* dgamma, float* dbeta, int accumulate, void* workspace, size_t workspace_bytes, void* stream);
int buctd_bn_bwd_from_partials(const float* dy, const float* y, const float* z, const float* mean, const float* invstd,
                               const float* gamma, const float* beta, int relu, long rows, int C, const float* part,
                               int nparts, float* dz, float* dres, float* dgamma, float* dbeta, int accumulate,
                               void* workspace, size_t workspace_bytes, void* stream);
size_t buctd_bn_acc_bytes(int C);
typedef struct buctd_bn_acc_in_ {
  const void* acc;
  long rows;
  float eps, momentum;
  float *mean_out, *invstd_out;
  float *running_mean, *running_var;
} buctd_bn_acc_in;
int buctd_bn_apply_acc(const float* z, const buctd_bn_acc_in* st, const float* gamma, const float* beta,
                       const float* residual, int relu, float* y, long rows, int C, void* stream);
int buctd_bn_bwd_acc(const float* dy, const float* y, const float* z, const float* mean, const float* invstd,
                     const float* gamma, const float* beta, int relu, long rows, int C, float* dz, float* dres,
                     float* dgamma, float* dbeta, int accumulate, void* acc, int acc_ready, void* stream);
typedef struct {
  const float* z;
  buctd_bn_acc_in st;
  const float *gamma, *beta, *residual;
  int relu;
  float* y;
  long rows;
  int C;
} buctd_bn_apply_item;
int buctd_bn_apply_acc_group(int n, const buctd_bn_apply_item* items, void* stream);
typedef struct {
  const float *dy, *y, *z, *mean, *invstd, *gamma, *beta;
  int relu;
  long rows;
  int C;
  float *dz, *dres, *dgamma, *dbeta;
  int accumulate;
  void* acc;
  int acc_ready;
} buctd_bn_bwd_item;
int buctd_bn_bwd_acc_group(int n, const buctd_bn_bwd_item* items, void* stream);
int buctd_bn_fold(const float* gamma, const float* beta, const float* running_mean, const float* running_var,
                  float eps, int C, float* scale, float* shift, void* stream);

int buctd_add(const float* a, const float* b, float* out, long n, int relu, void* stream);
int buctd_add_n(const float* const* terms, int n, float* out, long count, void* stream);
int buctd_mul(const float* a, const float* b, float* out, long n, void* stream);
int buctd_scale(const float* x, const float* dev_scalar, float alpha, float* out, long n, void* stream);
int buctd_copy_channels(const float* src, long rows, int Cs, int cs0, float* dst, int Cd, int cd0, int Cc,
                        void* stream);
int buctd_add_bcast(const float* a, const float* v, float* out, long batch, long n, void* stream);
int buctd_relu_bwd(const float* dy, const float* y, float* dx, long n, void* stream);
size_t buctd_colsum_workspace(long rows, int C);
int buctd_colsum(const float* x, long rows, int C, float* out, int accumulate, void* workspace,
                 size_t workspace_bytes, void* stream);
int buctd_nchw_to_nhwc(const float* x, int N, int Ctot, int c0, int Cc, int H, int W, float* y, void* stream);
int buctd_nhwc_to_nchw(const float* x, int N, int C, int H, int W, float* y, void* stream);
int buctd_fuse_sum(const float* const* terms, const int* shifts, int nterms, int N, int H, int W, int C, int relu,
                   float* out, void* stream);
int buctd_fuse_sum_bwd(const float* dy, const float* y, int shift, int N, int H, int W, int C, float* g,
                       void* stream);
int buctd_resize_bilinear(const float* x, int N, int Ctot, int c0, int Cc, int H, int W, int Ho, int Wo, float* y,
                          void* stream);
int buctd_maxpool3x3s2_fwd(const float* x, int N, int H, int W, int C, float* y, int32_t* idx, void* stream);
int buctd_maxpool3x3s2_bwd(const float* dy, const int32_t* idx, int N, int H, int W, int C, float* dx,
                           void* stream);

int buctd_softmax_dropout_fwd(const float* s, long rows, int L, float scale, float p_drop, uint64_t seed, float* p,
                              float* pd, void* stream);
int buctd_softmax_dropout_bwd(const float* dpd, const float* p, long rows, int L, float scale, float p_drop,
                              uint64_t seed, float* ds, void* stream);
// ... 272 lines not shown
```

Before: 512.9 images/s.

## Store ReLU-masked gradient from dgrad epilogue, dropping separate dres buffer in chains

When the BN-backward sums of the next block are fused into the conv1 dgrad epilogue, the kernel now writes the ReLU-masked gradient instead of the raw dx. The following BN-backward then reads dy directly and skips its own ReLU mask and its residual-gradient write. The residual skip path uses that masked tensor. This removes one full-size activation write and read per inner block and one temp slab per block, at the cost of a new kernel variant and more intricate buffer indexing.

```diff
diff --git a/buctd_amd/_C.py b/buctd_amd/_C.py
--- a/buctd_amd/_C.py
+++ b/buctd_amd/_C.py
@@ -37,7 +37,8 @@
                 [(n, C.c_void_p) for n in ("x", "wprep", "residual")] + [("relu", C.c_int)] +
                 [(n, C.c_void_p) for n in ("y", "stats_acc")] + [("in_bn", C.POINTER(BnAccIn))] +
                 [(n, C.c_void_p) for n in ("in_gamma", "in_beta")] + [("in_relu", C.c_int)] +
-                [(n, C.c_void_p) for n in ("bn_z", "bn_y", "bn_mean", "bn_invstd", "bn_gamma", "bn_beta", "bn_acc")])
+                [(n, C.c_void_p) for n in ("bn_z", "bn_y", "bn_mean", "bn_invstd", "bn_gamma", "bn_beta", "bn_acc")] +
+                [("mask_out", C.c_int)])
 
 
 class C3ConvEval(C.Structure):
@@ -157,6 +158,7 @@
     "buctd_bn_bwd_acc": (_I, [_P, _P, _P, _P, _P, _P, _P, _I, _L, _I, _P, _P, _P, _P, _I, _P, _I, _P]),
     "buctd_conv3x3_bf16x6_acc": (_I, [_I] * 5 + [_P, _P, _P, _I, _P, _P, C.POINTER(BnAccIn), _P, _P, _I, _P]),
     "buctd_conv3x3_bf16x6_bnstat_acc": (_I, [_I] * 5 + [_P] * 12),
+    "buctd_conv3x3_bf16x6_bnstat_acc_mask": (_I, [_I] * 5 + [_P] * 11 + [_I, _P]),
     "buctd_gconv_x6_fwd_acc": (_I, [_I] * 6 + [_P] * 6),
     "buctd_conv3x3_bf16x6_group": (_I, [_I, C.POINTER(C3Conv), _P]),
     "buctd_conv3x3_bf16x6_group_eval": (_I, [_I, C.POINTER(C3ConvEval), _P]),
diff --git a/buctd_amd/csrc/block.hip b/buctd_amd/csrc/block.hip
--- a/buctd_amd/csrc/block.hip
+++ b/buctd_amd/csrc/block.hip
@@ -12,9 +12,9 @@
   return b.x && b.w1_fwd && b.w2_fwd && b.z1 && b.z2 && b.y && b.acc && b.stat;
 }
 
-static bool bwd_ptrs_ok(const buctd_basic_block& b, const buctd_basic_block_grads& g) {
-  return b.x && b.w1_bwd && b.w2_bwd && b.z1 && b.z2 && b.y && b.stat && g.dy && g.dres && g.dy1 && g.dw1 && g.dw2 && g.bn_acc &&
-         g.wg_ws && g.dz2 && g.dz1;
+static bool bwd_ptrs_ok(const buctd_basic_block& b, const buctd_basic_block_grads& g, bool masked) {
+  return b.x && b.w1_bwd && b.w2_bwd && b.z1 && b.z2 && b.y && b.stat && g.dy && (g.dres || masked) && g.dy1 && g.dw1 && g.dw2 &&
+         g.bn_acc && g.wg_ws && g.dz2 && g.dz1;
 }
 
 
@@ -71,8 +71,8 @@
 static int issue_dgrad(bool group, int n, const buctd_c3_conv* c, void* s) {
   if (group) return buctd_conv3x3_bf16x6_group(n, c, s);
   if (c->bn_acc)
-    return buctd_conv3x3_bf16x6_bnstat_acc(c->N, c->H, c->W, c->Ci, c->Co, c->x, c->wprep, c->residual, c->y, c->bn_z, c->bn_y,
-                                           c->bn_mean, c->bn_invstd, c->bn_gamma, c->bn_beta, c->bn_acc, s);
+    return buctd_conv3x3_bf16x6_bnstat_acc_mask(c->N, c->H, c->W, c->Ci, c->Co, c->x, c->wprep, c->residual, c->y, c->bn_z, c->bn_y,
+                                                c->bn_mean, c->bn_invstd, c->bn_gamma, c->bn_beta, c->bn_acc, c->mask_out, s);
   return buctd_conv3x3_bf16x6(c->N, c->H, c->W, c->Ci, c->Co, c->x, c->wprep, nullptr, nullptr, nullptr, c->residual, 0, c->y,
                               nullptr, nullptr, s);
 }
@@ -146,8 +146,12 @@
       const buctd_basic_block& B = blocks[b * n + k];
       const buctd_basic_block_grads& G = grads[b * n + k];
       chain[b] = k > 0 && bn2_sums_chain(&B, &G);
-      bi[b] = buctd_bn_bwd_item{G.dy, B.y, B.z2, mean2_of(B), invstd2_of(B), B.gamma2, nullptr, 1, (long)B.N * B.H * B.W, B.C,
-                                G.dz2, G.dres, G.dgamma2, G.dbeta2, G.acc_bn2, acc2_of(G.bn_acc, B.C), ready[b] ? 1 : 0};
+      if (ready[b])
+        bi[b] = buctd_bn_bwd_item{G.dy, nullptr, B.z2, mean2_of(B), invstd2_of(B), B.gamma2, nullptr, 0, (long)B.N * B.H * B.W, B.C,
+                                  G.dz2, nullptr, G.dgamma2, G.dbeta2, G.acc_bn2, acc2_of(G.bn_acc, B.C), 1};
+      else
+        bi[b] = buctd_bn_bwd_item{G.dy, B.y, B.z2, mean2_of(B), invstd2_of(B), B.gamma2, nullptr, 1, (long)B.N * B.H * B.W, B.C,
+                                  G.dz2, G.dres, G.dgamma2, G.dbeta2, G.acc_bn2, acc2_of(G.bn_acc, B.C), 0};
     }
     BLK_TRY(issue_bn_bwd(group, nb, bi, stream));
     BLK_TRY(stream_fork(main_s, side_s, who));
@@ -186,14 +190,16 @@
     for (int b = 0; b < nb; ++b) {
       const buctd_basic_block& B = blocks[b * n + k];
       const buctd_basic_block_grads& G = grads[b * n + k];
+      const float* skip = ready[b] ? G.dy : G.dres;
       ready[b] = chain[b];
       if (!G.dx) continue;
       buctd_c3_conv& c = cv[m++] = c3_of(B);
-      c.x = G.dz1; c.wprep = B.w1_bwd; c.residual = G.dres; c.y = G.dx;
+      c.x = G.dz1; c.wprep = B.w1_bwd; c.residual = skip; c.y = G.dx;
       if (chain[b]) {
         const buctd_basic_block& Bp = blocks[b * n + k - 1];
         c.bn_z = Bp.z2; c.bn_y = Bp.y; c.bn_mean = mean2_of(Bp); c.bn_invstd = invstd2_of(Bp); c.bn_gamma = Bp.gamma2;
         c.bn_acc = acc2_of(grads[b * n + k - 1].bn_acc, B.C);
+        c.mask_out = 1;
       }
     }
     if (m) BLK_TRY(issue_dgrad(group, m, cv, stream));
@@ -210,7 +216,8 @@
                                      void* side_stream) {
   BUCTD_CHECK_ARG(n > 0 && blocks && grads, "buctd_basic_chain_bwd: bad argument");
   for (int k = 0; k < n; ++k)
-    BUCTD_CHECK_ARG(bwd_ptrs_ok(blocks[k], grads[k]), "buctd_basic_chain_bwd: null pointer in block %d", k);
+    BUCTD_CHECK_ARG(bwd_ptrs_ok(blocks[k], grads[k], k + 1 < n && bn2_sums_chain(&blocks[k + 1], &grads[k + 1])),
+                    "buctd_basic_chain_bwd: null pointer in block %d", k);
   return row_bwd(false, "buctd_basic_chain_bwd", 1, n, blocks, grads, stream, side_stream);
 }
 
@@ -224,7 +231,8 @@
                                         void* stream, void* side_stream) {
   BUCTD_CHECK_ARG(nb > 0 && nb <= BR_MAX && n > 0 && blocks && grads, "buctd_basic_branches_bwd: 1..%d branches", BR_MAX);
   for (int i = 0; i < nb * n; ++i)
-    BUCTD_CHECK_ARG(bwd_ptrs_ok(blocks[i], grads[i]), "buctd_basic_branches_bwd: null pointer in block %d", i);
+    BUCTD_CHECK_ARG(bwd_ptrs_ok(blocks[i], grads[i], i % n + 1 < n && bn2_sums_chain(&blocks[i + 1], &grads[i + 1])),
+                    "buctd_basic_branches_bwd: null pointer in block %d", i);
   return row_bwd(true, "buctd_basic_branches_bwd", nb, n, blocks, grads, stream, side_stream);
 }
 
diff --git a/buctd_amd/csrc/c3_common.h b/buctd_amd/csrc/c3_common.h
--- a/buctd_amd/csrc/c3_common.h
+++ b/buctd_amd/csrc/c3_common.h
@@ -53,6 +53,7 @@
   const float* bs_gamma;
   const float* bs_beta;
   float* bs_part;
+  int mask_out;
   long long* stats_acc;
   long long* bs_acc;
   BnAccFwd in_acc;
@@ -265,7 +266,7 @@
 #pragma unroll
           for (int j = 0; j < 4; ++j) v[j] = fmaxf(v[j], 0.f);
         }
-        *reinterpret_cast<f32x4*>(p.out + off + n) = v;
+        if (!p.mask_out) *reinterpret_cast<f32x4*>(p.out + off + n) = v;
         if (bs_on) {
           const f32x4 zz = pre_z[ps & 1][k];
           const f32x4 mu = *reinterpret_cast<const f32x4*>(p.bs_mean + n);
@@ -281,6 +282,7 @@
 #pragma unroll
           for (int j = 0; j < 4; ++j)
             if (!(yy[j] > 0.f)) gm[j] = 0.f;
+          if (p.mask_out) *reinterpret_cast<f32x4*>(p.out + off + n) = gm;
           bs1[k % NACC] += gm;
           bs2[k % NACC] += gm * (zz - mu) * is;
         }
diff --git a/buctd_amd/csrc/c3_lean.h b/buctd_amd/csrc/c3_lean.h
--- a/buctd_amd/csrc/c3_lean.h
+++ b/buctd_amd/csrc/c3_lean.h
@@ -1,7 +1,7 @@
 #pragma once
 #include "c3_common.h"
 
-enum { C3M_IN_BN = 1, C3M_STATS = 2, C3M_RES = 4, C3M_BS_REBUILD = 8, C3M_BS_Y = 16 };
+enum { C3M_IN_BN = 1, C3M_STATS = 2, C3M_RES = 4, C3M_BS_REBUILD = 8, C3M_BS_Y = 16, C3M_MASK_OUT = 32 };
 
 #define C3_OOB 0x80000000u
 __device__ __forceinline__ __amdgpu_buffer_rsrc_t c3_rsrc(const void* ptr, unsigned bytes) {
@@ -23,7 +23,9 @@
                                              int n0) {
   constexpr bool STATS = (MODE & C3M_STATS) != 0, RES = (MODE & C3M_RES) != 0;
   constexpr bool BSR = (MODE & C3M_BS_REBUILD) != 0, BSY = (MODE & C3M_BS_Y) != 0, BS = BSR || BSY;
+  constexpr bool MASK = (MODE & C3M_MASK_OUT) != 0;
   static_assert(!(STATS && BS), "c3l_epilogue: forward statistics and backward sums never meet in one launch");
+  static_assert(!MASK || (BSY && RES), "c3l_epilogue: the masked store belongs to the RES | BS_Y option set");
   const int t = threadIdx.x, lane = t & 63;
   const int wave = __builtin_amdgcn_readfirstlane(t >> 6);
   const int i16 = lane & 15, g = lane >> 4;
@@ -141,7 +143,7 @@
     for (int k = 0; k < NI; ++k) {
       const bool ok = off[k] != C3_OOB;
       if constexpr (RES) v[k] += pre_r[ps & 1][k];
-      c3_bstore(r_out, off[k] + colb + c4_k[k] * 16, v[k]);
+      if constexpr (!MASK) c3_bstore(r_out, off[k] + colb + c4_k[k] * 16, v[k]);
       if constexpr (STATS) {
         f32x4 d = v[k] - pq[k % NACC];
 #pragma unroll
@@ -166,6 +168,7 @@
         f32x4 gm;
 #pragma unroll
         for (int j = 0; j < 4; ++j) gm[j] = (ok && yy[j] > 0.f) ? v[k][j] : 0.f;
+        if constexpr (MASK) c3_bstore(r_out, off[k] + colb + c4_k[k] * 16, gm);
         s1[k % NACC] += gm;
         f32x4 tm = gm * (zz - mu) * is;
         s2[k % NACC] += tm;
diff --git a/buctd_amd/csrc/conv3x3.hip b/buctd_amd/csrc/conv3x3.hip
--- a/buctd_amd/csrc/conv3x3.hip
+++ b/buctd_amd/csrc/conv3x3.hip
@@ -1,7 +1,7 @@
 #include "c3_common.h"
 #include <string.h>
 
-enum { C3M_IN_BN = 1, C3M_STATS = 2, C3M_RES = 4, C3M_BS_REBUILD = 8, C3M_BS_Y = 16 };
+enum { C3M_IN_BN = 1, C3M_STATS = 2, C3M_RES = 4, C3M_BS_REBUILD = 8, C3M_BS_Y = 16, C3M_MASK_OUT = 32 };
 int c3_lean_launch(const C3Group& h, int fam, int mode, unsigned grid, size_t lds, hipStream_t st);
 
 template <int NP, int MF, int NF, int WM, int WN>
@@ -638,7 +638,7 @@
 }
 
 struct C3InBn { const float* mean; const float* invstd; const float* gamma; const float* beta; int relu; };
-struct C3BwdStat { const float* z; const float* y; const float* mean; const float* invstd; const float* gamma; const float* beta; float* part; long long* acc; };
+struct C3BwdStat { const float* z; const float* y; const float* mean; const float* invstd; const float* gamma; const float* beta; float* part; long long* acc; int mask_out; };
 struct C3Acc { long long* stats_acc; const buctd_bn_acc_in* in; };
 
 static int c3_fill_shape(int np, int N, int H, int W, int Ci, int Co, C3Args& a, C3Plan& pl) {
@@ -695,18 +695,23 @@
   }
   a.bs_z = a.bs_y = a.bs_mean = a.bs_invstd = a.bs_gamma = a.bs_beta = nullptr;
   a.bs_part = nullptr;
+  a.mask_out = 0;
+  BUCTD_CHECK_ARG(!(bst && bst->mask_out) || (bst->acc && bst->y && residual),
+                  "buctd_conv3x3: the masked store needs the BatchNorm-backward accumulator, the forward output y and a residual");
   if (bst && (bst->part || bst->acc)) {
     BUCTD_CHECK_ARG(np == 3 && bst->z && bst->mean && bst->invstd && (bst->y || (bst->gamma && bst->beta)),
                     "buctd_conv3x3: the BatchNorm-backward by-product needs the bf16x6 kernel, z, mean, invstd and y or gamma + beta");
     a.bs_z = bst->z; a.bs_y = bst->y; a.bs_mean = bst->mean; a.bs_invstd = bst->invstd; a.bs_gamma = bst->gamma;
     a.bs_beta = bst->beta; a.bs_part = bst->part; a.bs_acc = bst->acc;
+    a.mask_out = bst->mask_out ? 1 : 0;
   }
   return BUCTD_OK;
 }
 
 static int c3_lean_mask(int m) {
   switch (m) {
-    case C3M_STATS: case C3M_STATS | C3M_IN_BN: case C3M_BS_REBUILD: case C3M_RES | C3M_BS_Y: case C3M_RES: return m;
+    case C3M_STATS: case C3M_STATS | C3M_IN_BN: case C3M_BS_REBUILD: case C3M_RES | C3M_BS_Y: case C3M_RES:
+    case C3M_RES | C3M_BS_Y | C3M_MASK_OUT: return m;
     default: return -1;
   }
 }
@@ -720,6 +725,7 @@
   if (a.stats_acc) m |= C3M_STATS;
   if (a.res) m |= C3M_RES;
   if (a.bs_acc) m |= a.bs_y ? C3M_BS_Y : C3M_BS_REBUILD;
+  if (a.mask_out) m |= C3M_MASK_OUT;
   return c3_lean_mask(m);
 }
 
@@ -864,7 +870,7 @@
                                            const float* residual, float* y, const float* bn_z, const float* bn_y,
                                            const float* bn_mean, const float* bn_invstd, const float* bn_gamma,
                                            const float* bn_beta, float* bn_part, void* stream) {
-  C3BwdStat b{bn_z, bn_y, bn_mean, bn_invstd, bn_gamma, bn_beta, bn_part, nullptr};
+  C3BwdStat b{bn_z, bn_y, bn_mean, bn_invstd, bn_gamma, bn_beta, bn_part, nullptr, 0};
   BUCTD_CHECK_ARG(bn_part, "buctd_conv3x3_bf16x6_bnstat: null partials pointer");
   return c3_run(3, N, H, W, Ci, Co, x, wprep, nullptr, nullptr, nullptr, residual, 0, y, nullptr, nullptr, stream, nullptr,
                 &b);
@@ -884,7 +890,14 @@
                                                const float* residual, float* y, const float* bn_z, const float* bn_y,
                                                const float* bn_mean, const float* bn_invstd, const float* bn_gamma,
                                                const float* bn_beta, void* bn_acc, void* stream) {
-  C3BwdStat b{bn_z, bn_y, bn_mean, bn_invstd, bn_gamma, bn_beta, nullptr, (long long*)bn_acc};
+  return buctd_conv3x3_bf16x6_bnstat_acc_mask(N, H, W, Ci, Co, x, wprep, residual, y, bn_z, bn_y, bn_mean, bn_invstd, bn_gamma,
+                                              bn_beta, bn_acc, 0, stream);
+}
+extern "C" int buctd_conv3x3_bf16x6_bnstat_acc_mask(int N, int H, int W, int Ci, int Co, const float* x, const void* wprep,
+                                                    const float* residual, float* y, const float* bn_z, const float* bn_y,
+                                                    const float* bn_mean, const float* bn_invstd, const float* bn_gamma,
+                                                    const float* bn_beta, void* bn_acc, int mask_out, void* stream) {
+  C3BwdStat b{bn_z, bn_y, bn_mean, bn_invstd, bn_gamma, bn_beta, nullptr, (long long*)bn_acc, mask_out};
   BUCTD_CHECK_ARG(bn_acc, "buctd_conv3x3_bf16x6_bnstat_acc: null accumulator");
   return c3_run(3, N, H, W, Ci, Co, x, wprep, nullptr, nullptr, nullptr, residual, 0, y, nullptr, nullptr, stream, nullptr,
                 &b);
@@ -894,7 +907,8 @@
   for (int k = 0; k < n; ++k) {
     const buctd_c3_conv& c = convs[k];
     C3InBn ib{nullptr, nullptr, c.in_gamma, c.in_beta, c.in_relu};
-    C3BwdStat bs{c.bn_z, c.bn_y, c.bn_mean, c.bn_invstd, c.bn_gamma, c.bn_beta, nullptr, (long long*)c.bn_acc};
+    C3BwdStat bs{c.bn_z, c.bn_y, c.bn_mean, c.bn_invstd, c.bn_gamma, c.bn_beta, nullptr, (long long*)c.bn_acc, c.mask_out};
+    BUCTD_CHECK_ARG(!c.mask_out || c.bn_acc, "buctd_conv3x3_bf16x6_group: mask_out without a BatchNorm-backward accumulator");
     C3Acc ac{(long long*)c.stats_acc, c.in_bn};
     BUCTD_CHECK_ARG(!c.in_bn || c.in_bn->acc, "buctd_conv3x3_bf16x6_group: in_bn without an accumulator");
     const int rc = c3_fill(3, c.N, c.H, c.W, c.Ci, c.Co, c.x, c.wprep, nullptr, nullptr, nullptr, c.residual, c.relu, c.y,
@@ -961,6 +975,7 @@
     if (option_set & C3M_RES) a.res = on;
     if (option_set & (C3M_BS_REBUILD | C3M_BS_Y)) a.bs_acc = (long long*)on;
     if (option_set & C3M_BS_Y) a.bs_y = on;
+    if (option_set & C3M_MASK_OUT) a.mask_out = 1;
   }
   C3Dry dry{};
   if (const int rc = c3_launch_one(a, pl, nullptr, &dry)) return rc;
diff --git a/buctd_amd/csrc/conv3x3_lean.hip b/buctd_amd/csrc/conv3x3_lean.hip
--- a/buctd_amd/csrc/conv3x3_lean.hip
+++ b/buctd_amd/csrc/conv3x3_lean.hip
@@ -50,7 +50,7 @@
 }
 
 int c3_lean_launch(const C3Group& h, int fam, int mode, unsigned grid, size_t lds, hipStream_t st) {
-  static unsigned char attr_done[2][5][BUCTD_MAX_DEVICES] = {{{0}}};
+  static unsigned char attr_done[2][6][BUCTD_MAX_DEVICES] = {{{0}}};
   void (*fn)(C3Group) = nullptr;
   int mi = -1;
 #define C3L_PICK(i, m)                                                                               \
@@ -63,6 +63,7 @@
   C3L_PICK(2, C3M_BS_REBUILD)
   C3L_PICK(3, C3M_RES | C3M_BS_Y)
   C3L_PICK(4, C3M_RES)
+  C3L_PICK(5, C3M_RES | C3M_BS_Y | C3M_MASK_OUT)
 #undef C3L_PICK
   if (!fn) {
     buctd_set_error("conv3x3 (bf16x6, train mode): no kernel for option set %d", mode);
diff --git a/buctd_amd/csrc/conv_gather_x6.hip b/buctd_amd/csrc/conv_gather_x6.hip
--- a/buctd_amd/csrc/conv_gather_x6.hip
+++ b/buctd_amd/csrc/conv_gather_x6.hip
@@ -559,7 +559,7 @@
   e.P = (int)((long)N * e.IB + e.SW);
   e.relu = relu; e.na = 0;
   e.in_mean = e.in_invstd = e.in_gamma = e.in_beta = nullptr; e.in_relu = 0; e.col_major = 0;
-  e.bs_z = e.bs_y = e.bs_mean = e.bs_invstd = e.bs_gamma = e.bs_beta = nullptr; e.bs_part = nullptr;
+  e.bs_z = e.bs_y = e.bs_mean = e.bs_invstd = e.bs_gamma = e.bs_beta = nullptr; e.bs_part = nullptr; e.mask_out = 0;
   e.stats_acc = stats_acc; e.bs_acc = nullptr;
   memset(&e.in_acc, 0, sizeof(e.in_acc));
   BUCTD_CHECK_ARG(!(dir && stats_acc), "%s: no statistics on the data gradient", who);
diff --git a/buctd_amd/ops.py b/buctd_amd/ops.py
--- a/buctd_amd/ops.py
+++ b/buctd_amd/ops.py
@@ -1653,11 +1653,14 @@
     return act + 2 * step
 
 
-def _block_grads(g, tmp, step, dy, want_dx, params, bn_acc, ws, ws_bytes):
+def _block_grads(g, tmp, step, dy, want_dx, params, bn_acc, ws, ws_bytes, inner=False):
     w1, bn1, w2, bn2 = params
     g.dy = dy
-    g.dz2, g.dres, g.dy1, g.dz1 = tmp, tmp + step, tmp + 2 * step, tmp + 3 * step
-    g.dx = tmp + 4 * step if want_dx else 0
+    if inner:
+        g.dz2, g.dres, g.dy1, g.dz1 = tmp, 0, tmp + step, tmp + 2 * step
+    else:
+        g.dz2, g.dres, g.dy1, g.dz1 = tmp, tmp + step, tmp + 2 * step, tmp + 3 * step
+    g.dx = tmp + (3 if inner else 4) * step if want_dx else 0
     dg2, acc_g2 = grad_target(bn2.weight)
     db2, acc_b2 = grad_target(bn2.bias)
     dw2, acc_w2 = grad_target(w2)
@@ -1689,7 +1692,7 @@
 class _Chain:
     ACT = 3
     STAT = 4
-    TMP, DX = 5, 4
+    TMP = 5
     ACCS = 2
 
     def __init__(self, x, blocks, descs, at=0):
@@ -1709,18 +1712,23 @@
         self._fill(act, stat, AccRef(shape[3], dev, self.ACCS * n).ptr)
         return act, stat
 
-    def grad_buffers(self, slabs=TMP):
-        self.tmp = torch.empty((self.n, slabs) + self.shape, dtype=torch.float32, device=self.x.device)
+    def grad_buffers(self, last_dx=True):
+        slabs = (self.TMP - 1) * (self.n - 1) + (self.TMP if last_dx else self.TMP - 1)
+        self.tmp = torch.empty((slabs,) + self.shape, dtype=torch.float32, device=self.x.device)
         self.bn_acc = AccRef(self.shape[3], self.x.device, self.ACCS * self.n).ptr
         return self.tmp
 
+    def dx(self):
+        return self.tmp[self.TMP - 2 if self.n > 1 else self.TMP - 1]
+
     def backward(self, grads, act, stat, dy, want_dx, ws, ws_bytes):
         n, step, tb, at, bn_acc, accb = self.n, self.step, self.tmp.data_ptr(), self.at, self.bn_acc, self.accb
-        tstep = self.TMP * step
+        tstep = (self.TMP - 1) * step
         self._fill(act, stat)
         for k, blk in enumerate(self.blocks):
-            up = dy.data_ptr() if k == n - 1 else tb + tstep * (k + 1) + self.DX * step
-            _block_grads(grads[at + k], tb + tstep * k, step, up, k > 0 or want_dx, blk, bn_acc + k * accb, ws, ws_bytes)
+            inner = k < n - 1
+            up = tb + tstep * (k + 1) + (self.TMP - 2 if k + 2 < n else self.TMP - 1) * step if inner else dy.data_ptr()
+            _block_grads(grads[at + k], tb + tstep * k, step, up, k > 0 or want_dx, blk, bn_acc + k * accb, ws, ws_bytes, inner)
 
 
 def _chain_forward(ctx, x, blocks):
@@ -1741,7 +1749,7 @@
     descs = (_C.BasicBlockDesc * n)()
     grads = (_C.BasicBlockGrads * n)()
     ch = _Chain(x, blocks, descs)
-    tmp = ch.grad_buffers(_Chain.TMP if (n > 1 or want_dx) else _Chain.TMP - 1)
+    tmp = ch.grad_buffers(n > 1 or want_dx)
     main = torch.cuda.current_stream(x.device)
     use_side = _side["on"]
     side = _side_stream(x.device) if use_side else main
@@ -1750,7 +1758,7 @@
     check(lib().buctd_basic_chain_bwd(n, descs, grads, main.cuda_stream, side.cuda_stream if use_side else None),
           "basic_chain_bwd")
     _native_bwd_done(side if use_side else None, (x, act, stat, tmp, dy), reversed(blocks))
-    return tmp[0, _Chain.DX] if want_dx else None
+    return ch.dx() if want_dx else None
 
 
 class BasicChainFn(torch.autograd.Function):
@@ -1882,19 +1890,20 @@
                 nb, N, H, W, Cn, Cn)) + 255) & ~255))
         wg_ws = workspace_on(side, sum(needs), dev)
         ws_ptr = wg_ws.data_ptr()
-        tmps, keep = [], []
+        tmps, keep, dxs = [], [], []
         for b, x in enumerate(xs):
             dy = torch.zeros_like(x) if dys[b] is None else _contig(dys[b])
             keep.append(dy)
             ch = _Chain(x, chains[b], descs, b * n)
             tmps.append(ch.grad_buffers())
+            dxs.append(ch.dx())
             ch.backward(grads, acts[b], stats[b], dy, ctx.needs_input_grad[2 + b], ws_ptr, needs[b])
             ws_ptr += needs[b]
         check(lib().buctd_basic_branches_bwd(nb, n, descs, grads, main.cuda_stream, side.cuda_stream if use_side else None),
               "basic_branches_bwd")
         _native_bwd_done(side if use_side else None, list(xs) + list(acts) + list(stats) + tmps + keep,
                          (chains[b][k] for k in range(n - 1, -1, -1) for b in range(nb)))
-        return (None, None) + tuple(tmps[b][0, _Chain.DX] if ctx.needs_input_grad[2 + b] else None for b in range(nb))
+        return (None, None) + tuple(dxs[b] if ctx.needs_input_grad[2 + b] else None for b in range(nb))
 
 
 class Conv(torch.autograd.Function):
diff --git a/include/buctd_hip.h b/include/buctd_hip.h
--- a/include/buctd_hip.h
+++ b/include/buctd_hip.h
@@ -57,6 +57,10 @@
                                     const float* residual, float* y, const float* bn_z, const float* bn_y,
                                     const float* bn_mean, const float* bn_invstd, const float* bn_gamma, const float* bn_beta,
                                     void* bn_acc, void* stream);
+int buctd_conv3x3_bf16x6_bnstat_acc_mask(int N, int H, int W, int Ci, int Co, const float* x, const void* wprep,
+                                         const float* residual, float* y, const float* bn_z, const float* bn_y,
+                                         const float* bn_mean, const float* bn_invstd, const float* bn_gamma,
+                                         const float* bn_beta, void* bn_acc, int mask_out, void* stream);
 typedef struct {
   int N, H, W, Ci, Co;
   const float* x;
@@ -70,6 +74,7 @@
   int in_relu;
   const float *bn_z, *bn_y, *bn_mean, *bn_invstd, *bn_gamma, *bn_beta;
   void* bn_acc;
+  int mask_out;
 } buctd_c3_conv;
 int buctd_conv3x3_bf16x6_group(int n, const buctd_c3_conv* convs, void* stream);
 typedef struct {
```

Measured after the change: 516.1 images/s (median of 6 runs). No clear change (+0.6%).
